# SheffieldML/GPy

Measured on AMD Instinct MI355X. Metric: exact-GP log_lik+grad iters/sec, higher is better.
Workload: dtype f64; 1 GPU; BASELINE configs[2]: matern52 ARD exact GP, one GPRegression.parameters_changed, N=16384 D=32 Dy=1 per GPU; N=16384, D=32, kernel=matern52, ARD=True, parallelism=replicas x1

## Files before the change

### gpy_amd/_lib.py

```python
import ctypes
import os
import subprocess

import numpy as np
from numpy.ctypeslib import ndpointer

_HERE = os.path.dirname(os.path.abspath(__file__))
LIB_PATH = os.environ.get("MI355GP_LIB") or os.path.join(_HERE, "libmi355gp.so")
CSRC = os.path.join(_HERE, "csrc")

KIND_IDS = {"rbf": 0, "matern52": 1, "matern32": 2, "exponential": 3, "white": 4, "bias": 5, "ratquad": 6, "stdperiodic": 7,
            "coregionalize": 8, "linear": 9, "mlp": 10, "poly": 11, "cosine": 12, "sinc": 13, "expquadcosine": 14}


def ard_id(kind, ARD):
    if kind == "coregionalize":
        return int(ARD)
    return int(ARD) & 3 if kind == "stdperiodic" else int(bool(ARD))


class Part(ctypes.Structure):
    _fields_ = [("kind", ctypes.c_int), ("ard", ctypes.c_int), ("n_active", ctypes.c_int),
                ("active_dims", ctypes.POINTER(ctypes.c_int)), ("theta", ctypes.POINTER(ctypes.c_double)),
                ("term", ctypes.c_int)]


def make_parts(specs):
    arr = (Part * len(specs))()
    keep, ntheta = [], 0
    for i, spec in enumerate(specs):
        kind, ARD, theta, dims = spec[:4]
        arr[i].term = int(spec[4]) if len(spec) > 4 else 0
        th = np.ascontiguousarray(theta, dtype=np.float64)
        keep.append(th)
        arr[i].kind = KIND_IDS[kind]
        arr[i].ard = ard_id(kind, ARD)
        arr[i].theta = th.ctypes.data_as(ctypes.POINTER(ctypes.c_double))
        if dims is None:
            arr[i].n_active = 0
            arr[i].active_dims = None
        else:
            d = np.ascontiguousarray(dims, dtype=np.int32)
            keep.append(d)
            arr[i].n_active = d.size
            arr[i].active_dims = d.ctypes.data_as(ctypes.POINTER(ctypes.c_int))
        ntheta += th.size
    return arr, keep, ntheta
FETCH_L, FETCH_KINV, FETCH_DLDK, FETCH_K = 0, 1, 2, 3
EP_BERNOULLI_PROBIT = 0
OUT_LML, OUT_LOGDET, OUT_DATAFIT, OUT_DNOISE, OUT_TRKINV, NUM_OUT = 0, 1, 2, 3, 4, 8
STAGE_NAMES = ("kbuild", "potrf", "trtri", "lauum", "solve", "grad", "total")
NUM_T = 8
PROFILE_FAMILIES = ("update_nt", "trtri", "lauum", "diag128", "trsm128", "update_nt64", "potrf_persist", "trtri_early")

_lib = None


class MI355GPError(RuntimeError):
    pass


DIAG_LIB_PATH = os.path.join(_HERE, "libmi355gp_diag.so")


def build(force=False):
    srcs = [os.path.join(CSRC, f) for f in os.listdir(CSRC) if f.endswith((".hip", ".h")) or f == "Makefile"]
    srcs.append(os.path.join(_HERE, "..", "include", "mi355gp.h"))
    srcs.append(os.path.join(_HERE, "..", "include", "mi355gp_debug.h"))
    product = os.path.join(_HERE, "libmi355gp.so")
    if not force and os.path.exists(product) and os.path.exists(DIAG_LIB_PATH):
        t = min(os.path.getmtime(product), os.path.getmtime(DIAG_LIB_PATH))
        if all(os.path.getmtime(s) <= t for s in srcs if os.path.exists(s)):
            return product
    r = subprocess.run(["make", "-C", CSRC, "-j8", "all", "diag"], capture_output=True, text=True)
    if r.returncode != 0 or not os.path.exists(product) or not os.path.exists(DIAG_LIB_PATH):
        raise MI355GPError("building libmi355gp.so failed:\n" + r.stdout[-4000:] + r.stderr[-4000:])
    return product


_ci, _i64, _cd, _vp, _str = ctypes.c_int, ctypes.c_int64, ctypes.c_double, ctypes.c_void_p, ctypes.c_char_p
_dp = ndpointer(dtype=np.float64, flags="C_CONTIGUOUS")
_c_dp = ctypes.POINTER(ctypes.c_double)
_ip, _hp, _parts = ctypes.POINTER(_ci), ctypes.POINTER(_vp), ctypes.POINTER(Part)
_i32a, _i64a = (ndpointer(dtype=t, flags="C_CONTIGUOUS") for t in (np.int32, np.int64))
_EXACT = [_vp, _ci, _ci, _dp, _dp, _i64, _cd, _cd, _dp] + [_c_dp] * 4
_KERN_X2 = [_dp, _i64, _c_dp, _i64, _ci, _dp]

ABI = {
    "mi355gp_last_error": [],
    "mi355gp_version": [],
    "mi355gp_device_count": [_ip],
    "mi355gp_device_synchronize": [_ci],
    "mi355gp_create": [_ci, _hp],
    "mi355gp_destroy": [_vp],
    "mi355gp_set_data": [_vp, _dp, _i64, _ci, _dp, _ci],
    "mi355gp_set_targets": [_vp, _dp, _ci],
    "mi355gp_kern_K": [_ci, _ci, _ci, _dp] + _KERN_X2,
    "mi355gp_kern_Kdiag": [_ci, _dp, _i64, _dp],
    "mi355gp_update_gradients_full": [_ci, _ci, _ci, _dp, _dp] + _KERN_X2,
    "mi355gp_gradients_X": [_ci, _ci, _ci, _dp, _dp] + _KERN_X2,
    "mi355gp_exact_inference": _EXACT,
    "mi355gp_exact_inference_sum": [_vp, _ci, _parts, _dp, _i64, _cd, _cd, _dp] + [_c_dp] * 4,
    "mi355gp_exact_studentt_sum": [_vp, _ci, _parts, _cd, _cd, _cd, _dp] + [_c_dp] * 3,
    "mi355gp_inference_given_K": [_vp, _dp, _dp, _i64, _cd, _cd, _dp] + [_c_dp] * 3,
    "mi355gp_fetch": [_vp, _ci, _dp, _ci],
    "mi355gp_predict": [_vp, _ci, _ci, _dp, _dp, _i64, _c_dp, _c_dp, _ci],
    "mi355gp_predict_sum": [_vp, _ci, _parts, _dp, _i64, _c_dp, _c_dp, _ci],
    "mi355gp_predictive_gradients_sum": [_vp, _ci, _parts, _dp, _i64, _c_dp, _c_dp],
    "mi355gp_laplace_begin": [_vp, _ci, _parts],
    "mi355gp_laplace_newton": [_vp, _dp, _dp, _cd, _dp, _dp, _c_dp],
    "mi355gp_laplace_finish": [_vp, _dp, _cd, _dp, _c_dp],
    "mi355gp_laplace_gradients": [_vp, _dp, _dp, _dp],
    "mi355gp_laplace_implicit": [_vp, _dp, _dp],
    "mi355gp_laplace_predict": [_vp, _ci, _parts, _dp, _i64, _dp, _c_dp, _c_dp, _ci],
    "mi355gp_ep_recompute": [_vp, _dp, _dp, _cd, _cd, _ci, _dp, _dp, _c_dp, _c_dp],
    "mi355gp_ep_sweep": [_vp, _ci, _i64a, _dp, _cd, _cd] + [_dp] * 7 + [_c_dp],
    "mi355gp_covariance_between_points": [_vp, _ci, _parts, _dp, _i64, _dp, _i64, _dp],
    "mi355gp_potrf": [_ci, _dp, _i64, _c_dp],
    "mi355gp_pdinv": [_ci, _dp, _i64] + [_c_dp] * 4,
    "mi355gp_pdinv_full": [_ci, _dp, _i64] + [_c_dp] * 5,
    "mi355gp_set_option": [_vp, _ci, _ci],
    "mi355gp_get_option": [_vp, _ci, _ip],
    "mi355gp_get_profile": [_vp, _dp, _dp, _i32a],
    "mi355gp_grid_unique_id": [_str],
    "mi355gp_grid_create": [_ci] * 6 + [_str, _hp],
    "mi355gp_grid_destroy": [_vp],
    "mi355gp_grid_set_data": [_vp, _dp, _i64, _ci, _dp, _ci],
    "mi355gp_grid_exact_inference": _EXACT,
    "mi355gp_grid_fetch": [_vp, _ci, _dp],
    "mi355gp_grid_set_option": [_vp, _ci, _ci],
    "mi355gp_grid_get_option": [_vp, _ci, _ip],
    "mi355gp_grid_coll_log": [_vp, _ci, _dp],
    "mi355gp_sparse_create": [_ci, _hp],
    "mi355gp_sparse_destroy": [_vp],
    "mi355gp_sparse_set_data": [_vp, _dp, _i64, _ci, _dp, _ci],
    "mi355gp_vardtc_inference": _EXACT,
    "mi355gp_vardtc_inference_sum": [_vp, _ci, _parts, _dp, _i64, _dp, _i64, _cd, _dp] + [_c_dp] * 6,
    "mi355gp_sparse_set_input_variance": [_vp, _dp, _i64, _ci],
    "mi355gp_sparse_set_inputs": [_vp, _dp, _c_dp, _i64, _ci],
    "mi355gp_vardtc_inference_uncertain": [_vp, _ci, _parts, _dp, _i64, _dp, _i64, _cd, _dp] + [_c_dp] * 6,
    "mi355gp_sparse_predict": [_vp, _ci, _parts, _dp, _i64, _c_dp, _c_dp, _ci],
    "mi355gp_sparse_predict_uncertain": [_vp, _ci, _parts, _dp, _dp, _i64, _dp, _c_dp],
    "mi355gp_sparse_get_predict_ms": [_vp, _c_dp],
    "mi355gp_sparse_fetch_dLdKnm": [_vp, _i64, _i64, _dp],
    "mi355gp_sparse_attach_comm": [_vp, _ci, _ci, _str],
    "mi355gp_sparse_attach_loopback": [_vp, _ci, _ci, _ci],
    "mi355gp_sparse_fetch": [_vp, _ci, _dp],
    "mi355gp_sparse_get_profile": [_vp, _dp],
    "mi355gp_svgp_forward": [_vp, _ci, _parts, _dp, _i64, _dp, _dp, _ci, _cd, _dp, _dp, _dp, _c_dp],
    "mi355gp_svgp_backward": [_vp, _dp, _dp] + [_c_dp] * 5,
    "mi355gp_svgp_predict": [_vp, _ci, _parts, _c_dp, _i64, _ci] + [_c_dp] * 4,
    "mi355gp_pep_inference": [_vp, _ci, _parts, _dp, _i64, _cd, _cd, _cd, _dp] + [_c_dp] * 5,
    "mi355gp_pep_check_sigma": [_dp, _i64, _i64, _cd, _cd],
    "mi355gp_rbf_psi": [_ci, _cd, _dp, _ci, _dp, _i64, _dp, _dp, _i64, _ci] + [_c_dp] * 3,
    "mi355gp_rbf_psi_grad": [_ci, _cd, _dp, _ci, _dp, _i64, _dp, _dp, _i64, _ci] + [_c_dp] * 4 + [_dp] * 5,
    "mi355gp_bench_factor": [_ci, _i64, _ci, _c_dp, _c_dp, _c_dp],
    "mi355gp_dbg_ipc_selftest": [_str, _ci, _ci, _ci, _ci, _i64, _dp],
    "mi355gp_dbg_comm_selftest": [_ci, _str, _ci, _ci, _ci, _ci, _i64, _ci, _dp],
    "mi355gp_dbg_grid_multi": [_ci, _ci, _ci, _ci, _dp],
    "mi355gp_dbg_update_nt": [_ci, _ci, _ip, _ci, _ci, _dp],
    "mi355gp_dbg_update_rect": [_ci, _ci, _ci, _ip, _ci, _ci, _dp],
    "mi355gp_dbg_mfma": [_ci, _dp, _dp, _dp],
    "mi355gp_dbg_gemm": [_ci, _ci, _ci, _i64, _i64, _i64, _dp, _dp, _dp, _cd, _cd, _ci, _c_dp],
    "mi355gp_dbg_peaks": [_ci, _dp],
    "mi355gp_dbg_gemm_clock": [_c_dp, _c_dp],
    "mi355gp_dbg_cu_map": [_ci, _ci, _ci, ctypes.POINTER(ctypes.c_uint)],
    "mi355gp_dbg_pipe_share": [_ci, _dp],
    "mi355gp_dbg_graph_factor": [_ci, _i64, _ci, _dp],
    "mi355gp_dbg_persist": [_ci, _i64, _ci, _ci, _dp],
    "mi355gp_dbg_lauum_plan": [_ci, _ip, _ci, _ip],
    "mi355gp_dbg_persist_owners": [_ci, _ci, _ci, _ip, _ip],
    "mi355gp_dbg_mask_probe": [_ci, _ci, _ci, _dp],
}
EXPORTED = tuple(ABI)


def _opt(a):
    return None if a is None else a.ctypes.data_as(_c_dp)


def lib():
    global _lib
    if _lib is None:
        if not os.path.exists(LIB_PATH):
            build()
        L = ctypes.CDLL(LIB_PATH)
        for name, argtypes in ABI.items():
            getattr(L, name).argtypes = argtypes
        L.mi355gp_last_error.restype = L.mi355gp_version.restype = _str
        _lib = L
    return _lib


OPTIONS = {"profile": 0, "lookahead": 1, "tri_overlap": 2, "tri_min_nt": 3, "tri_h": 4, "tri_wgs": 5, "tri_half": 6,
           "part1_on_panel": 7, "nbo": 8, "solve_overlap": 9, "diag_excl_first": 10, "graph": 11, "persist": 12, "agg2": 13,
           "persist_test": 14, "persist_aborts": 15, "persist_skip": 16, "persist_sched": 17}


def last_error():
    return lib().mi355gp_last_error().decode()


def check(rc, what):
    if rc < 0:
        raise MI355GPError("%s failed (rc=%d): %s" % (what, rc, last_error()))
    return rc


def device_count():
    n = ctypes.c_int(0)
    lib().mi355gp_device_count(ctypes.byref(n))
    return n.value


def device_synchronize(device=0):
    require_device(device)
    check(lib().mi355gp_device_synchronize(int(device)), "mi355gp_device_synchronize")


def require_device(device=0):
    n = device_count()
    if device >= n:
        raise MI355GPError("no MI355X visible to HIP (device %d requested, %d present): the gpy_amd backend has "
                           "no CPU fallback" % (device, n))


def f64(a):
    return np.ascontiguousarray(a, dtype=np.float64)


def theta_vec(variance, lengthscale, ARD, D):
    ls = np.atleast_1d(np.asarray(lengthscale, dtype=np.float64)).ravel()
    if ARD:
        if ls.size == 1:
            ls = np.full(D, ls[0])
        assert ls.size == D, "ARD kernel needs one lengthscale per input dimension"
    else:
        assert ls.size == 1, "isotropic kernel has a single lengthscale"
    return np.concatenate([[float(np.asarray(variance).ravel()[0])], ls])


def _exact_result(out, ms, **arrays):
    res = dict(lml=out[OUT_LML], logdet=out[OUT_LOGDET], datafit=out[OUT_DATAFIT], dnoise=out[OUT_DNOISE],
               trKinv=out[OUT_TRKINV], **arrays)
    if ms is not None:
        res["stage_ms"] = dict(zip(STAGE_NAMES, ms[:len(STAGE_NAMES)]))
    return res


def _predict(entry, head, Xnew, D, Dy, full_cov, want_var, between=()):
    Xnew = f64(Xnew)
    M = Xnew.shape[0]
    assert Xnew.shape[1] == D
    mu = np.empty((M, Dy))
    var = (np.empty((M, M)) if full_cov else np.empty(M)) if want_var else None
    check(getattr(lib(), entry)(*(tuple(head) + (Xnew, M) + tuple(between) + (mu.ctypes.data_as(_c_dp), _opt(var),
                                                                              int(bool(full_cov))))), entry)
    if var is not None and not full_cov:
        var = var[:, None]
    return mu, var


class _Handle(object):
    _create = _destroy = None

    def __init__(self, device=0):
        require_device(device)
        self._h = ctypes.c_void_p()
        check(getattr(lib(), self._create)(device, ctypes.byref(self._h)), self._create)
        self.device = device

    def close(self):
        if getattr(self, "_h", None) is not None and self._h.value:
            getattr(lib(), self._destroy)(self._h)
            self._h = ctypes.c_void_p()

    def __del__(self):
        try:
            self.close()
        except Exception:
            pass


class Context(_Handle):
    _create, _destroy = "mi355gp_create", "mi355gp_destroy"

    def __init__(self, device=0):
        super(Context, self).__init__(device)
        self.N = self.D = self.Dy = 0

    def set_data(self, X, R):
        X, R = f64(X), f64(R)
        assert X.ndim == 2 and R.ndim == 2 and X.shape[0] == R.shape[0]
        self.N, self.D = X.shape
        self.Dy = R.shape[1]
        check(lib().mi355gp_set_data(self._h, X, self.N, self.D, R, self.Dy), "mi355gp_set_data")

    def set_targets(self, R):
        R = f64(R)
        check(lib().mi355gp_set_targets(self._h, R, R.shape[1]), "mi355gp_set_targets")

    def _exact(self, entry, head, ntheta, noise, jitter, extra_jitter, want_alpha, want_diag, want_stage_ms):
        noise = f64(np.atleast_1d(noise))
        out = np.zeros(NUM_OUT)
        alpha = np.empty((self.N, self.Dy)) if want_alpha else None
        dtheta = np.zeros(ntheta)
        diag = np.empty(self.N) if want_diag else None
        ms = np.zeros(NUM_T) if want_stage_ms else None
        rc = check(getattr(lib(), entry)(self._h, *(tuple(head) + (noise, noise.size, jitter, extra_jitter, out, _opt(alpha),
                                                                   _opt(dtheta), _opt(diag), _opt(ms)))), entry)
        return rc, _exact_result(out, ms, alpha=alpha, dtheta=dtheta, diag_dL_dK=diag)

    def exact_inference(self, kind, ARD, theta, noise, jitter=1e-8, extra_jitter=0.0, want_alpha=True,
                        want_diag=False, want_stage_ms=False):
        theta = f64(theta)
        return self._exact("mi355gp_exact_inference", (KIND_IDS[kind], ard_id(kind, ARD), theta), theta.size, noise, jitter,
                           extra_jitter, want_alpha, want_diag, want_stage_ms)

    def exact_inference_sum(self, specs, noise, jitter=1e-8, extra_jitter=0.0, want_alpha=True, want_diag=False,
                            want_stage_ms=False):
        arr, keep, ntheta = make_parts(specs)
        return self._exact("mi355gp_exact_inference_sum", (len(specs), arr), ntheta, noise, jitter, extra_jitter, want_alpha,
                           want_diag, want_stage_ms)

    def predict_sum(self, specs, Xnew, full_cov=False, want_var=True):
        arr, keep, _ = make_parts(specs)
        return _predict("mi355gp_predict_sum", (self._h, len(specs), arr), Xnew, self.D, self.Dy, full_cov, want_var)

    def exact_studentt_sum(self, specs, nu, jitter=1e-8, extra_jitter=0.0):
        arr, keep, ntheta = make_parts(specs)
        out = np.zeros(NUM_OUT)
        alpha = np.empty((self.N, self.Dy))
        dtheta = np.zeros(ntheta)
        rc = check(lib().mi355gp_exact_studentt_sum(self._h, len(specs), arr, float(nu), jitter, extra_jitter, out,
                                                    _opt(alpha), _opt(dtheta), None), "mi355gp_exact_studentt_sum")
        return rc, dict(lml=out[OUT_LML], logdet=out[OUT_LOGDET], beta=out[OUT_DATAFIT], scale=out[5], alpha=alpha,
                        dtheta=dtheta)

    def predictive_gradients(self, specs, Xnew, want_var=True):
        arr, keep, _ = make_parts(specs)
        Xnew = f64(Xnew)
        M = Xnew.shape[0]
        assert Xnew.shape[1] == self.D
        dmu = np.empty((M, self.D, self.Dy))
        dvar = np.empty((M, self.D)) if want_var else None
        check(lib().mi355gp_predictive_gradients_sum(self._h, len(specs), arr, Xnew, M, dmu.ctypes.data_as(_c_dp), _opt(dvar)),
              "mi355gp_predictive_gradients_sum")
        return dmu, dvar

    def covariance_between_points(self, specs, X1, X2):
        arr, keep, _ = make_parts(specs)
        X1, X2 = f64(X1), f64(X2)
        out = np.empty((X1.shape[0], X2.shape[0]))
        check(lib().mi355gp_covariance_between_points(self._h, len(specs), arr, X1, X1.shape[0], X2, X2.shape[0], out),
              "mi355gp_covariance_between_points")
        return out

    def inference_given_K(self, K, noise, jitter=1e-8, extra_jitter=0.0, want_diag=False, want_stage_ms=False):
        K = f64(K)
        assert K.shape == (self.N, self.N)
        noise = f64(np.atleast_1d(noise))
        out = np.zeros(NUM_OUT)
        alpha = np.empty((self.N, self.Dy))
        diag = np.empty(self.N) if want_diag else None
        ms = np.zeros(NUM_T) if want_stage_ms else None
        rc = check(lib().mi355gp_inference_given_K(self._h, K, noise, noise.size, jitter, extra_jitter, out,
                                                   _opt(alpha), _opt(diag), _opt(ms)), "mi355gp_inference_given_K")
        return rc, _exact_result(out, ms, alpha=alpha, diag_dL_dK=diag)

    def laplace_begin(self, specs):
        arr, keep, ntheta = make_parts(specs)
        check(lib().mi355gp_laplace_begin(self._h, len(specs), arr), "mi355gp_laplace_begin")
        self._lap_ntheta = ntheta

    def laplace_newton(self, W, b, extra_jitter=0.0):
        W, b = f64(np.ravel(W)), f64(np.ravel(b))
        assert W.size == self.N and b.size == self.N
        a, Ka = np.empty(self.N), np.empty(self.N)
        ld = ctypes.c_double(0.0)
        rc = check(lib().mi355gp_laplace_newton(self._h, W, b, float(extra_jitter), a, Ka, ctypes.byref(ld)),
                   "mi355gp_laplace_newton")
        return rc, a, Ka, ld.value

    def laplace_finish(self, W, extra_jitter=0.0):
        W = f64(np.ravel(W))
        assert W.size == self.N
        d = np.empty(self.N)
        ld = ctypes.c_double(0.0)
        rc = check(lib().mi355gp_laplace_finish(self._h, W, float(extra_jitter), d, ctypes.byref(ld)), "mi355gp_laplace_finish")
        return rc, d, ld.value

    def laplace_gradients(self, Ki_f, dL_dfhat):
        Ki_f, s = f64(np.ravel(Ki_f)), f64(np.ravel(dL_dfhat))
        assert Ki_f.size == self.N and s.size == self.N
        dtheta = np.zeros(self._lap_ntheta)
        check(lib().mi355gp_laplace_gradients(self._h, Ki_f, s, dtheta), "mi355gp_laplace_gradients")
        return dtheta

    def laplace_implicit(self, dL_dfhat):
        d = f64(np.ravel(dL_dfhat))
        assert d.size == self.N
        s = np.empty(self.N)
        check(lib().mi355gp_laplace_implicit(self._h, d, s), "mi355gp_laplace_implicit")
        return s

    def laplace_predict(self, specs, Xnew, wv, full_cov=False, want_var=True):
        arr, keep, _ = make_parts(specs)
        wv = f64(np.ravel(wv))
        assert wv.size == self.N
        return _predict("mi355gp_laplace_predict", (self._h, len(specs), arr), Xnew, self.D, 1, full_cov, want_var,
                        between=(wv,))

    def ep_recompute(self, tau, v, extra_jitter=0.0, add_diag=0.0, want_sigma=True, want_ms=False):
        tau, v = f64(np.ravel(tau)), f64(np.ravel(v))
        assert tau.size == self.N and v.size == self.N
        mu, sd = np.empty(self.N), np.empty(self.N)
        ld, ms = ctypes.c_double(0.0), ctypes.c_double(0.0)
        rc = check(lib().mi355gp_ep_recompute(self._h, tau, v, float(extra_jitter), float(add_diag), int(bool(want_sigma)), mu, sd,
                                              ctypes.byref(ld), ctypes.byref(ms)), "mi355gp_ep_recompute")
        return (rc, mu, sd, ld.value) + ((ms.value,) if want_ms else ())

    def ep_sweep(self, order, ysign, tau, v, eta=1.0, delta=1.0, lik=EP_BERNOULLI_PROBIT, want_ms=False):
        order = np.ascontiguousarray(np.ravel(order), dtype=np.int64)
        ysign = f64(np.ravel(ysign))
        tau, v = f64(np.ravel(tau)).copy(), f64(np.ravel(v)).copy()
        assert order.size == self.N and ysign.size == self.N and tau.size == self.N and v.size == self.N
        o = [np.empty(self.N) for _ in range(5)]
        ms = ctypes.c_double(0.0)
        check(lib().mi355gp_ep_sweep(self._h, int(lik), order, ysign, float(eta), float(delta), tau, v, o[0], o[1], o[2], o[3], o[4],
                                     ctypes.byref(ms)), "mi355gp_ep_sweep")
        r = dict(tau=tau, v=v, cav_tau=o[0], cav_v=o[1], log_Z_hat=o[2], mu=o[3], Sigma_diag=o[4])
        if want_ms:
            r["ms"] = ms.value
        return r

    def set_option(self, name, value):
        if name == "profile" and not isinstance(value, (int, bool)):
            value = sum(1 << PROFILE_FAMILIES.index(f) for f in value) << 1
        check(lib().mi355gp_set_option(self._h, OPTIONS[name], int(value)), "mi355gp_set_option")

    def get_option(self, name):
        v = ctypes.c_int(0)
        check(lib().mi355gp_get_option(self._h, OPTIONS[name], ctypes.byref(v)), "mi355gp_get_option")
        return int(v.value)

    def get_profile(self):
        ms, fl, n = np.zeros(8), np.zeros(8), np.zeros(8, dtype=np.int32)
        check(lib().mi355gp_get_profile(self._h, ms, fl, n), "mi355gp_get_profile")
        return {k: (ms[i], fl[i], int(n[i])) for i, k in enumerate(PROFILE_FAMILIES)}

    def predict(self, kind, ARD, theta, Xnew, full_cov=False, want_var=True):
        return _predict("mi355gp_predict", (self._h, KIND_IDS[kind], ard_id(kind, ARD), f64(theta)), Xnew, self.D, self.Dy,
                        full_cov, want_var)

    def fetch(self, which, fortran_order=False):
        out = np.empty((self.N, self.N))
        check(lib().mi355gp_fetch(self._h, which, out, int(fortran_order)), "mi355gp_fetch")
        if fortran_order:
            return out.T
        return out


class SparseContext(_Handle):
    FETCH_DLDKMM, FETCH_WOODBURY_INV, FETCH_LM, FETCH_KMM, FETCH_PSI2, FETCH_DLDPSI2_BETA = 0, 1, 2, 3, 4, 5
    sharded = False
    _create, _destroy = "mi355gp_sparse_create", "mi355gp_sparse_destroy"

    def __init__(self, device=0):
        super(SparseContext, self).__init__(device)
        self.N = self.D = self.Dy = self.M = 0

    def attach_comm(self, rank, world, id_bytes):
        check(lib().mi355gp_sparse_attach_comm(self._h, rank, world, id_bytes), "mi355gp_sparse_attach_comm")
        self.sharded = True

    def set_data(self, X, Y):
        X, Y = f64(X), f64(Y)
        self.N, self.D = X.shape
        self.Dy = Y.shape[1]
        check(lib().mi355gp_sparse_set_data(self._h, X, self.N, self.D, Y, self.Dy), "mi355gp_sparse_set_data")

    def get_profile(self):
        o = np.zeros(6)
        check(lib().mi355gp_sparse_get_profile(self._h, o), "mi355gp_sparse_get_profile")
        return {"gemm_T": (o[0], o[1], int(o[2])), "gram_psi2": (o[3], o[4], int(o[5]))}

    def _fit(self, entry, head, ntheta, Z, scalars, extras, want_stage_ms, wv_cols=None):
        Z = f64(Z)
        self.M = Z.shape[0]
        assert Z.shape[1] == self.D
        out = np.zeros(NUM_OUT)
        dtheta = np.zeros(ntheta)
        dZ = np.zeros((self.M, self.D))
        wv = np.zeros((self.M, self.Dy if wv_cols is None else wv_cols))
        ms = np.zeros(4) if want_stage_ms else None
        args = tuple(head) + (Z, self.M) + tuple(scalars) + (out, _opt(dtheta), _opt(dZ), _opt(wv))
        rc = check(getattr(lib(), entry)(self._h, *(args + tuple(_opt(e) for e in extras) + (_opt(ms),))), entry)
        res = dict(lml=out[0], dnoise=out[1], dtheta=dtheta, dZ=dZ, woodbury_vector=wv)
        if ms is not None:
            res["stage_ms"] = dict(pass1=ms[0], mxm=ms[1], pass2=ms[2], total=ms[3])
        return rc, out, res

    def vardtc(self, kind, ARD, theta, Z, noise_var, extra_jitter=0.0, want_stage_ms=False):
        theta = f64(theta)
        rc, out, res = self._fit("mi355gp_vardtc_inference", (KIND_IDS[kind], int(bool(ARD)), theta), theta.size, Z,
                                 (float(noise_var), float(extra_jitter)), (), want_stage_ms)
        res.update(trA=out[2], data_fit=out[3])
        return rc, res

    def fetch(self, which):
        out = np.empty((self.M, self.M))
        check(lib().mi355gp_sparse_fetch(self._h, which, out), "mi355gp_sparse_fetch")
        return out

    def attach_loopback(self, rank, world, group_key):
        check(lib().mi355gp_sparse_attach_loopback(self._h, rank, world, int(group_key)), "mi355gp_sparse_attach_loopback")
        self.sharded = True

    def vardtc_sum(self, specs, Z, noise, extra_jitter=0.0, want_dL_dm=False, want_stage_ms=False):
        arr, keep, ntheta = make_parts(specs)
        noise = f64(np.atleast_1d(noise)).ravel()
        rows = np.zeros((self.N, self.Dy)) if noise.size > 1 else None
        dm = np.zeros((self.N, self.Dy)) if want_dL_dm else None
        rc, out, res = self._fit("mi355gp_vardtc_inference_sum", (len(specs), arr), ntheta, Z,
                                 (noise, noise.size, float(extra_jitter)), (rows, dm), want_stage_ms)
        if rows is not None:
            res["dnoise"] = rows[:, 0] if self.Dy == 1 else rows
        res.update(trA=out[2], data_fit=out[3], dL_dm=dm)
        return rc, res

    def set_input_variance(self, S):
        S = f64(S)
        assert S.ndim == 2, "S must be N x D"
        check(lib().mi355gp_sparse_set_input_variance(self._h, S, S.shape[0], S.shape[1]), "mi355gp_sparse_set_input_variance")

    def set_inputs(self, X, S=None):
        X = f64(X)
        S = None if S is None else f64(S)
        assert X.ndim == 2 and (S is None or S.shape == X.shape), "X and S must be N x D"
        check(lib().mi355gp_sparse_set_inputs(self._h, X, _opt(S), X.shape[0], X.shape[1]), "mi355gp_sparse_set_inputs")

    def predict_uncertain(self, specs, mu_new, S_new, want_var=True):
        arr, keep, _ = make_parts(specs)
        mu_new, S_new = f64(mu_new), f64(S_new)
        assert mu_new.ndim == 2 and mu_new.shape[1] == self.D and S_new.shape == mu_new.shape, "mu_new and S_new must be M* x D"
        Mn = mu_new.shape[0]
        mean = np.empty((Mn, self.Dy))
        var = np.empty((Mn, self.Dy)) if want_var else None
        check(lib().mi355gp_sparse_predict_uncertain(self._h, len(specs), arr, mu_new, S_new, Mn, mean, _opt(var)),
              "mi355gp_sparse_predict_uncertain")
        return mean, var

    def predict_ms(self):
        out = np.zeros(1)
        check(lib().mi355gp_sparse_get_predict_ms(self._h, out.ctypes.data_as(_c_dp)), "mi355gp_sparse_get_predict_ms")
        return float(out[0])

    def vardtc_uncertain(self, specs, Z, noise, extra_jitter=0.0, want_dmu_dS=True, want_stage_ms=False):
        arr, keep, ntheta = make_parts(specs)
        noise = f64(np.atleast_1d(noise)).ravel()
        dmu = np.zeros((self.N, self.D)) if want_dmu_dS else None
        dS = np.zeros((self.N, self.D)) if want_dmu_dS else None
        rc, out, res = self._fit("mi355gp_vardtc_inference_uncertain", (len(specs), arr), ntheta, Z,
                                 (noise, noise.size, float(extra_jitter)), (dmu, dS), want_stage_ms)
        res.update(trA=out[2], data_fit=out[3], dmu=dmu, dS=dS)
        return rc, res

    def predict(self, specs, Xnew, full_cov=False, want_var=True):
        arr, keep, _ = make_parts(specs)
        return _predict("mi355gp_sparse_predict", (self._h, len(specs), arr), Xnew, self.D, self.Dy, full_cov, want_var)

    def fetch_dL_dKnm(self, row0, nrows):
        out = np.empty((nrows, self.M))
        check(lib().mi355gp_sparse_fetch_dLdKnm(self._h, int(row0), int(nrows), out), "mi355gp_sparse_fetch_dLdKnm")
        return out

    def pep(self, specs, Z, noise_variance, alpha, jitter, want_stage_ms=False):
        arr, keep, ntheta = make_parts(specs)
        dR = np.zeros(self.N)
        rc, out, res = self._fit("mi355gp_pep_inference", (len(specs), arr), ntheta, Z,
                                 (float(noise_variance), float(alpha), float(jitter)), (dR,), want_stage_ms, wv_cols=1)
        res.update(sum_dL_dR=out[2], dL_dR=dR)
        return rc, res

    def svgp_forward(self, specs, Z, q_mean, q_chol, extra_jitter=0.0, want_stage_ms=False):
        arr, keep, ntheta = make_parts(specs)
        Z, q_mean, q_chol = f64(Z), f64(q_mean), f64(q_chol)
        self.M = Z.shape[0]
        assert Z.shape[1] == self.D
        assert q_mean.ndim == 2 and q_mean.shape[0] == self.M, "q_mean must be M x L"
        L = q_mean.shape[1]
        assert q_chol.shape == (L, self.M, self.M), "q_chol must be L x M x M"
        self.L, self._svgp_ntheta = L, ntheta
        mu, v = np.zeros((self.N, L)), np.zeros((self.N, L))
        sc = np.zeros(2 + L)
        ms = np.zeros(3) if want_stage_ms else None
        rc = check(lib().mi355gp_svgp_forward(self._h, len(specs), arr, Z, self.M, q_mean, q_chol, L, float(extra_jitter), mu, v,
                                              sc, _opt(ms)), "mi355gp_svgp_forward")
        res = dict(mu=mu, v=v, KL=sc[0], logdet_Kmm=sc[1], logdet_S=sc[2:2 + L].copy())
        if ms is not None:
            res["stage_ms"] = dict(mxm=ms[0], rows=ms[1], total=ms[2])
        return rc, res

    def svgp_backward(self, dF_dmu, dF_dv, want_stage_ms=False):
        L = getattr(self, "L", 0)
        dF_dmu, dF_dv = f64(dF_dmu), f64(dF_dv)
        if L:
            assert dF_dmu.shape == (self.N, L) and dF_dv.shape == (self.N, L), "dF_dmu and dF_dv must be N x L"
        dtheta = np.zeros(getattr(self, "_svgp_ntheta", 0))
        dZ, dm, dchol = np.zeros((self.M, self.D)), np.zeros((self.M, L)), np.zeros((L, self.M, self.M))
        ms = np.zeros(3) if want_stage_ms else None
        check(lib().mi355gp_svgp_backward(self._h, dF_dmu, dF_dv, _opt(dtheta), _opt(dZ), _opt(dm), _opt(dchol), _opt(ms)),
              "mi355gp_svgp_backward")
        res = dict(dtheta=dtheta, dZ=dZ, dL_dm=dm, dL_dchol=dchol)
        if ms is not None:
            res["stage_ms"] = dict(rows=ms[0], mxm=ms[1], total=ms[2])
        return res

    def svgp_predict(self, specs, Xnew, full_cov=False, want_var=True):
        arr, keep, _ = make_parts(specs)
        Xnew = f64(Xnew)
        Mn, L = Xnew.shape[0], getattr(self, "L", 1)
        assert Xnew.shape[1] == self.D
        mu = np.empty((Mn, L))
        var = (np.empty((Mn, Mn, L)) if full_cov else np.empty((Mn, L))) if want_var else None
        check(lib().mi355gp_svgp_predict(self._h, len(specs), arr, Xnew.ctypes.data_as(_c_dp), Mn, int(bool(full_cov)),
                                         mu.ctypes.data_as(_c_dp), _opt(var), None, None), "mi355gp_svgp_predict")
        return mu, var

    def svgp_woodbury(self, want_inv=True):
        L = getattr(self, "L", 1)
        wv = np.empty((self.M, L))
        wi = np.empty((L, self.M, self.M)) if want_inv else None
        check(lib().mi355gp_svgp_predict(self._h, 0, None, None, 0, 0, None, None, wv.ctypes.data_as(_c_dp), _opt(wi)),
              "mi355gp_svgp_predict")
        return wv, (None if wi is None else np.ascontiguousarray(np.transpose(wi, (1, 2, 0))))


def _point_sets(X, X2, dL_dK=None):
    X = f64(X)
    N, D = X.shape
    if X2 is None:
        M, p2 = N, None
    else:
        X2 = f64(X2)
        M, p2 = X2.shape[0], X2.ctypes.data_as(_c_dp)
        assert X2.shape[1] == D
    if dL_dK is None:
        return X, N, p2, M, D
    G = f64(dL_dK)
    assert G.shape == (N, M), "dL_dK must be N x M"
    return G, X, N, p2, M, D


def kern_K(kind, ARD, theta, X, X2=None, device=0):
    require_device(device)
    sets = _point_sets(X, X2)
    out = np.empty((sets[1], sets[3]))
    check(lib().mi355gp_kern_K(device, KIND_IDS[kind], ard_id(kind, ARD), f64(theta), *(sets + (out,))), "mi355gp_kern_K")
    return out


def kern_Kdiag(kind, theta, N):
    out = np.empty(N)
    check(lib().mi355gp_kern_Kdiag(KIND_IDS[kind], f64(theta), N, out), "mi355gp_kern_Kdiag")
    return out


def update_gradients_full(kind, ARD, theta, dL_dK, X, X2=None, device=0):
    require_device(device)
    theta = f64(theta)
    out = np.zeros(theta.size)
    check(lib().mi355gp_update_gradients_full(device, KIND_IDS[kind], ard_id(kind, ARD), theta,
                                              *(_point_sets(X, X2, dL_dK) + (out,))), "mi355gp_update_gradients_full")
    return out


def gradients_X(kind, ARD, theta, dL_dK, X, X2=None, device=0):
    require_device(device)
    sets = _point_sets(X, X2, dL_dK)
    out = np.zeros(sets[1].shape)
    check(lib().mi355gp_gradients_X(device, KIND_IDS[kind], ard_id(kind, ARD), f64(theta), *(sets + (out,))),
          "mi355gp_gradients_X")
    return out


def _psi_args(variance, lengthscale, ARD, Z, mu, S, weights):
    Z, mu, S = f64(Z), f64(mu), f64(S)
    N, D = mu.shape
    assert S.shape == mu.shape and Z.ndim == 2 and Z.shape[1] == D, "Z is M x D, mu and S are N x D"
    ls = theta_vec(variance, lengthscale, ARD, D)[1:]
    w = None if weights is None else f64(np.ravel(weights))
    assert w is None or w.size == N
    return (float(np.ravel(variance)[0]), f64(ls), int(bool(ARD)), Z, Z.shape[0], mu, S, N, D, _opt(w)), w


def rbf_psi(variance, lengthscale, ARD, Z, mu, S, weights=None, want_psi1=True, want_psi2=True, device=0):
    require_device(device)
    args, keep = _psi_args(variance, lengthscale, ARD, Z, mu, S, weights)
    M, N = args[4], args[7]
    p1 = np.empty((N, M)) if want_psi1 else None
    p2 = np.empty((M, M)) if want_psi2 else None
    check(lib().mi355gp_rbf_psi(device, *(args + (_opt(p1), _opt(p2)))), "mi355gp_rbf_psi")
    return p1, p2


def rbf_psi_grad(variance, lengthscale, ARD, Z, mu, S, dL_dpsi0=None, dL_dpsi1=None, dL_dpsi2=None, weights=None, device=0):
    require_device(device)
    args, keep = _psi_args(variance, lengthscale, ARD, Z, mu, S, weights)
    M, N, D = args[4], args[7], args[8]
    d0 = None if dL_dpsi0 is None else f64(np.ravel(dL_dpsi0))
    d1 = None if dL_dpsi1 is None else f64(dL_dpsi1)
    d2 = None if dL_dpsi2 is None else f64(dL_dpsi2)
    assert d0 is None or d0.size == N
    assert d1 is None or d1.shape == (N, M), "dL_dpsi1 must be N x M"
    assert d2 is None or d2.shape == (M, M), "dL_dpsi2 must be M x M"
    dvar, dl = np.zeros(1), np.zeros(D if ARD else 1)
    dZ, dmu, dS = np.zeros((M, D)), np.zeros((N, D)), np.zeros((N, D))
    check(lib().mi355gp_rbf_psi_grad(device, *(args + (_opt(d0), _opt(d1), _opt(d2), dvar, dl, dZ, dmu, dS))),
          "mi355gp_rbf_psi_grad")
    return dvar[0], dl, dZ, dmu, dS


def potrf(A, device=0):
    require_device(device)
    L = f64(A).copy()
    ms = ctypes.c_double(0.0)
    info = check(lib().mi355gp_potrf(device, L, L.shape[0], ctypes.byref(ms)), "mi355gp_potrf")
    return L, info, ms.value


def pdinv(A, device=0):
    require_device(device)
    A = f64(A)
    n = A.shape[0]
    Ai, L = np.empty((n, n)), np.empty((n, n))
    ld, ms = ctypes.c_double(0.0), ctypes.c_double(0.0)
    info = check(lib().mi355gp_pdinv(device, A, n, Ai.ctypes.data_as(_c_dp), L.ctypes.data_as(_c_dp),
                                     ctypes.byref(ld), ctypes.byref(ms)), "mi355gp_pdinv")
    return Ai, L, ld.value, info, ms.value


def pdinv_full(A, device=0):
    require_device(device)
    A = f64(A)
    n = A.shape[0]
    Ai, L, Li = np.empty((n, n)), np.empty((n, n)), np.empty((n, n))
    ld, ms = ctypes.c_double(0.0), ctypes.c_double(0.0)
    info = check(lib().mi355gp_pdinv_full(device, A, n, Ai.ctypes.data_as(_c_dp), L.ctypes.data_as(_c_dp),
                                          Li.ctypes.data_as(_c_dp), ctypes.byref(ld), ctypes.byref(ms)), "mi355gp_pdinv_full")
    return Ai, L, Li, ld.value, info


def bench_factor(N, reps=3, device=0):
    require_device(device)
    p, t, l = ctypes.c_double(0.0), ctypes.c_double(0.0), ctypes.c_double(0.0)
    check(lib().mi355gp_bench_factor(device, N, reps, ctypes.byref(p), ctypes.byref(t), ctypes.byref(l)),
          "mi355gp_bench_factor")
    fl = float(N) ** 3 / 3.0
    return {"potrf_ms": p.value, "trtri_ms": t.value, "lauum_ms": l.value,
            "potrf_tflops": fl / p.value / 1e9, "trtri_tflops": fl / t.value / 1e9, "lauum_tflops": fl / l.value / 1e9}


def dbg_persist(N, reps=3, kcap=0, device=0):
    require_device(device)
    nt = (int(N) + 127) // 128
    out = np.zeros(8 + 32 * nt)
    check(lib().mi355gp_dbg_persist(device, int(N), int(reps), int(kcap), out), "mi355gp_dbg_persist")
    st = out[8:8 + 8 * nt].reshape(nt, 8)
    near = out[8 + 8 * nt:8 + 20 * nt].reshape(nt, 3, 4)
    far = out[8 + 20 * nt:].reshape(nt, 12)
    return dict(ms_steps=out[0], ms_persist=out[1], mismatches=int(out[2]), info=int(out[3]), abort=int(out[4]), nt=nt,
                steps=(st - st[0, 0]) / 100.0, near=(near - st[0, 0]) / 100.0, far=(far - st[0, 0]) / 100.0)


def dbg_mask_probe(pct=75, order=0, device=0):
    require_device(device)
    out = np.zeros(3)
    check(lib().mi355gp_dbg_mask_probe(device, pct, order, out), "mi355gp_dbg_mask_probe")
    return out


def dbg_mfma(a, b, device=0):
    require_device(device)
    d = np.zeros(256)
    check(lib().mi355gp_dbg_mfma(device, f64(a), f64(b), d), "dbg_mfma")
    return d.reshape(64, 4)


def dbg_gemm(A, B, C, a_mcontig, b_ncontig, alpha=1.0, beta=0.0, reps=0, device=0):
    require_device(device)
    A, B, C = f64(A), f64(B), f64(C).copy()
    M, K = (A.shape[1], A.shape[0]) if a_mcontig else A.shape
    N = B.shape[1] if b_ncontig else B.shape[0]
    ms = ctypes.c_double(0.0)
    check(lib().mi355gp_dbg_gemm(device, int(a_mcontig), int(b_ncontig), M, N, K, A, B, C, alpha, beta, reps,
                                 ctypes.byref(ms)), "dbg_gemm")
    return C, ms.value


def dbg_gemm_clock():
    mhz, cyc = ctypes.c_double(0.0), ctypes.c_double(0.0)
    check(lib().mi355gp_dbg_gemm_clock(ctypes.byref(mhz), ctypes.byref(cyc)), "dbg_gemm_clock")
    return mhz.value, cyc.value


def dbg_peaks(device=0):
    require_device(device)
    out = np.zeros(8)
    check(lib().mi355gp_dbg_peaks(device, out), "dbg_peaks")
    return dict(mfma_f64_tflops=out[0], valu_f64_tflops=out[1], hbm_copy_gbs=out[2], hbm_fill_gbs=out[3],
                mfma_cycles_per_inst_1wave=out[4], shader_mhz_under_load=out[5], mfma_1wave_tflops=out[6],
                mfma_cycles_per_inst_loaded=out[7])


def dbg_grid_multi(T, nb=512, reps=3, device=0):
    require_device(device)
    out = np.zeros(5)
    check(lib().mi355gp_dbg_grid_multi(device, int(T), int(nb), int(reps), out), "mi355gp_dbg_grid_multi")
    return out


def dbg_update_nt(nt, ks, reps=5, device=0):
    require_device(device)
    ka = (ctypes.c_int * len(ks))(*[int(k) for k in ks])
    out = np.zeros(len(ks))
    check(lib().mi355gp_dbg_update_nt(device, int(nt), ka, len(ks), int(reps), out), "mi355gp_dbg_update_nt")
    return out


def dbg_update_rect(ntr, ntc, ks, reps=5, device=0):
    require_device(device)
    ka = (ctypes.c_int * len(ks))(*[int(k) for k in ks])
    out = np.zeros(len(ks))
    check(lib().mi355gp_dbg_update_rect(device, int(ntr), int(ntc), ka, len(ks), int(reps), out), "mi355gp_dbg_update_rect")
    return out


def persist_owners(nt, nw, tune=0):
    owner = (ctypes.c_int * (nt * nt))()
    out4 = (ctypes.c_int * 4)()
    dup = lib().mi355gp_dbg_persist_owners(nt, nw, tune, owner, out4)
    return np.frombuffer(owner, dtype=np.int32, count=nt * nt).reshape(nt, nt).copy(), out4[0], out4[1], out4[2], out4[3], dup


def lauum_plan(nt):
    out4 = (ctypes.c_int * 4)()
    lib().mi355gp_dbg_lauum_plan(nt, None, 0, out4)
    n = out4[0]
    buf = (ctypes.c_int * (6 * max(n, 1)))()
    check(lib().mi355gp_dbg_lauum_plan(nt, buf, n, out4), "mi355gp_dbg_lauum_plan")
    return np.frombuffer(buf, dtype=np.int32, count=6 * n).reshape(n, 6).copy(), out4[1], out4[2], out4[3]
```

### gpy_amd/csrc/api.hip

```cpp
#include <cstdarg>
#include <cstdio>
#include <climits>
#include <string>
#include <vector>

#include "ctx.h"

static thread_local std::string g_err;

void mi355gp_set_error(const char* fmt, ...) {
    char buf[1024];
    va_list ap;
    va_start(ap, fmt);
    vsnprintf(buf, sizeof(buf), fmt, ap);
    va_end(ap);
    g_err = buf;
}

void apply_options(mi355gp_ctx* c) {
    FactorWs& w = c->ws;
    auto set = [&](int o, int* field) { if (c->opt[o] != INT_MIN) *field = c->opt[o]; };
    set(MI355GP_OPT_LOOKAHEAD, &w.lookahead);
    set(MI355GP_OPT_TRI_OVERLAP, &w.tri_overlap);
    set(MI355GP_OPT_TRI_MIN_NT, &w.tri_min_nt);
    set(MI355GP_OPT_TRI_H, &w.tri_h_override);
    set(MI355GP_OPT_TRI_WGS, &w.tri_wgs);
    set(MI355GP_OPT_TRI_HALF, &w.tri_half_ok);
    set(MI355GP_OPT_PART1_ON_PANEL, &w.part1_on_panel);
    set(MI355GP_OPT_NBO, &w.nbo_override);
    set(MI355GP_OPT_SOLVE_OVERLAP, &w.solve_overlap);
    set(MI355GP_OPT_DIAG_EXCL_FIRST, &w.diag_excl_first);
    set(MI355GP_OPT_PERSIST, &w.persist);
    set(MI355GP_OPT_AGG2, &w.agg2);
    if (c->opt[MI355GP_OPT_GRAPH] != INT_MIN) c->graph_enabled = c->opt[MI355GP_OPT_GRAPH] ? 1 : 0;
}

void drop_graph(mi355gp_ctx* c) {
    if (c->fgraph) (void)hipGraphExecDestroy(c->fgraph);
    c->fgraph = nullptr;
    c->fgraph_calls = 0;
}

void free_data(mi355gp_ctx* c) {
    drop_graph(c);
    c->parts.clear();
    double** ptrs[] = {&c->dX, &c->dR, &c->dNoise, &c->A, &c->B, &c->C, &c->Mbuf,
                       &c->dTmp, &c->dTrmvPart, &c->dGradPart, &c->dGradOut, &c->dPack, &c->dCoregPart};
    for (auto p : ptrs) {
        if (*p) (void)hipFree(*p);
        *p = nullptr;
    }
    if (c->hPack) (void)hipHostFree(c->hPack);
    c->hPack = nullptr;
    c->dAlpha = c->dScal = c->dDiag = c->dGradOutAll = nullptr;
    c->hIdx.clear();
    c->hIdxCol = -1;
    laplace_session_free(c->lap);
    c->lap = nullptr;
    c->lap_stage = 0;
    factor_ws_free(&c->ws);
    c->have_factor = c->have_kernel = false;
}

int ctx_prepare_parts(mi355gp_ctx* c, int nparts, const mi355gp_part* parts) {
    ARG_CHECK(nparts >= 1 && nparts <= 16 && parts, "between 1 and 16 kernel parts");
    if ((int)c->parts.size() != nparts) {
        c->parts.clear();
        c->parts.resize((size_t)nparts);
        for (auto& p : c->parts) HIP_CHECK(p.dXt.alloc((size_t)c->D * c->npad));
    }
    for (int i = 0; i < nparts; ++i) {
        mi355gp_ctx::Part& p = c->parts[(size_t)i];
        if (int rc = parse_part(parts[i], c->D, KS_STATIONARY | KS_STATIC | KS_EXT | KS_COREG | KS_LINEAR | KS_DOT | KS_OSC, "exact-GP path", &p)) return rc;
        if (p.coreg()) {
            const int col = p.kp.col;
            if (c->hIdxCol != col) {
                c->hIdx.resize((size_t)c->n);
                HIP_CHECK(hipMemcpy2D(c->hIdx.data(), sizeof(double), c->dX + col, sizeof(double) * c->D, sizeof(double), c->n,
                                      hipMemcpyDeviceToHost));
                c->hIdxCol = col;
            }
            if (int rc = coreg_check_index(c->hIdx.data(), c->n, 1, p.kp.ard, "training")) return rc;
            if (!c->dCoregPart) HIP_CHECK(hipMalloc(&c->dCoregPart, sizeof(double) * grad_num_blocks(c->n) * COREG_REC));
        }
        if (int rc = p.upload(c->st)) return rc;
    }
    c->terms = group_terms(c->parts);
    if (has_product(c->terms) && !c->Mbuf) HIP_CHECK(hipMalloc(&c->Mbuf, sizeof(double) * c->npad * c->npad));
    return 0;
}

void ctx_scale_parts(mi355gp_ctx* c) {
    for (auto& p : c->parts) launch_scale_inputs(c->st, c->dX, c->n, c->D, p.dIl,  1, p.dXt, c->npad);
}
Resident<mi355gp_ctx::Part> ctx_training_points(const mi355gp_ctx* c) { return {&mi355gp_ctx::Part::dXt, c->npad, c->n}; }

int ctx_coreg_check_points(const mi355gp_ctx* c, const double* Xn, int64_t M, const char* what) {
    for (const auto& p : c->parts)
        if (p.coreg())
            if (int rc = coreg_check_index(Xn + p.kp.col, M, c->D, p.kp.ard, what)) return rc;
    return 0;
}
bool ctx_has_point_diag(const mi355gp_ctx* c) {
    for (const auto& p : c->parts)
        if (p.diag_by_point()) return true;
    return false;
}
std::vector<double> ctx_kdiag_points(const mi355gp_ctx* c, const double* Xn, int64_t M) {
    std::vector<double> kd((size_t)M, 0.0);
    for (int64_t m = 0; m < M; ++m) {
        double s = 0.0;
        for (const auto& t : c->terms) {
            double v = 1.0;
            for (int f : t) {
                const mi355gp_ctx::Part& p = c->parts[(size_t)f];
                if (p.coreg()) {
                    const int a = (int)Xn[m * c->D + p.kp.col], P = p.kp.ard;
                    v *= p.theta[(size_t)(a * P + a)];
                } else if (p.linear()) {
                    double d = 0.0;
                    for (size_t a = 0; a < p.dims.size(); ++a) {
                        const double x = Xn[m * c->D + p.dims[a]];
                        d += p.theta[p.kp.ard ? a : 0] * x * x;
                    }
                    v *= d;
                } else if (p.mlp()) {
                    v *= mlp_kdiag(p, Xn + m * c->D);
                } else if (p.poly()) {
                    v *= poly_kdiag(p, Xn + m * c->D);
                } else {
                    v *= p.kp.variance;
                }
            }
            s += v;
        }
        kd[(size_t)m] = s;
    }
    return kd;
}

extern "C" {

const char* mi355gp_last_error(void) { return g_err.c_str(); }
const char* mi355gp_version(void) { return "mi355gp 0.1 (gfx950)"; }

int mi355gp_device_synchronize(int device) {
    HIP_CHECK(hipSetDevice(device));
    HIP_CHECK(hipDeviceSynchronize());
    return 0;
}

int mi355gp_device_count(int* count) {
    int n = 0;
    hipError_t e = hipGetDeviceCount(&n);
    if (e != hipSuccess) {
        (void)hipGetLastError();
        n = 0;
    }
    *count = n;
    return 0;
}

int mi355gp_create(int device, mi355gp_ctx** out) {
    int n = 0;
    mi355gp_device_count(&n);
    if (device < 0 || device >= n) {
        mi355gp_set_error("mi355gp_create: device %d not available (%d HIP devices visible)", device, n);
        return -2;
    }
    HIP_CHECK(hipSetDevice(device));
    mi355gp_ctx* c = new mi355gp_ctx();
    c->device = device;
    for (int& o : c->opt) o = INT_MIN;
    if (factor_engine(device, &c->st, nullptr, nullptr) != 0) return -2;
    for (auto& e : c->ev) HIP_CHECK(hipEventCreate(&e));
    {
        const char* e = PRODUCT_ENV("GRAPH");
        if (e && *e) c->graph_enabled = atoi(e) ? 1 : 0;
    }
    *out = c;
    return 0;
}

int mi355gp_destroy(mi355gp_ctx* c) {
    if (!c) return 0;
    (void)hipSetDevice(c->device);
    (void)hipStreamSynchronize(c->st);
    free_data(c);
    for (auto& e : c->ev)
        if (e) (void)hipEventDestroy(e);
    if (c->st) (void)hipStreamSynchronize(c->st);
    delete c;
    return 0;
}

int mi355gp_set_data(mi355gp_ctx* c, const double* X, int64_t N, int D, const double* R, int Dy) {
    ARG_CHECK(c && X && R && N > 0 && D > 0 && Dy > 0, "mi355gp_set_data: bad arguments");
    HIP_CHECK(hipSetDevice(c->device));
    EngineShared gate(c->device);
    HIP_CHECK(hipStreamSynchronize(c->st));
    free_data(c);
    c->n = N;
    c->npad = round_up(N, NB);
    c->D = D;
    c->Dy = Dy;
    const long np = c->npad;
    HIP_CHECK(hipMalloc(&c->dX, sizeof(double) * N * D));
    HIP_CHECK(hipMalloc(&c->dR, sizeof(double) * N * Dy));
    HIP_CHECK(hipMalloc(&c->dNoise, sizeof(double) * N));
    HIP_CHECK(hipMalloc(&c->A, sizeof(double) * np * np));
    HIP_CHECK(hipMalloc(&c->B, sizeof(double) * np * np));
    HIP_CHECK(hipMalloc(&c->C, sizeof(double) * np * np));
    if (factor_ws_alloc(&c->ws, np) != 0) return -3;
    c->ws.can_calibrate = 1;
    {
        const int lookahead = c->ws.lookahead;
        const char* e = PRODUCT_ENV("GRAPH");
        c->graph_enabled = (e && *e) ? (atoi(e) ? 1 : 0) : 1;
        apply_options(c);
        if (c->opt[MI355GP_OPT_LOOKAHEAD] == INT_MIN) c->ws.lookahead = lookahead;
    }
    HIP_CHECK(hipMalloc(&c->dTmp, sizeof(double) * N * Dy));
    const long nchunks = (N + trmv_chunk_rows(N) - 1) / trmv_chunk_rows(N);
    HIP_CHECK(hipMalloc(&c->dTrmvPart, sizeof(double) * nchunks * N * Dy));
    const int groups = (D + 31) / 32;
    c->gradPartDoubles = 2L * groups * 2048 * GP_STRIDE;
    HIP_CHECK(hipMalloc(&c->dGradPart, sizeof(double) * c->gradPartDoubles));
    HIP_CHECK(hipMalloc(&c->dGradOut, sizeof(double) * groups * GP_STRIDE));
    c->offGrad = 8;
    c->offExt = c->offGrad + (size_t)16 * groups * GP_STRIDE;
    c->offAlpha = c->offExt + (size_t)16 * groups * GP_STRIDE;
    c->offDiag = c->offAlpha + (size_t)N * Dy;
    c->offCoreg = c->offDiag + (size_t)N;
    c->packDoubles = c->offCoreg + (size_t)16 * COREG_REC;
    HIP_CHECK(hipMalloc(&c->dPack, sizeof(double) * c->packDoubles));
    HIP_CHECK(hipHostMalloc(&c->hPack, sizeof(double) * c->packDoubles, hipHostMallocDefault));
    c->dScal = c->dPack;
    c->dGradOutAll = c->dPack + c->offGrad;
    c->dAlpha = c->dPack + c->offAlpha;
    c->dDiag = c->dPack + c->offDiag;
    HIP_CHECK(hipMemcpy(c->dX, X, sizeof(double) * N * D, hipMemcpyHostToDevice));
    HIP_CHECK(hipMemcpy(c->dR, R, sizeof(double) * N * Dy, hipMemcpyHostToDevice));
    return 0;
}

int mi355gp_set_targets(mi355gp_ctx* c, const double* R, int Dy) {
    ARG_CHECK(c && R && c->n > 0 && Dy == c->Dy, "mi355gp_set_targets: set_data first / Dy mismatch");
    HIP_CHECK(hipSetDevice(c->device));
    EngineShared gate(c->device);
    HIP_CHECK(hipStreamSynchronize(c->st));
    HIP_CHECK(hipMemcpy(c->dR, R, sizeof(double) * c->n * Dy, hipMemcpyHostToDevice));
    return 0;
}

int mi355gp_fetch(mi355gp_ctx* c, int which, double* out, int fortran_order) {
    ARG_CHECK(c && c->n > 0 && out, "mi355gp_fetch: bad arguments");
    HIP_CHECK(hipSetDevice(c->device));
    EngineShared gate(c->device);
    const long n = c->n, np = c->npad;
    hipStream_t st = c->st;
    DevBuf tmp, scratch;
    HIP_CHECK(tmp.alloc(n * n));
    if (c->lap_stage > 0) {
        if (int rc = laplace_fetch(c, which, tmp)) return rc;
    } else if (which == MI355GP_FETCH_K) {
        if (!c->have_kernel) {
            mi355gp_set_error("mi355gp_fetch(K): no device kernel evaluation in this context");
            return -4;
        }
        if (has_product(c->terms)) HIP_CHECK(scratch.alloc(n * n));
        const auto x = ctx_training_points(c);
        emit_cross(st, c->parts, c->terms, x, x, tmp, n, scratch, false, 1);
    } else if (!c->have_factor) {
        mi355gp_set_error("mi355gp_fetch: no successful factorisation in this context");
        return -4;
    } else if (which == MI355GP_FETCH_L) {
        launch_extract(st, c->A, np, n, 0, nullptr, 0, tmp, fortran_order);
    } else if (which == MI355GP_FETCH_LINV) {
        launch_extract(st, c->B, np, n, 0, nullptr, 0, tmp, fortran_order);
    } else if (which == MI355GP_FETCH_KINV) {
        launch_extract(st, c->C, np, n, 1, nullptr, 0, tmp, 0);
    } else if (which == MI355GP_FETCH_DLDK) {
        launch_extract(st, c->C, np, n, 2, c->dAlpha, c->Dy, tmp, 0, c->studentt ? c->dScal + 4 : nullptr);
    } else {
        mi355gp_set_error("mi355gp_fetch: unknown matrix id %d", which);
        return -1;
    }
    HIP_CHECK(hipMemcpyAsync(out, tmp, sizeof(double) * n * n, hipMemcpyDeviceToHost, st));
    HIP_CHECK(hipStreamSynchronize(st));
    return 0;
}

int mi355gp_set_option(mi355gp_ctx* c, int option, int value) {
    ARG_CHECK(c != nullptr, "mi355gp_set_option: NULL context");
    if (option == MI355GP_OPT_PROFILE) {
        c->ws.prof.on = (value != 0);
        c->ws.prof.mask = (value == 1) ? 0xffu : (unsigned)value >> 1;
        return 0;
    }
    if (option == MI355GP_OPT_PERSIST_TEST) {
#ifndef MI355GP_DIAG
        if (value != 0) {
            mi355gp_set_error("mi355gp_set_option: MI355GP_OPT_PERSIST_TEST is a test hook of the diagnostics build (libmi355gp_diag.so)");
            return -1;
        }
#endif
        c->ws.persist_test = value;
        if (value) c->ws.persist_skip = 0;
        drop_graph(c);
        return 0;
    }
    if (option < 0 || option >= MI355GP_OPT_NUM || option == MI355GP_OPT_PERSIST_ABORTS || option == MI355GP_OPT_PERSIST_SKIP ||
        option == MI355GP_OPT_PERSIST_SCHED) {
        mi355gp_set_error("mi355gp_set_option: unknown or read-only option %d", option);
        return -1;
    }
    if (option == MI355GP_OPT_LOOKAHEAD) value = (value == 0) ? 0 : 1;
    if (option == MI355GP_OPT_NBO && value > 0 && value % NB != 0) {
        mi355gp_set_error("mi355gp_set_option: NBO must be a multiple of %d", NB);
        return -1;
    }
    c->opt[option] = (value < 0) ? INT_MIN : value;
    if (value < 0) {
        FactorWs d;
#define env(name, dflt) diag_env_int(DIAG_ENV(name), dflt)
#define penv(name, dflt) diag_env_int(PRODUCT_ENV(name), dflt)
        switch (option) {
            case MI355GP_OPT_LOOKAHEAD: c->ws.lookahead = d.lookahead; break;
            case MI355GP_OPT_TRI_OVERLAP: c->ws.tri_overlap = penv("TRI_OVERLAP", d.tri_overlap) ? 1 : 0; break;
            case MI355GP_OPT_TRI_MIN_NT: c->ws.tri_min_nt = env("TRI_MIN_NT", d.tri_min_nt); break;
            case MI355GP_OPT_TRI_H: c->ws.tri_h_override = env("TRI_H", d.tri_h_override); break;
            case MI355GP_OPT_TRI_WGS: c->ws.tri_wgs = env("TRI_WGS", d.tri_wgs); break;
            case MI355GP_OPT_TRI_HALF: c->ws.tri_half_ok = env("TRI_HALF", d.tri_half_ok) ? 1 : 0; break;
            case MI355GP_OPT_PART1_ON_PANEL: c->ws.part1_on_panel = env("PART1_ON_PANEL", d.part1_on_panel) ? 1 : 0; break;
            case MI355GP_OPT_NBO: c->ws.nbo_override = env("NBO", d.nbo_override); break;
            case MI355GP_OPT_SOLVE_OVERLAP: c->ws.solve_overlap = env("SOLVE_OVERLAP", d.solve_overlap) ? 1 : 0; break;
            case MI355GP_OPT_DIAG_EXCL_FIRST: c->ws.diag_excl_first = env("DIAG_EXCL_FIRST", d.diag_excl_first) ? 1 : 0; break;
            case MI355GP_OPT_PERSIST: c->ws.persist = penv("PERSIST", d.persist); break;
            case MI355GP_OPT_AGG2: c->ws.agg2 = env("AGG2", d.agg2) ? 1 : 0; break;
            case MI355GP_OPT_GRAPH: c->graph_enabled = penv("GRAPH", 1) ? 1 : 0; break;
            default: break;
        }
#undef env
#undef penv
    }
    if (option == MI355GP_OPT_PERSIST) {
        c->ws.persist_auto_off = 0;
        c->ws.sched_force_steps = 0;
        c->ws.sched_np = c->ws.sched_ns = 0;
        c->ws.sched_state = (value < 0) ? 0 : 2;
    }
    apply_options(c);
    drop_graph(c);
    return 0;
}

int mi355gp_get_option(mi355gp_ctx* c, int option, int* value) {
    ARG_CHECK(c && value && option > MI355GP_OPT_PROFILE && option < MI355GP_OPT_NUM, "mi355gp_get_option: bad arguments");
    const FactorWs& w = c->ws;
    const int v[MI355GP_OPT_NUM] = {0, w.lookahead, w.tri_overlap, w.tri_min_nt, w.tri_h_override, w.tri_wgs, w.tri_half_ok,
                                    w.part1_on_panel, w.nbo_override, w.solve_overlap, w.diag_excl_first, c->graph_enabled,
                                    w.persist, w.agg2, w.persist_test, w.persist_aborts, w.persist_skip,
                                    w.sched_state == 2 ? ((w.persist_auto_off || !w.persist) ? 2 : 1) : 0};
    *value = v[option];
    return 0;
}

int mi355gp_get_profile(mi355gp_ctx* c, double* ms, double* flops, int* launches) {
    ARG_CHECK(c && ms && flops && launches, "mi355gp_get_profile: NULL argument");
    HIP_CHECK(hipSetDevice(c->device));
    HIP_CHECK(hipStreamSynchronize(c->st));
    if (c->ws.st_panel) HIP_CHECK(hipStreamSynchronize(c->ws.st_panel));
    if (c->ws.prof.collect(ms, flops, launches) != 0) {
        mi355gp_set_error("mi355gp_get_profile: event timing failed");
        return -5;
    }
    return 0;
}

}
```

### gpy_amd/csrc/common.h

```cpp
#pragma once
#include <hip/hip_runtime.h>
#include <stdint.h>

typedef double d4 __attribute__((ext_vector_type(4)));
typedef double d2 __attribute__((ext_vector_type(2)));

#define NB 128
#define NBO 512
#define FACTOR_NBO_SMALL_N 0
#define FACTOR_NBO_SMALL 256
#define FACTOR_DEFAULT_TRI_OVERLAP 1
#define FACTOR_DEFAULT_PERSIST 1
#define FACTOR_PERSIST_MAX_NT 64
#define PS_ABORT_INFO (1 << 30)
#define PS_ABORT_CLEAN ((1 << 30) + 1)
#define PS_SKIP_AFTER_CLEAN 16
#define FACTOR_DEFAULT_DIAG_EXCL_FIRST 1
#define GEMM_DEFAULT_TRI64_MAX 512
#define GEMM_DEFAULT_LAUUM64_MAX 528
#define LAUUM_SPLIT_MAX_NT 44
#define GEMM_DEFAULT_UPD64_MAX 128

__device__ __forceinline__ d4 mfma_f64(double a, double b, d4 c) {
    return __builtin_amdgcn_mfma_f64_16x16x4f64(a, b, c, 0, 0, 0);
}

void mi355gp_set_error(const char* fmt, ...);
#define HIP_CHECK(expr)                                                                          \
    do {                                                                                         \
        hipError_t _e = (expr);                                                                  \
        if (_e != hipSuccess) {                                                                  \
            mi355gp_set_error("%s failed: %s (%s:%d)", #expr, hipGetErrorString(_e), __FILE__,  \
                              __LINE__);                                                         \
            return -(1000 + (int)_e);                                                            \
        }                                                                                        \
    } while (0)
#define ARG_CHECK(cond, msg)              \
    do {                                  \
        if (!(cond)) {                    \
            mi355gp_set_error("%s", msg); \
            return -1;                    \
        }                                 \
    } while (0)

template <typename T>
struct DevArr {
    T* p = nullptr;
    DevArr() = default;
    DevArr(DevArr&& o) noexcept : p(o.p) { o.p = nullptr; }
    DevArr(const DevArr&) = delete;
    DevArr& operator=(const DevArr&) = delete;
    DevArr& operator=(DevArr&& o) noexcept {
        if (this != &o) {
            if (p) (void)hipFree(p);
            p = o.p;
            o.p = nullptr;
        }
        return *this;
    }
    ~DevArr() {
        if (p) (void)hipFree(p);
    }
    hipError_t alloc(size_t count) { return hipMalloc(&p, sizeof(T) * (count ? count : 1)); }
    operator T*() const { return p; }
};
typedef DevArr<double> DevBuf;

static inline int64_t round_up(int64_t n, int64_t m) { return (n + m - 1) / m * m; }

#define MI355GP_LOCAL __attribute__((visibility("hidden")))

#include <cstdlib>
#define PRODUCT_ENV(name) getenv("MI355GP_" name)
#ifdef MI355GP_DIAG
#define DIAG_ENV(name) getenv("MI355GP_" name)
#else
#define DIAG_ENV(name) ((const char*)nullptr)
#endif
static inline int diag_env_int(const char* v, int dflt) { return (v && *v) ? atoi(v) : dflt; }
```

### gpy_amd/csrc/factor.hip

```cpp
#include <cstdlib>
#include <mutex>
#include <vector>

#include "internal.h"

void KernelProf::begin(hipStream_t st, int fam, double flops) {
    open = on && ((mask >> fam) & 1u);
    if (!open) return;
    const size_t e0 = 2 * recs.size();
    while (pool.size() < e0 + 2) {
        hipEvent_t e;
        (void)hipEventCreate(&e);
        pool.push_back(e);
    }
    recs.push_back(Rec{fam, flops, e0});
    (void)hipEventRecord(pool[e0], st);
}

void KernelProf::end(hipStream_t st) {
    if (!open) return;
    open = false;
    (void)hipEventRecord(pool[recs.back().e0 + 1], st);
}

int KernelProf::collect(double* ms, double* flops, int* launches) {
    for (int f = 0; f < PF_NUM; ++f) { ms[f] = 0.0; flops[f] = 0.0; launches[f] = 0; }
    for (const Rec& r : recs) {
        float t = 0.f;
        if (hipEventElapsedTime(&t, pool[r.e0], pool[r.e0 + 1]) != hipSuccess) return -1;
        ms[r.fam] += t;
        flops[r.fam] += r.flops;
        launches[r.fam] += 1;
    }
    return 0;
}

void KernelProf::destroy() {
    for (hipEvent_t e : pool) (void)hipEventDestroy(e);
    pool.clear();
    recs.clear();
}

struct FactorEngine {
    hipStream_t main = nullptr, panel = nullptr, tri = nullptr, tri_half = nullptr;
    int tri_pct = 0;
    bool ready = false;
};
static FactorEngine g_engine[16];
static std::mutex g_engine_mutex;
static std::shared_mutex g_engine_gate[16];
std::shared_mutex& engine_gate(int device) { return g_engine_gate[device & 15]; }

int factor_engine(int device, hipStream_t* main, hipStream_t* panel, hipStream_t* tri, hipStream_t* tri_half) {
    if (device < 0 || device >= 16) return -1;
    std::lock_guard<std::mutex> lock(g_engine_mutex);
    FactorEngine& e = g_engine[device];
    if (!e.ready) {
        int least = 0, greatest = 0;
        HIP_CHECK(hipDeviceGetStreamPriorityRange(&least, &greatest));
        HIP_CHECK(hipStreamCreateWithFlags(&e.main, hipStreamNonBlocking));
        HIP_CHECK(hipStreamCreateWithPriority(&e.panel, hipStreamNonBlocking, greatest));
        const char* envc = DIAG_ENV("TRI_CU_PCT");
        e.tri_pct = (envc && *envc) ? atoi(envc) : 75;
        hipDeviceProp_t prop;
        HIP_CHECK(hipGetDeviceProperties(&prop, device));
        const int ncu = prop.multiProcessorCount, nx = 8;
        if (e.tri_pct > 0 && e.tri_pct < 100 && ncu % nx == 0) {
            const int per = ncu / nx, keep = (per * e.tri_pct + 50) / 100;
            std::vector<uint32_t> mask((size_t)(ncu + 31) / 32, 0u);
            const char* envm = DIAG_ENV("TRI_MASK_MODE");
            const int mode = (envm && *envm) ? atoi(envm) : 0;
            for (int cu = 0; cu < ncu; ++cu) {
                const int idx = cu / nx;
                bool on = idx < keep;
                if (mode == 1) on = (idx % 4) != 3;
                if (mode == 2) on = idx >= per - keep;
                if (on) mask[cu / 32] |= 1u << (cu % 32);
            }
            if (hipExtStreamCreateWithCUMask(&e.tri, (uint32_t)mask.size(), mask.data()) != hipSuccess) {
                (void)hipGetLastError();
                e.tri = nullptr;
            }
        }
        if (!e.tri) HIP_CHECK(hipStreamCreateWithPriority(&e.tri, hipStreamNonBlocking, least));
        if (ncu % nx == 0) {
            const int per = ncu / nx, keep = per / 2;
            std::vector<uint32_t> mask((size_t)(ncu + 31) / 32, 0u);
            for (int cu = 0; cu < ncu; ++cu)
                if (cu / nx < keep) mask[cu / 32] |= 1u << (cu % 32);
            if (hipExtStreamCreateWithCUMask(&e.tri_half, (uint32_t)mask.size(), mask.data()) != hipSuccess) {
                (void)hipGetLastError();
                e.tri_half = nullptr;
            }
        }
        {
            void* touch = nullptr;
            if (hipMalloc(&touch, 256) == hipSuccess) {
                hipStream_t order[4] = {e.main, e.panel, e.tri, e.tri_half};
                for (hipStream_t s : order)
                    if (s) {
                        (void)hipMemsetAsync(touch, 0, 256, s);
                        (void)hipStreamSynchronize(s);
                    }
                (void)hipFree(touch);
            }
        }
        e.ready = true;
    }
    if (main) *main = e.main;
    if (panel) *panel = e.panel;
    if (tri) *tri = e.tri;
    if (tri_half) *tri_half = e.tri_half;
    return 0;
}

static bool lauum_plan_wanted(const FactorWs* ws, int nt);
static bool lauum_plan_build(FactorWs* ws, int nt);
int factor_ws_alloc(FactorWs* ws, long npad) {
    ws->nblk = npad / NB;
    HIP_CHECK(hipMalloc(&ws->dinv, sizeof(double) * ws->nblk * 8 * 256));
    HIP_CHECK(hipMalloc(&ws->logsum, sizeof(double) * ws->nblk));
    HIP_CHECK(hipMalloc(&ws->info, sizeof(int) * 4));
    int least = 0, greatest = 0;
    HIP_CHECK(hipDeviceGetStreamPriorityRange(&least, &greatest));
    int dev = 0;
    HIP_CHECK(hipGetDevice(&dev));
    if (factor_engine(dev, nullptr, &ws->st_panel, &ws->st_tri, &ws->st_tri_half) != 0) return -1;
    {
        const char* envo = PRODUCT_ENV("TRI_OVERLAP");
        if (envo && *envo) ws->tri_overlap = atoi(envo) ? 1 : 0;
        const char* envn2 = DIAG_ENV("TRI_MIN_NT");
        if (envn2 && *envn2) ws->tri_min_nt = atoi(envn2);
        const char* envw2 = DIAG_ENV("TRI_WGS");
        if (envw2 && *envw2) ws->tri_wgs = atoi(envw2);
        ws->tri_cu_pct = g_engine[dev].tri_pct > 0 && g_engine[dev].tri_pct <= 100 ? g_engine[dev].tri_pct : 75;
        HIP_CHECK(hipEventCreateWithFlags(&ws->ev_tri, hipEventDisableTiming));
        HIP_CHECK(hipEventCreateWithFlags(&ws->ev_tri_lead, hipEventDisableTiming));
        HIP_CHECK(hipMalloc(&ws->tri_counter, sizeof(int) * 4));
        const char* envh = DIAG_ENV("TRI_H");
        if (envh && *envh) ws->tri_h_override = atoi(envh);
    }
    const char* envp1 = DIAG_ENV("PART1_ON_PANEL");
    if (envp1 && *envp1) ws->part1_on_panel = atoi(envp1) ? 1 : 0;
    ws->sched_state = ws->sched_force_steps = ws->persist_auto_off = 0;
    ws->sched_np = ws->sched_ns = 0;
    ws->evals_done = ws->early_pending = 0;
    const char* envpa = PRODUCT_ENV("PERSIST_AUTO");
    if (envpa && *envpa) ws->persist_auto = atoi(envpa) ? 1 : 0;
    const char* envls = DIAG_ENV("LAUUM_SPLIT");
    if (envls && *envls) ws->lauum_split = atoi(envls) > 0 ? atoi(envls) : 0;
    const char* envptri = DIAG_ENV("PERSIST_TRI");
    if (envptri && *envptri) ws->persist_tri = atoi(envptri) ? 1 : 0;
    const char* envptn = DIAG_ENV("PERSIST_TRI_MIN_NT");
    if (envptn && *envptn) ws->persist_tri_min_nt = atoi(envptn);
#ifdef MI355GP_DIAG
    const char* envuq = DIAG_ENV("DBG_UPD_QUEUE");
    if (envuq && *envuq && atoi(envuq)) {
        ws->upd_queue_probe = 1;
        HIP_CHECK(hipMalloc(&ws->upd_tasks, sizeof(UpdTask) * 64 + 64));
    }
#endif
    const char* envag = DIAG_ENV("AGG2");
    if (envag && *envag) ws->agg2 = atoi(envag) ? 1 : 0;
    const char* envnbo = DIAG_ENV("NBO");
    if (envnbo && *envnbo) ws->nbo_override = atoi(envnbo);
    const char* envso = DIAG_ENV("SOLVE_OVERLAP");
    if (envso && *envso) ws->solve_overlap = atoi(envso) ? 1 : 0;
    const char* envth = DIAG_ENV("TRI_HALF");
    if (envth && *envth) ws->tri_half_ok = atoi(envth) ? 1 : 0;
    const char* envps = PRODUCT_ENV("PERSIST");
    if (envps && *envps) ws->persist = atoi(envps);
    const char* envpm = DIAG_ENV("PERSIST_MAX_NT");
    if (envpm && *envpm) ws->persist_max_nt = atoi(envpm);
    const char* envpt = DIAG_ENV("PERSIST_TUNE");
    if (envpt && *envpt) ws->persist_tune = atoi(envpt);
    const char* envpk = DIAG_ENV("PERSIST_KCAP");
    if (envpk && *envpk) ws->persist_kcap = atoi(envpk) > 0 ? atoi(envpk) : 1;
    {
        hipDeviceProp_t prop;
        HIP_CHECK(hipGetDeviceProperties(&prop, dev));
        ws->persist_cus = prop.multiProcessorCount;
        const char* envpc = DIAG_ENV("PERSIST_WGS");
        if (envpc && *envpc && atoi(envpc) >= 2 && atoi(envpc) <= ws->persist_cus) ws->persist_cus = atoi(envpc);
        HIP_CHECK(hipMalloc(&ws->persist_sync, sizeof(int) * potrf_persist_sync_ints()));
        HIP_CHECK(hipMalloc(&ws->persist_hs, sizeof(double) * (size_t)(ws->nblk < 64 ? ws->nblk : 64) * NB * NB));
    }
    const char* envx = DIAG_ENV("DIAG_EXCL_FIRST");
    if (envx && *envx) ws->diag_excl_first = atoi(envx) ? 1 : 0;
    HIP_CHECK(hipEventCreateWithFlags(&ws->ev_fork, hipEventDisableTiming));
    HIP_CHECK(hipEventCreateWithFlags(&ws->ev_early_pre, hipEventDisableTiming));
    if (lauum_plan_wanted(ws, (int)ws->nblk)) (void)lauum_plan_build(ws, (int)ws->nblk);
    const size_t nouter = (size_t)(npad + NB - 1) / NB + 2;
    ws->ev_panel.resize(nouter);
    ws->ev_cols.resize(nouter);
    for (size_t i = 0; i < nouter; ++i) {
        HIP_CHECK(hipEventCreateWithFlags(&ws->ev_panel[i], hipEventDisableTiming));
        HIP_CHECK(hipEventCreateWithFlags(&ws->ev_cols[i], hipEventDisableTiming));
    }
    return 0;
}

void factor_ws_free(FactorWs* ws) {
    if (ws->dinv) (void)hipFree(ws->dinv);
    if (ws->logsum) (void)hipFree(ws->logsum);
    if (ws->info) (void)hipFree(ws->info);
    ws->dinv = ws->logsum = nullptr;
    ws->info = nullptr;
    for (hipEvent_t e : ws->ev_panel) (void)hipEventDestroy(e);
    for (hipEvent_t e : ws->ev_cols) (void)hipEventDestroy(e);
    ws->ev_panel.clear();
    ws->ev_cols.clear();
    if (ws->ev_fork) (void)hipEventDestroy(ws->ev_fork);
    ws->ev_fork = nullptr;
    if (ws->ev_early_pre) (void)hipEventDestroy(ws->ev_early_pre);
    ws->ev_early_pre = nullptr;
    ws->st_panel = nullptr;
    ws->st_tri = nullptr;
    ws->st_tri_half = ws->st_tri_cur = nullptr;
    if (ws->ev_tri) (void)hipEventDestroy(ws->ev_tri);
    ws->ev_tri = nullptr;
    if (ws->ev_tri_lead) (void)hipEventDestroy(ws->ev_tri_lead);
    ws->ev_tri_lead = nullptr;
    if (ws->tri_counter) (void)hipFree(ws->tri_counter);
    ws->tri_counter = nullptr;
    if (ws->upd_tasks) (void)hipFree(ws->upd_tasks);
    ws->upd_tasks = nullptr;
    if (ws->lauum_plan_dev) (void)hipFree(ws->lauum_plan_dev);
    ws->lauum_plan_dev = nullptr;
    if (ws->lauum_part) (void)hipFree(ws->lauum_part);
    ws->lauum_part = nullptr;
    ws->lauum_plan_nt = 0;
    if (ws->persist_sync) (void)hipFree(ws->persist_sync);
    ws->persist_sync = nullptr;
    if (ws->persist_hs) (void)hipFree(ws->persist_hs);
    ws->persist_hs = nullptr;
    ws->prof.destroy();
}

static double syrk_flops(double n, double K) { return K * n * (n + 1.0); }
static double gemm_flops(double m, double n, double K) { return 2.0 * m * n * K; }

static void factor_panel(hipStream_t s, double* A, long npad, long K0, long W, FactorWs* ws) {
    const long ld = npad;
    for (long j = 0; j < W; j += NB) {
        const long c = K0 + j, blk = c / NB;
        double* dv = ws->dinv + blk * 8 * 256;
        ws->prof.begin(s, PF_DIAG, (double)NB * NB * NB / 3.0);
        launch_diag128(s, A, ld, c, dv, ws->logsum + blk, ws->info,
                       ws->diag_excl_first && c == K0 && ws->lookahead == 1 && ws->excl_first_ok);
        ws->prof.end(s);
        const long below = npad - (c + NB);
        if (below <= 0) continue;
        ws->prof.begin(s, PF_TRSM, (double)below * NB * NB);
        launch_trsm128(s, A, ld, c, c + NB, below, dv);
        ws->prof.end(s);
        const long cd = c + NB, ncols = K0 + W - cd;
        if (ncols <= 0) continue;
        const double* P = A + cd * ld + c;
        ws->prof.begin(s, update_nt_uses_64((int)(below / NB), (int)(ncols / NB), (int)(cd / NB), (int)(cd / NB)) ? PF_UPDATE64 : PF_UPDATE,
                       syrk_flops((double)ncols, (double)NB) + gemm_flops((double)(below - ncols), (double)ncols, (double)NB));
        launch_update_nt(s, A + cd * ld + cd, ld, P, ld, P, ld, NB, (int)(below / NB), (int)(ncols / NB), (int)(cd / NB), (int)(cd / NB));
        ws->prof.end(s);
    }
}

static void update_cols(hipStream_t s, double* A, long npad, long K0, long W, long c0, long c1, FactorWs* ws) {
    if (c1 <= c0) return;
    const long ld = npad, rows = npad - c0, cols = c1 - c0;
    const double* P = A + c0 * ld + K0;
    ws->prof.begin(s, update_nt_uses_64((int)(rows / NB), (int)(cols / NB), (int)(c0 / NB), (int)(c0 / NB)) ? PF_UPDATE64 : PF_UPDATE,
                   syrk_flops((double)cols, (double)W) + gemm_flops((double)(rows - cols), (double)cols, (double)W));
    launch_update_nt(s, A + c0 * ld + c0, ld, P, ld, P, ld, (int)W, (int)(rows / NB), (int)(cols / NB), (int)(c0 / NB),
                     (int)(c0 / NB));
    ws->prof.end(s);
}

static void potrf_serial(hipStream_t st, double* A, long npad, FactorWs* ws) {
    (void)hipMemsetAsync(ws->info, 0, sizeof(int) * 4, st);
    const long nbo = ws->nbo_for(npad);
    const long P = (npad + nbo - 1) / nbo;
    auto pcol = [&](long p) { return (p * nbo < npad) ? p * nbo : npad; };
    for (long p = 0; p < P; ++p) {
        factor_panel(st, A, npad, pcol(p), pcol(p + 1) - pcol(p), ws);
        update_cols(st, A, npad, pcol(p), pcol(p + 1) - pcol(p), pcol(p + 1), npad, ws);
    }
}

static void early_inverse(hipStream_t sq, double* A, long npad, int h, FactorWs* ws, bool gated, int gate_gives_up = 0) {
    const int ntl = (int)(npad / NB);
    (void)hipMemsetAsync(ws->tri_counter, 0, sizeof(int) * 4, sq);
    if (gated) launch_wait_persist_rows(sq, ws, 0, h, 0, gate_gives_up);
    ws->prof.begin(sq, PF_TRTRI_EARLY, 0.0);
    launch_inv128(sq, A, ws->scratchX, npad, h, ws->dinv);
    int level = 0;
    for (; (1 << level) < h; ++level) launch_trtri_level(sq, A, ws->scratchX, ws->scratchT, npad, h, level);
    (void)hipEventRecord(ws->ev_tri_lead, sq);
    const int nt_pair = ntl < 2 * h ? ntl : 2 * h;
    if (gated) launch_wait_persist_rows(sq, ws, h, nt_pair, h);
    launch_trtri_stage1_steal(sq, A, ws->scratchX, ws->scratchT, npad, nt_pair, level, ws->tri_counter,
                              ws->tri_wgs > 0 ? ws->tri_wgs : 512 * ws->tri_cur_pct / 100);
    ws->prof.end(sq);
    (void)hipEventRecord(ws->ev_tri, sq);
    ws->early_pending = 1;
}

int persist_early_h(long npad, const FactorWs* ws) {
    const int ntl = (int)(npad / NB);
    if (!potrf_persist_eligible(npad, ws) || !ws->tri_overlap || !ws->persist_tri || !ws->st_tri || !ws->scratchX || !ws->scratchT ||
        ntl < ws->persist_tri_min_nt || ws->evals_done < 1)
        return 0;
    int h = 1;
    static const int two_thirds = diag_env_int(DIAG_ENV("PERSIST_TRI_H23"), 1);
    if (two_thirds) while (6 * h <= 2 * ntl) h *= 2;
    else while (4 * h <= ntl) h *= 2;
    return h;
}

void calibrate_schedule(FactorWs& w, float ms, int nt) {
    if (w.sched_state == 0 && w.persist_used && w.evals_done >= 3) {
        w.sched_ms_persist = (w.sched_np == 0 || ms < w.sched_ms_persist) ? ms : w.sched_ms_persist;
        if (++w.sched_np >= 2) {
            w.sched_state = 1;
            w.sched_force_steps = 3;
            w.sched_ns = 0;
        }
    } else if (w.sched_state == 1 && !w.persist_used) {
        if (w.sched_ns++ > 0) w.sched_ms_steps = (w.sched_ns == 2 || ms < w.sched_ms_steps) ? ms : w.sched_ms_steps;
        if (w.sched_ns >= 3) {
            w.sched_state = 2;
            w.sched_force_steps = 0;
            w.persist_auto_off = (w.sched_ms_steps < 0.97f * w.sched_ms_persist) ? 1 : 0;
            if (nt >= 21) persist_box_verdict(w.persist_auto_off);
        }
    }
}

void potrf_device(hipStream_t st, double* A, long npad, FactorWs* ws) {
    if (ws->early_pending) {
        (void)hipStreamWaitEvent(st, ws->ev_tri, 0);
        ws->early_pending = 0;
    }
    ws->ovl_h = 0;
    ws->persist_used = 0;
    if (potrf_persist_eligible(npad, ws)) {
        const int h = persist_early_h(npad, ws);
        const int gate_gives_up = (ws->persist_test == 3) ? 1 : 0;
        hipEvent_t pre_saved = ws->ev_persist_pre;
        if (h > 0 && !ws->ev_persist_pre) ws->ev_persist_pre = ws->ev_early_pre;
        const bool ok = launch_potrf_persist(st, A, npad, ws);
        hipEvent_t pre = ws->ev_persist_pre;
        ws->ev_persist_pre = pre_saved;
        if (ok) {
            ws->persist_used = 1;
            if (h > 0) {
                hipStream_t sq = ws->st_tri;
                ws->tri_cur_pct = ws->tri_cu_pct;
                (void)hipStreamWaitEvent(sq, pre, 0);
                launch_wait_persist_resident(sq, ws, 50);
                early_inverse(sq, A, npad, h, ws, true, gate_gives_up);
                ws->ovl_h = h;
            }
            return;
        }
        ws->persist = 0;
    } else if (ws->persist_skip > 0 && ws->persist_skip != 0x7fffffff) {
        --ws->persist_skip;
    }
    if (ws->sched_force_steps > 0) --ws->sched_force_steps;
    if (ws->lookahead != 1) {
        potrf_serial(st, A, npad, ws);
        return;
    }
    (void)hipMemsetAsync(ws->info, 0, sizeof(int) * 4, st);
    const long nbo = ws->nbo_for(npad);
    const long P = (npad + nbo - 1) / nbo;
    auto pcol = [&](long p) { return (p * nbo < npad) ? p * nbo : npad; };
    hipStream_t sp = ws->st_panel;
    hipStream_t su = st;
    (void)hipEventRecord(ws->ev_fork, st);
    (void)hipStreamWaitEvent(sp, ws->ev_fork, 0);
    factor_panel(sp, A, npad, 0, pcol(1), ws);
    const int ntl = (int)(npad / NB);
    int ovl_h = 0;
    if (ws->tri_overlap && ws->st_tri && ws->scratchX && ws->scratchT && ntl >= ws->tri_min_nt) {
        int h = 1;
        while (2 * h < ntl) h *= 2;
        for (; h >= 8; h /= 2) {
            const double lead = (double)h * NB, rest = (double)npad - lead;
            const double t_lead = lead * lead * lead / 3.0 / 45e12;
            const double t_tail = rest * rest * rest / 3.0 / 50e12 + rest / (double)nbo * 0.45e-3 * ((double)nbo / NBO);
            if (t_lead <= t_tail) break;
        }
        if (ws->tri_h_override > 0) h = ws->tri_h_override;
        if (h >= 8 && h < ntl && (h & (h - 1)) == 0) ovl_h = h;
        if (ovl_h > 0) {
            const double lead = (double)ovl_h * NB, rest = (double)npad - lead, right = rest < lead ? rest : lead;
            const double t_early = (lead * lead * lead / 3.0 + lead * lead * right) / 60e12;
            const double t_tail = rest * rest * rest / 3.0 / 50e12 + rest / (double)nbo * 0.45e-3 * ((double)nbo / NBO);
            ws->st_tri_cur = (ws->st_tri_half && ws->tri_half_ok && t_early < 0.8 * t_tail) ? ws->st_tri_half : ws->st_tri;
            ws->tri_cur_pct = (ws->st_tri_cur == ws->st_tri_half) ? 50 : ws->tri_cu_pct;
        }
    }
    ws->ovl_h = 0;
    ws->excl_first_ok = (ovl_h == 0 && ntl < ws->tri_min_nt) ? 1 : 0;
#ifdef MI355GP_DIAG
    const bool uq = ws->upd_queue_probe && ws->upd_tasks && ws->part1_on_panel && ntl >= ws->tri_min_nt && !ws->agg2 && P <= 64;
#else
    const bool uq = false;
#endif
#ifdef MI355GP_DIAG
    if (uq) {
        std::vector<UpdTask> tasks;
        for (long p = 0; p + 2 < P; ++p) {
            const long c0 = pcol(p + 2), ntr = (npad - c0) / NB;
            tasks.push_back(UpdTask{c0 * npad + c0, c0 * npad + pcol(p), ntr * (ntr + 1) / 2, (int)(pcol(p + 1) - pcol(p)), (int)ntr});
        }
        int* counter = reinterpret_cast<int*>(ws->upd_tasks + 64);
        (void)hipMemcpyAsync(ws->upd_tasks, tasks.data(), sizeof(UpdTask) * tasks.size(), hipMemcpyHostToDevice, su);
        (void)hipMemsetAsync(counter, 0, sizeof(int), su);
        ws->prof.begin(su, PF_UPDATE, 0.0);
        launch_update_nt_queue(su, A, npad, ws->upd_tasks, (int)tasks.size(), counter, 512);
        ws->prof.end(su);
    }
#endif
    for (long p = 0; p + 1 < P; ++p) {
        const long K0 = pcol(p), W = pcol(p + 1) - K0;
        (void)hipEventRecord(ws->ev_panel[p], sp);
        if (ovl_h > 0 && pcol(p + 1) == (long)ovl_h * NB) {
            hipStream_t sq = ws->st_tri_cur ? ws->st_tri_cur : ws->st_tri;
            (void)hipStreamWaitEvent(sq, ws->ev_panel[p], 0);
            early_inverse(sq, A, npad, ovl_h, ws, false);
            ws->ovl_h = ovl_h;
        }
        if (ws->part1_on_panel && ntl >= ws->tri_min_nt) {
            if (p > 0 && !uq) (void)hipStreamWaitEvent(sp, ws->ev_cols[p], 0);
            update_cols(sp, A, npad, K0, W, pcol(p + 1), pcol(p + 2), ws);
            factor_panel(sp, A, npad, pcol(p + 1), pcol(p + 2) - pcol(p + 1), ws);
            if (uq) continue;
            (void)hipStreamWaitEvent(su, ws->ev_panel[p], 0);
            if (!ws->agg2) {
                update_cols(su, A, npad, K0, W, pcol(p + 2), npad, ws);
                (void)hipEventRecord(ws->ev_cols[p + 1], su);
                continue;
            }
            if ((p & 1) == 0) {
                if (p + 2 < P) {
                    update_cols(su, A, npad, K0, W, pcol(p + 2), pcol(p + 3), ws);
                } else {
                    update_cols(su, A, npad, K0, W, pcol(p + 2), npad, ws);
                }
                (void)hipEventRecord(ws->ev_cols[p + 1], su);
            } else {
                const long K1 = pcol(p - 1), W2 = pcol(p + 1) - K1;
                update_cols(su, A, npad, K1, W2, pcol(p + 2), pcol(p + 3), ws);
                (void)hipEventRecord(ws->ev_cols[p + 1], su);
                update_cols(su, A, npad, K1, W2, pcol(p + 3), npad, ws);
            }
            continue;
        }
        (void)hipStreamWaitEvent(su, ws->ev_panel[p], 0);
        update_cols(su, A, npad, K0, W, pcol(p + 1), pcol(p + 2), ws);
        (void)hipEventRecord(ws->ev_cols[p + 1], su);
        (void)hipStreamWaitEvent(sp, ws->ev_cols[p + 1], 0);
        factor_panel(sp, A, npad, pcol(p + 1), pcol(p + 2) - pcol(p + 1), ws);
        update_cols(su, A, npad, K0, W, pcol(p + 2), npad, ws);
    }
    (void)hipEventRecord(ws->ev_panel[P], sp);
    (void)hipStreamWaitEvent(st, ws->ev_panel[P], 0);
}

void trtri_device(hipStream_t st, const double* L, double* X, double* T, long npad, FactorWs* ws) {
    const int nt = (int)(npad / NB);
    ws->prof.begin(st, PF_TRTRI, (double)npad * npad * npad / 3.0);
    const int h = ws->ovl_h;
    ws->ovl_h = 0;
    ws->evals_done += 1;
    ws->early_pending = 0;
    if (h > 0 && X == ws->scratchX && T == ws->scratchT && h < nt) {
        int lev = 0;
        while ((1 << lev) < h) ++lev;
        const long off = (long)h * NB * npad + (long)h * NB;
        launch_inv128(st, L + off, X + off, npad, nt - h, ws->dinv + (long)h * 8 * 256);
        for (int level = 0; level < lev; ++level) launch_trtri_level(st, L + off, X + off, T + off, npad, nt - h, level);
        if (nt > 2 * h) {
            const long off2 = (long)2 * h * NB * npad + (long)2 * h * NB;
            launch_trtri_level(st, L + off2, X + off2, T + off2, npad, nt - 2 * h, lev);
        }
        const int nt_pair = nt < 2 * h ? nt : 2 * h;
        (void)hipStreamWaitEvent(st, ws->ev_tri_lead, 0);
        launch_trtri_stage1_steal(st, L, X, T, npad, nt_pair, lev, ws->tri_counter, 512);
        (void)hipStreamWaitEvent(st, ws->ev_tri, 0);
        launch_trtri_level(st, L, X, T, npad, nt_pair, lev, 2);
        for (int level = lev + 1; (1 << level) < nt; ++level) launch_trtri_level(st, L, X, T, npad, nt, level);
    } else {
        if (h > 0) (void)hipStreamWaitEvent(st, ws->ev_tri, 0);
        launch_inv128(st, L, X, npad, nt, ws->dinv);
        for (int level = 0; (1 << level) < nt; ++level) launch_trtri_level(st, L, X, T, npad, nt, level);
    }
    ws->prof.end(st);
}

static bool lauum_plan_wanted(const FactorWs* ws, int nt) {
    return ws->lauum_split && nt <= (ws->lauum_split > 1 ? ws->lauum_split : LAUUM_SPLIT_MAX_NT) && (long)nt * NB > 1024;
}
static bool lauum_plan_build(FactorWs* ws, int nt) {
    std::vector<LauumItem> items;
    std::vector<LauumSum> sums;
    int nparts = 0;
    lauum_split_plan(nt, items, sums, &nparts);
    if (ws->lauum_plan_dev) (void)hipFree(ws->lauum_plan_dev);
    if (ws->lauum_part) (void)hipFree(ws->lauum_part);
    ws->lauum_plan_dev = nullptr;
    ws->lauum_part = nullptr;
    ws->lauum_plan_nt = 0;
    const size_t bi = sizeof(LauumItem) * items.size(), bs = sizeof(LauumSum) * sums.size();
    if (hipMalloc(&ws->lauum_plan_dev, bi + bs + 16) == hipSuccess &&
        hipMalloc(&ws->lauum_part, sizeof(double) * (size_t)lauum_split_tile(nt) * lauum_split_tile(nt) * (size_t)(nparts + 1)) ==
            hipSuccess) {
        (void)hipMemcpy(ws->lauum_plan_dev, items.data(), bi, hipMemcpyHostToDevice);
        if (bs) (void)hipMemcpy((char*)ws->lauum_plan_dev + bi, sums.data(), bs, hipMemcpyHostToDevice);
        ws->lauum_plan_nt = nt;
        ws->lauum_nitems = (int)items.size();
        ws->lauum_nsums = (int)sums.size();
        return true;
    }
    (void)hipGetLastError();
    return false;
}

void lauum_device(hipStream_t st, const double* X, double* W, long npad, FactorWs* ws) {
    const int nt = (int)(npad / NB);
    ws->prof.begin(st, PF_LAUUM, (double)npad * npad * npad / 3.0);
    bool split = lauum_plan_wanted(ws, nt);
    if (split && ws->lauum_plan_nt != nt) {
        hipStreamCaptureStatus cap = hipStreamCaptureStatusNone;
        if (hipStreamIsCapturing(st, &cap) != hipSuccess) (void)hipGetLastError();
        split = (cap == hipStreamCaptureStatusNone) && lauum_plan_build(ws, nt);
    }
    if (split && ws->lauum_plan_nt == nt)
        launch_lauum_split(st, X, W, npad, nt, (const LauumItem*)ws->lauum_plan_dev, ws->lauum_nitems,
                           (const LauumSum*)((const char*)ws->lauum_plan_dev + sizeof(LauumItem) * ws->lauum_nitems), ws->lauum_nsums,
                           ws->lauum_part);
    else
        launch_lauum(st, X, W, npad, nt);
    ws->prof.end(st);
}
```

### gpy_amd/csrc/gemm.hip

```cpp
#include "gemm_tile.h"
#include "internal.h"

#define LDS_OPT_IN(kernel)                                                                              \
    do {                                                                                                \
        static bool done = false;                                                                       \
        if (!done) {                                                                                    \
            (void)hipFuncSetAttribute(reinterpret_cast<const void*>(kernel),                            \
                                      hipFuncAttributeMaxDynamicSharedMemorySize, GT_LDS_BYTES);        \
            done = true;                                                                                \
        }                                                                                               \
    } while (0)

#include <algorithm>
#include <cstdlib>
#include <vector>
#define env_int(name, dflt) diag_env_int(DIAG_ENV(name), dflt)
#define LB(NW) __launch_bounds__((NW) * 64, (NW) / 2)

template <int NW, bool PRE>
__global__ LB(NW) void k_update_nt(double* __restrict__ C, long ldc,
                                                      const double* __restrict__ A, long lda,
                                                      const double* __restrict__ B, long ldb, int K, int ntc,
                                                      int row0t, int col0t, int tri, long ntiles) {
    extern __shared__ __attribute__((aligned(16))) double smem[];
    for (long bid = blockIdx.x; bid < ntiles; bid += gridDim.x) {
        int ti, tj;
        if (tri) {
            ti = (int)((sqrtf(8.0f * (float)bid + 1.0f) - 1.0f) * 0.5f);
            while ((long)ti * (ti + 1) / 2 > bid) --ti;
            while ((long)(ti + 1) * (ti + 2) / 2 <= bid) ++ti;
            tj = (int)(bid - (long)ti * (ti + 1) / 2);
        } else {
            ti = (int)(bid / ntc);
            tj = (int)(bid - (long)ti * ntc);
            if (col0t + tj > row0t + ti) continue;
        }
        d4 acc[4][GTCfg<NW>::NI];
        double* Ct = C + (long)ti * NB * ldc + (long)tj * NB;
        if (PRE) {
            gt_load_buf<NW>(Ct, ldc, acc);
            gemm_tile_128<true, true, NW, true>(A + (long)ti * NB * lda, lda, B + (long)tj * NB * ldb, ldb, K, acc, smem);
            gt_store<0, NW>(Ct, ldc, acc);
        } else {
            gt_zero<NW>(acc);
            gemm_tile_128<true, true, NW>(A + (long)ti * NB * lda, lda, B + (long)tj * NB * ldb, ldb, K, acc, smem);
            gt_store<2, NW>(Ct, ldc, acc);
        }
    }
}

__global__ __launch_bounds__(256) void k_update_nt64(double* __restrict__ C, long ldc, const double* __restrict__ A, long lda,
                                                     const double* __restrict__ B, long ldb, int K, int ntc, int row0t,
                                                     int col0t, int tri) {
    extern __shared__ __attribute__((aligned(16))) double smem[];
    const long bid = blockIdx.x >> 2;
    const int qi = (blockIdx.x >> 1) & 1, qj = blockIdx.x & 1;
    int ti, tj;
    if (tri) {
        ti = (int)((sqrtf(8.0f * (float)bid + 1.0f) - 1.0f) * 0.5f);
        while ((long)ti * (ti + 1) / 2 > bid) --ti;
        while ((long)(ti + 1) * (ti + 2) / 2 <= bid) ++ti;
        tj = (int)(bid - (long)ti * (ti + 1) / 2);
    } else {
        ti = (int)(bid / ntc);
        tj = (int)(bid - (long)ti * ntc);
        if (col0t + tj > row0t + ti) return;
    }
    d4 acc[2][2];
    double* Ct = C + ((long)ti * NB + qi * 64) * ldc + (long)tj * NB + qj * 64;
    gt64_load(Ct, ldc, acc);
    gemm_tile_64_v3<true, true, true>(A + ((long)ti * NB + qi * 64) * lda, lda, B + ((long)tj * NB + qj * 64) * ldb, ldb, K,
                                      acc, smem);
    gt64_store<0>(Ct, ldc, acc);
}

bool update_nt_uses_64(int ntr, int ntc, int row0t, int col0t) {
    static const int upd64_max = env_int("UPD64_MAX", GEMM_DEFAULT_UPD64_MAX);
    const int tri = (row0t == col0t && ntr == ntc) ? 1 : 0;
    const long nblocks = tri ? (long)ntr * (ntr + 1) / 2 : (long)ntr * ntc;
    return nblocks <= upd64_max;
}

void launch_update_nt(hipStream_t st, double* C, long ldc, const double* A, long lda, const double* B, long ldb,
                      int K, int ntr, int ntc, int row0t, int col0t) {
    if (ntr <= 0 || ntc <= 0) return;
    const int tri = (row0t == col0t && ntr == ntc) ? 1 : 0;
    const long nblocks = tri ? (long)ntr * (ntr + 1) / 2 : (long)ntr * ntc;
    if (update_nt_uses_64(ntr, ntc, row0t, col0t)) {
        hipLaunchKernelGGL(k_update_nt64, dim3((unsigned)(4 * nblocks)), dim3(256), GT64_LDS_BYTES, st, C, ldc, A, lda, B, ldb,
                           K, ntc, row0t, col0t, tri);
        return;
    }
    LDS_OPT_IN((k_update_nt<4, true>));
    hipLaunchKernelGGL((k_update_nt<4, true>), dim3((unsigned)nblocks), dim3(256), GT_LDS_BYTES, st, C, ldc, A, lda, B, ldb, K,
                       ntc, row0t, col0t, tri, nblocks);
}

#ifdef MI355GP_DIAG
__global__ LB(4) void k_update_nt_queue(double* __restrict__ A, long ld, const UpdTask* __restrict__ tasks, int ntasks,
                                        int* __restrict__ counter) {
    extern __shared__ __attribute__((aligned(16))) double smem[];
    __shared__ long s_tile;
    for (;;) {
        __syncthreads();
        if (threadIdx.x == 0) s_tile = (long)atomicAdd(counter, 1);
        __syncthreads();
        long bid = s_tile;
        int q = 0;
        while (q < ntasks && bid >= tasks[q].ntiles) bid -= tasks[q++].ntiles;
        if (q >= ntasks) return;
        const UpdTask tk = tasks[q];
        int ti = (int)((sqrtf(8.0f * (float)bid + 1.0f) - 1.0f) * 0.5f);
        while ((long)ti * (ti + 1) / 2 > bid) --ti;
        while ((long)(ti + 1) * (ti + 2) / 2 <= bid) ++ti;
        const int tj = (int)(bid - (long)ti * (ti + 1) / 2);
        d4 acc[4][GTCfg<4>::NI];
        double* Ct = A + tk.c_off + (long)ti * NB * ld + (long)tj * NB;
        const double* P = A + tk.p_off;
        gt_load_buf<4>(Ct, ld, acc);
        gemm_tile_128<true, true, 4, true>(P + (long)ti * NB * ld, ld, P + (long)tj * NB * ld, ld, tk.K, acc, smem);
        gt_store<0, 4>(Ct, ld, acc);
    }
}

void launch_update_nt_queue(hipStream_t st, double* A, long ld, const UpdTask* tasks_dev, int ntasks, int* counter, int wgs) {
    LDS_OPT_IN(k_update_nt_queue);
    hipLaunchKernelGGL(k_update_nt_queue, dim3((unsigned)wgs), dim3(256), GT_LDS_BYTES, st, A, ld, tasks_dev, ntasks, counter);
}
#endif

__host__ __device__ __forceinline__ int trtri_rows_last(int nt, int nbt) {
    const int pairs = (nt + 2 * nbt - 1) / (2 * nbt), right0 = (2 * (pairs - 1) + 1) * nbt;
    const int rows = nt - right0;
    return rows < 0 ? 0 : (rows > nbt ? nbt : rows);
}
__host__ __device__ __forceinline__ long trtri_level_tiles(int nt, int nbt) {
    const int pairs = (nt + 2 * nbt - 1) / (2 * nbt);
    return (long)(pairs - 1) * nbt * nbt + (long)nbt * trtri_rows_last(nt, nbt);
}
template <int STAGE>
__device__ __forceinline__ void trtri_map(int bid, int nt, int nbt, int& p, int& ri, int& cj) {
    const int per = nbt * nbt, pairs = (nt + 2 * nbt - 1) / (2 * nbt), full = (pairs - 1) * per;
    if (bid < full) {
        p = bid / per;
        const int rem = bid - p * per;
        if (STAGE == 1) {
            cj = rem / nbt;
            ri = rem - cj * nbt;
        } else {
            ri = nbt - 1 - rem / nbt;
            cj = rem % nbt;
        }
    } else {
        p = pairs - 1;
        const int rem = bid - full, rows = trtri_rows_last(nt, nbt);
        if (STAGE == 1) {
            cj = rem / rows;
            ri = rem - cj * rows;
        } else {
            ri = rows - 1 - rem / nbt;
            cj = rem % nbt;
        }
    }
}

template <int STAGE, int NW>
__device__ __forceinline__ void trtri_stage_tile(int bid, const double* __restrict__ L, double* __restrict__ X,
                                                 double* __restrict__ T, long ld, int nt, int nbt, double* smem) {
    int p, ri, cj;
    trtri_map<STAGE>(bid, nt, nbt, p, ri, cj);
    const int left0 = 2 * p * nbt, right0 = left0 + nbt;
    const int ti = right0 + ri, tj = left0 + cj;
    if (ti >= nt) return;
    d4 acc[4][GTCfg<NW>::NI];
    gt_zero<NW>(acc);
    if (STAGE == 1) {
        const int K = (right0 - tj) * NB;
        gemm_tile_128<true, false, NW>(L + (long)ti * NB * ld + (long)tj * NB, ld,
                                   X + (long)tj * NB * ld + (long)tj * NB, ld, K, acc, smem);
        gt_store<0, NW>(T + (long)ti * NB * ld + (long)tj * NB, ld, acc);
    } else {
        const int K = (ti - right0 + 1) * NB;
        gemm_tile_128<true, false, NW>(X + (long)ti * NB * ld + (long)right0 * NB, ld,
                                   T + (long)right0 * NB * ld + (long)tj * NB, ld, K, acc, smem);
        gt_store<1, NW>(X + (long)ti * NB * ld + (long)tj * NB, ld, acc);
    }
}

template <int STAGE>
__global__ __launch_bounds__(256) void k_trtri_stage64(const double* __restrict__ L, double* __restrict__ X,
                                                       double* __restrict__ T, long ld, int nt, int nbt) {
    extern __shared__ __attribute__((aligned(16))) double smem[];
    const int bid = blockIdx.x >> 2, qi = (blockIdx.x >> 1) & 1, qj = blockIdx.x & 1;
    int p, ri, cj;
    trtri_map<STAGE>(bid, nt, nbt, p, ri, cj);
    const int left0 = 2 * p * nbt, right0 = left0 + nbt;
    const int ti = right0 + ri, tj = left0 + cj;
    if (ti >= nt) return;
    d4 acc[2][2];
    gt64_zero(acc);
    const long r0 = (long)ti * NB + qi * 64, c0 = (long)tj * NB + qj * 64;
    if (STAGE == 1) {
        const int K = (right0 - tj) * NB;
        gemm_tile_64_v3<true, false>(L + r0 * ld + (long)tj * NB, ld, X + (long)tj * NB * ld + c0, ld, K, acc, smem);
        gt64_store<0>(T + r0 * ld + c0, ld, acc);
    } else {
        const int K = (ti - right0 + 1) * NB;
        gemm_tile_64_v3<true, false>(X + r0 * ld + (long)right0 * NB, ld, T + (long)right0 * NB * ld + c0, ld, K, acc, smem);
        gt64_store<1>(X + r0 * ld + c0, ld, acc);
    }
}

template <int STAGE, int NW>
__global__ LB(NW) void k_trtri_stage(const double* __restrict__ L, double* __restrict__ X,
                                                        double* __restrict__ T, long ld, int nt, int nbt) {
    extern __shared__ __attribute__((aligned(16))) double smem[];
    trtri_stage_tile<STAGE, NW>((int)blockIdx.x, L, X, T, ld, nt, nbt, smem);
}

__global__ LB(4) void k_trtri_stage1_steal(const double* __restrict__ L, double* __restrict__ X, double* __restrict__ T,
                                           long ld, int nt, int nbt, int* __restrict__ counter, int nblocks) {
    extern __shared__ __attribute__((aligned(16))) double smem[];
    __shared__ int s_bid;
    for (;;) {
        if (threadIdx.x == 0) s_bid = atomicAdd(counter, 1);
        __syncthreads();
        const int bid = s_bid;
        __syncthreads();
        if (bid >= nblocks) return;
        trtri_stage_tile<1, 4>(bid, L, X, T, ld, nt, nbt, smem);
    }
}

void launch_trtri_stage1_steal(hipStream_t st, const double* L, double* X, double* T, long ld, int nt, int level,
                               int* counter, int grid) {
    const int nbt = 1 << level;
    if (nbt >= nt) return;
    const int nblocks = (int)trtri_level_tiles(nt, nbt);
    if (nblocks <= 0) return;
    LDS_OPT_IN(k_trtri_stage1_steal);
    if (grid > nblocks) grid = nblocks;
    hipLaunchKernelGGL(k_trtri_stage1_steal, dim3((unsigned)grid), dim3(256), GT_LDS_BYTES, st, L, X, T, ld, nt, nbt,
                       counter, nblocks);
}

template <int NW>
static void launch_trtri_level_t(hipStream_t st, long nblocks, const double* L, double* X, double* T, long ld, int nt,
                                 int nbt, int stages) {
    LDS_OPT_IN((k_trtri_stage<1, NW>));
    LDS_OPT_IN((k_trtri_stage<2, NW>));
    if (stages & 1)
        hipLaunchKernelGGL((k_trtri_stage<1, NW>), dim3((unsigned)nblocks), dim3(NW * 64), GT_LDS_BYTES, st, L, X, T, ld, nt, nbt);
    if (stages & 2)
        hipLaunchKernelGGL((k_trtri_stage<2, NW>), dim3((unsigned)nblocks), dim3(NW * 64), GT_LDS_BYTES, st, L, X, T, ld, nt, nbt);
}

void launch_trtri_level(hipStream_t st, const double* L, double* X, double* T, long ld, int nt, int level, int stages) {
    const int nbt = 1 << level;
    if (nbt >= nt) return;
    const long nblocks = trtri_level_tiles(nt, nbt);
    if (nblocks <= 0) return;
    static const int tri64_max = env_int("TRI64_MAX", GEMM_DEFAULT_TRI64_MAX);
    if (nblocks <= tri64_max) {
        if (stages & 1)
            hipLaunchKernelGGL((k_trtri_stage64<1>), dim3((unsigned)(4 * nblocks)), dim3(256), GT64_LDS_BYTES, st, L, X, T, ld, nt, nbt);
        if (stages & 2)
            hipLaunchKernelGGL((k_trtri_stage64<2>), dim3((unsigned)(4 * nblocks)), dim3(256), GT64_LDS_BYTES, st, L, X, T, ld, nt, nbt);
        return;
    }
    launch_trtri_level_t<4>(st, nblocks, L, X, T, ld, nt, nbt, stages);
}

template <int NW>
__global__ LB(NW) void k_lauum(const double* __restrict__ X, double* __restrict__ W, long ld, int nt) {
    extern __shared__ __attribute__((aligned(16))) double smem[];
    const int bid = blockIdx.x;
    int ti = (int)((sqrtf(8.0f * (float)bid + 1.0f) - 1.0f) * 0.5f);
    while ((long)ti * (ti + 1) / 2 > bid) --ti;
    while ((long)(ti + 1) * (ti + 2) / 2 <= bid) ++ti;
    const int tj = bid - (int)((long)ti * (ti + 1) / 2);
    d4 acc[4][GTCfg<NW>::NI];
    gt_zero<NW>(acc);
    const int K = (nt - ti) * NB;
    gemm_tile_128<false, false, NW>(X + (long)ti * NB * ld + (long)ti * NB, ld, X + (long)ti * NB * ld + (long)tj * NB, ld,
                                K, acc, smem);
    gt_store<0, NW>(W + (long)ti * NB * ld + (long)tj * NB, ld, acc);
}

__global__ __launch_bounds__(256) void k_lauum64(const double* __restrict__ X, double* __restrict__ W, long ld, int nt) {
    extern __shared__ __attribute__((aligned(16))) double smem[];
    const int bid = blockIdx.x >> 2, qi = (blockIdx.x >> 1) & 1, qj = blockIdx.x & 1;
    int ti = (int)((sqrtf(8.0f * (float)bid + 1.0f) - 1.0f) * 0.5f);
    while ((long)ti * (ti + 1) / 2 > bid) --ti;
    while ((long)(ti + 1) * (ti + 2) / 2 <= bid) ++ti;
    const int tj = bid - (int)((long)ti * (ti + 1) / 2);
    d4 acc[2][2];
    gt64_zero(acc);
    const int K = (nt - ti) * NB;
    const long r0 = (long)ti * NB + qi * 64, c0 = (long)tj * NB + qj * 64;
    gemm_tile_64_v3<false, false>(X + (long)ti * NB * ld + r0, ld, X + (long)ti * NB * ld + c0, ld, K, acc, smem);
    gt64_store<0>(W + r0 * ld + c0, ld, acc);
}

#define LAUUM_KC 1024
#define LAUUM_T128_MIN_NT 24
static int lauum_kc_rows_128(int nt) {
    static const int forced = env_int("LAUUM_KC", 0);
    if (forced >= NB) return forced / NB * NB;
    int best = LAUUM_KC;
    double best_us = 1e30;
    for (int kc = 2; kc <= 32 && kc <= nt; ++kc) {
        std::vector<int> len;
        long parts = 0;
        for (int ti = 0; ti < nt; ++ti) {
            const int K = nt - ti, nch = (K + kc - 1) / kc;
            for (int tj = 0; tj <= ti; ++tj)
                for (int c = 0; c < nch; ++c) len.push_back(c + 1 < nch ? kc : K - c * kc);
            if (nch > 1) parts += (long)nch * (ti + 1);
        }
        std::sort(len.begin(), len.end(), [](int a, int b) { return a > b; });
        std::vector<double> slot(512, 0.0);
        std::make_heap(slot.begin(), slot.end(), [](double a, double b) { return a > b; });
        double end = 0.0;
        for (int l : len) {
            std::pop_heap(slot.begin(), slot.end(), [](double a, double b) { return a > b; });
            const double t = slot.back() + 27.4 * l + 8.0;
            slot.back() = t;
            if (t > end) end = t;
            std::push_heap(slot.begin(), slot.end(), [](double a, double b) { return a > b; });
        }
        const double us = end + (double)parts * (NB * NB * 8.0) / 3.0e6;
        if (us < best_us - 0.5) {
            best_us = us;
            best = kc * NB;
        }
    }
    return best;
}
__global__ __launch_bounds__(256) void k_lauum64_items(const double* __restrict__ X, double* __restrict__ W, long ld,
                                                       const LauumItem* __restrict__ items, double* __restrict__ part) {
    extern __shared__ __attribute__((aligned(16))) double smem[];
    const LauumItem it = items[blockIdx.x];
    d4 acc[2][2];
    gt64_zero(acc);
    const long r0 = (long)it.ti * NB + (it.q >> 1) * 64, c0 = (long)it.tj * NB + (it.q & 1) * 64;
    gemm_tile_64_v3<false, false>(X + (long)it.k0 * ld + r0, ld, X + (long)it.k0 * ld + c0, ld, it.klen, acc, smem);
    if (it.part < 0) gt64_store<0>(W + r0 * ld + c0, ld, acc);
    else gt64_store<0>(part + (long)it.part * 4096, 64, acc);
}

__global__ LB(4) void k_lauum128_items(const double* __restrict__ X, double* __restrict__ W, long ld,
                                       const LauumItem* __restrict__ items, double* __restrict__ part) {
    extern __shared__ __attribute__((aligned(16))) double smem[];
    const LauumItem it = items[blockIdx.x];
    d4 acc[4][GTCfg<4>::NI];
    gt_zero<4>(acc);
    const long r0 = (long)it.ti * NB, c0 = (long)it.tj * NB;
    gemm_tile_128<false, false, 4>(X + (long)it.k0 * ld + r0, ld, X + (long)it.k0 * ld + c0, ld, it.klen, acc, smem);
    if (it.part < 0) gt_store<0, 4>(W + r0 * ld + c0, ld, acc);
    else gt_store<0, 4>(part + (long)it.part * (NB * NB), NB, acc);
}

__global__ __launch_bounds__(256) void k_lauum128_reduce(double* __restrict__ W, long ld, const LauumSum* __restrict__ sums,
                                                         const double* __restrict__ part) {
    const LauumSum sm = sums[blockIdx.x];
    const long r0 = (long)sm.ti * NB, c0 = (long)sm.tj * NB;
    for (int e = threadIdx.x; e < NB * NB / 2; e += 256) {
        const int i = e >> 6, j = 2 * (e & 63);
        d2 s = *reinterpret_cast<const d2*>(part + (long)sm.first * (NB * NB) + i * NB + j);
        for (int c = 1; c < sm.n; ++c) s += *reinterpret_cast<const d2*>(part + (long)(sm.first + c) * (NB * NB) + i * NB + j);
        *reinterpret_cast<d2*>(W + (r0 + i) * ld + c0 + j) = s;
    }
}

__global__ __launch_bounds__(256) void k_lauum64_reduce(double* __restrict__ W, long ld, const LauumSum* __restrict__ sums,
                                                        const double* __restrict__ part) {
    const LauumSum sm = sums[blockIdx.x];
    const long r0 = (long)sm.ti * NB + (sm.q >> 1) * 64, c0 = (long)sm.tj * NB + (sm.q & 1) * 64;
    for (int e = threadIdx.x; e < 2048; e += 256) {
        const int i = e >> 5, j = 2 * (e & 31);
        d2 s = *reinterpret_cast<const d2*>(part + (long)sm.first * 4096 + i * 64 + j);
        for (int c = 1; c < sm.n; ++c) s += *reinterpret_cast<const d2*>(part + (long)(sm.first + c) * 4096 + i * 64 + j);
        *reinterpret_cast<d2*>(W + (r0 + i) * ld + c0 + j) = s;
    }
}

int lauum_split_tile(int nt) { return nt >= LAUUM_T128_MIN_NT ? 128 : 64; }

void lauum_split_plan(int nt, std::vector<LauumItem>& items, std::vector<LauumSum>& sums, int* nparts) {
    items.clear();
    sums.clear();
    int np = 0;
    const int nq = lauum_split_tile(nt) == 128 ? 1 : 4;
    static const int kc64 = env_int("LAUUM_KC64", 0) / NB * NB;
    const int kc = (nq == 1) ? lauum_kc_rows_128(nt) : (kc64 >= NB ? kc64 : (nt <= 16 ? 512 : LAUUM_KC));
    for (int ti = 0; ti < nt; ++ti)
        for (int tj = 0; tj <= ti; ++tj)
            for (int q = 0; q < nq; ++q) {
                const int k0 = ti * NB, K = (nt - ti) * NB, nch = (K + kc - 1) / kc;
                if (nch > 1) sums.push_back(LauumSum{ti, tj, q, np, nch});
                for (int c = 0; c < nch; ++c) {
                    const int len = (c + 1 < nch) ? kc : K - c * kc;
                    items.push_back(LauumItem{ti, tj, q, k0 + c * kc, len, nch > 1 ? np++ : -1});
                }
            }
    std::stable_sort(items.begin(), items.end(), [](const LauumItem& a, const LauumItem& b) { return a.klen > b.klen; });
    *nparts = np;
}

void launch_lauum_split(hipStream_t st, const double* X, double* W, long ld, int nt, const LauumItem* items_dev, int nitems,
                        const LauumSum* sums_dev, int nsums, double* part) {
    if (lauum_split_tile(nt) == 128) {
        LDS_OPT_IN(k_lauum128_items);
        hipLaunchKernelGGL(k_lauum128_items, dim3((unsigned)nitems), dim3(256), GT_LDS_BYTES, st, X, W, ld, items_dev, part);
        if (nsums > 0) hipLaunchKernelGGL(k_lauum128_reduce, dim3((unsigned)nsums), dim3(256), 0, st, W, ld, sums_dev, part);
        return;
    }
    hipLaunchKernelGGL(k_lauum64_items, dim3((unsigned)nitems), dim3(256), GT64_LDS_BYTES, st, X, W, ld, items_dev, part);
    if (nsums > 0) hipLaunchKernelGGL(k_lauum64_reduce, dim3((unsigned)nsums), dim3(256), 0, st, W, ld, sums_dev, part);
}

template <int NW>
static void launch_lauum_t(hipStream_t st, long nblocks, const double* X, double* W, long ld, int nt) {
    LDS_OPT_IN((k_lauum<NW>));
    hipLaunchKernelGGL((k_lauum<NW>), dim3((unsigned)nblocks), dim3(NW * 64), GT_LDS_BYTES, st, X, W, ld, nt);
}

bool lauum_uses_64(int nt) {
    static const int lauum64_max = env_int("LAUUM64_MAX", GEMM_DEFAULT_LAUUM64_MAX);
    return (long)nt * (nt + 1) / 2 <= lauum64_max;
}

void launch_lauum(hipStream_t st, const double* X, double* W, long ld, int nt) {
    const long nblocks = (long)nt * (nt + 1) / 2;
    static const int lauum64_max = env_int("LAUUM64_MAX", GEMM_DEFAULT_LAUUM64_MAX);
    if (nblocks <= lauum64_max) {
        hipLaunchKernelGGL(k_lauum64, dim3((unsigned)(4 * nblocks)), dim3(256), GT64_LDS_BYTES, st, X, W, ld, nt);
        return;
    }
    launch_lauum_t<4>(st, nblocks, X, W, ld, nt);
}

template <int NW>
__global__ LB(NW) void k_trmm_lower(const double* __restrict__ X, long ldx,
                                                       const double* __restrict__ B, long ldb,
                                                       double* __restrict__ Out, long ldo, int ntc) {
    extern __shared__ __attribute__((aligned(16))) double smem[];
    const int ti = (int)(gridDim.x / ntc) - 1 - (int)(blockIdx.x / ntc), tj = blockIdx.x % ntc;
    d4 acc[4][GTCfg<NW>::NI];
    gt_zero<NW>(acc);
    gemm_tile_128<true, false, NW>(X + (long)ti * NB * ldx, ldx, B + (long)tj * NB, ldb, (ti + 1) * NB, acc, smem);
    gt_store<0, NW>(Out + (long)ti * NB * ldo + (long)tj * NB, ldo, acc);
}

template <int NW>
__global__ LB(NW) void k_trmm_lower_T(const double* __restrict__ X, long ldx, const double* __restrict__ B, long ldb,
                                      double* __restrict__ Out, long ldo, int ntc, int nt) {
    extern __shared__ __attribute__((aligned(16))) double smem[];
    const int ti = blockIdx.x / ntc, tj = blockIdx.x % ntc;
    d4 acc[4][GTCfg<NW>::NI];
    gt_zero<NW>(acc);
    gemm_tile_128<false, false, NW>(X + (long)ti * NB * ldx + (long)ti * NB, ldx, B + (long)ti * NB * ldb + (long)tj * NB, ldb,
                                    (nt - ti) * NB, acc, smem);
    gt_store<0, NW>(Out + (long)ti * NB * ldo + (long)tj * NB, ldo, acc);
}

void launch_trmm_lower_T(hipStream_t st, const double* X, long ldx, const double* B, long ldb, double* Out, long ldo,
                         int ntr, int ntc) {
    LDS_OPT_IN((k_trmm_lower_T<4>));
    hipLaunchKernelGGL((k_trmm_lower_T<4>), dim3((unsigned)(ntr * ntc)), dim3(256), GT_LDS_BYTES, st, X, ldx, B, ldb, Out,
                       ldo, ntc, ntr);
}

template <int NW>
static void launch_trmm_lower_t(hipStream_t st, const double* X, long ldx, const double* B, long ldb, double* Out,
                                long ldo, int ntr, int ntc) {
    LDS_OPT_IN((k_trmm_lower<NW>));
    hipLaunchKernelGGL((k_trmm_lower<NW>), dim3((unsigned)(ntr * ntc)), dim3(NW * 64), GT_LDS_BYTES, st, X, ldx, B, ldb,
                       Out, ldo, ntc);
}

void launch_trmm_lower(hipStream_t st, const double* X, long ldx, const double* B, long ldb, double* Out, long ldo,
                       int ntr, int ntc) {
    launch_trmm_lower_t<4>(st, X, ldx, B, ldb, Out, ldo, ntr, ntc);
}

template <int MODE>
__global__ __launch_bounds__(256) void k_trmm64(const double* __restrict__ X, long ldx, const double* __restrict__ B, long ldb,
                                                double* __restrict__ Out, long ldo, int nt, int ntother, double alpha) {
    extern __shared__ __attribute__((aligned(16))) double smem[];
    const int q = blockIdx.x & 3, qi = q >> 1, qj = q & 1, bid = blockIdx.x >> 2;
    int ti, tj;
    if (MODE == 0) { ti = nt - 1 - bid / ntother; tj = bid % ntother; }
    else if (MODE == 1) { ti = bid / ntother; tj = bid % ntother; }
    else if (MODE == 2) { tj = nt - 1 - bid / ntother; ti = bid % ntother; }
    else { tj = bid / ntother; ti = bid % ntother; }
    const long r0 = (long)ti * NB + qi * 64, c0 = (long)tj * NB + qj * 64;
    d4 acc[2][2];
    gt64_zero(acc);
    if (MODE == 0) gemm_tile_64_v3<true, false>(X + r0 * ldx, ldx, B + c0, ldb, (ti + 1) * NB, acc, smem);
    else if (MODE == 1) gemm_tile_64_v3<false, false>(X + (long)ti * NB * ldx + r0, ldx, B + (long)ti * NB * ldb + c0, ldb, (nt - ti) * NB, acc, smem);
    else if (MODE == 2) gemm_tile_64_v3<true, true>(B + r0 * ldb, ldb, X + c0 * ldx, ldx, (tj + 1) * NB, acc, smem);
    else gemm_tile_64_v3<true, false>(B + r0 * ldb + (long)tj * NB, ldb, X + (long)tj * NB * ldx + c0, ldx, (nt - tj) * NB, acc, smem);
#pragma unroll
    for (int mi = 0; mi < 2; ++mi)
#pragma unroll
        for (int ni = 0; ni < 2; ++ni) acc[mi][ni] *= alpha;
    gt64_store<0>(Out + r0 * ldo + c0, ldo, acc);
}

void launch_trmm64(hipStream_t st, int mode, const double* X, long ldx, const double* B, long ldb, double* Out, long ldo, int nt,
                   int ntother, double alpha) {
    const unsigned grid = (unsigned)(4 * nt * ntother);
    switch (mode) {
        case 0: hipLaunchKernelGGL((k_trmm64<0>), dim3(grid), dim3(256), GT64_LDS_BYTES, st, X, ldx, B, ldb, Out, ldo, nt, ntother, alpha); break;
        case 1: hipLaunchKernelGGL((k_trmm64<1>), dim3(grid), dim3(256), GT64_LDS_BYTES, st, X, ldx, B, ldb, Out, ldo, nt, ntother, alpha); break;
        case 2: hipLaunchKernelGGL((k_trmm64<2>), dim3(grid), dim3(256), GT64_LDS_BYTES, st, X, ldx, B, ldb, Out, ldo, nt, ntother, alpha); break;
        default: hipLaunchKernelGGL((k_trmm64<3>), dim3(grid), dim3(256), GT64_LDS_BYTES, st, X, ldx, B, ldb, Out, ldo, nt, ntother, alpha); break;
    }
}

void launch_gemm_tn_sq(hipStream_t st, const double* A, long lda, long K, double* C, long ldc, int nt, double alpha,
                       double beta);

__device__ long long g_gemm_clk[2];

template <bool AK, bool BK, int NW>
__global__ LB(NW) void k_gemm_full(const double* __restrict__ A, long lda,
                                                      const double* __restrict__ B, long ldb, double* __restrict__ C,
                                                      long ldc, int K, int ntc, double alpha, double beta, int swz) {
    extern __shared__ __attribute__((aligned(16))) double smem[];
    int bid = blockIdx.x;
    if (swz & 1) {
        const int xcd = bid & 7, loc = bid >> 3;
        const int stiles = ntc >> 3;
        const int sidx = (loc >> 6) * 8 + xcd;
        const int in = loc & 63;
        bid = ((sidx / stiles) * 8 + (in >> 3)) * ntc + (sidx % stiles) * 8 + (in & 7);
    }
    const int ti = bid / ntc, tj = bid % ntc;
    d4 acc[4][GTCfg<NW>::NI];
    gt_zero<NW>(acc);
    const double* Ap = AK ? A + (long)ti * NB * lda : A + (long)ti * NB;
    const double* Bp = BK ? B + (long)tj * NB * ldb : B + (long)tj * NB;
    const long long c0 = clock64(), w0 = wall_clock64();
    gemm_tile_128<AK, BK, NW>(Ap, lda, Bp, ldb, K, acc, smem);
    if (blockIdx.x == 0 && threadIdx.x == 0) {
        g_gemm_clk[0] = clock64() - c0;
        g_gemm_clk[1] = wall_clock64() - w0;
    }
    double* Ct = C + (long)ti * NB * ldc + (long)tj * NB;
    if (beta == 0.0) {
#pragma unroll
        for (int mi = 0; mi < 4; ++mi)
#pragma unroll
            for (int ni = 0; ni < GTCfg<NW>::NI; ++ni) acc[mi][ni] *= alpha;
        gt_store<0, NW>(Ct, ldc, acc);
    } else {
        gt_store<3, NW>(Ct, ldc, acc, alpha, beta);
    }
}

template <bool AK, bool BK>
static void launch_gemm_full(hipStream_t st, unsigned nblocks, const double* A, long lda, const double* B, long ldb,
                             double* C, long ldc, int K, int ntc, double alpha, double beta) {
    static const int dbg_ld0 = env_int("DBG_LD0", 0), dbg_swz = env_int("DBG_SWZ", 0);
    if (dbg_ld0) lda = ldb = 0;
    static const int dbg_1wg = env_int("DBG_1WG", 0);
    const int swz = (dbg_swz && (ntc % 8 == 0) && ((nblocks / ntc) % 8 == 0)) ? 1 : 0;
    const size_t lds = dbg_1wg ? 100 * 1024 : GT_LDS_BYTES;
    (void)hipFuncSetAttribute(reinterpret_cast<const void*>(k_gemm_full<AK, BK, 4>),
                              hipFuncAttributeMaxDynamicSharedMemorySize, (int)lds);
    hipLaunchKernelGGL((k_gemm_full<AK, BK, 4>), dim3(nblocks), dim3(256), lds, st, A, lda, B, ldb, C, ldc, K,
                       ntc, alpha, beta, swz);
}

void launch_dbg_gemm(hipStream_t st, int a_mcontig, int b_ncontig, long M, long N, long K, const double* A,
                     const double* B, double* C, double alpha, double beta) {
    const int ntr = (int)(M / NB), ntc = (int)(N / NB);
    const unsigned grid = (unsigned)(ntr * ntc);
    const long lda = a_mcontig ? M : K, ldb = b_ncontig ? N : K;
    if (!a_mcontig && !b_ncontig) launch_gemm_full<true, true>(st, grid, A, lda, B, ldb, C, N, (int)K, ntc, alpha, beta);
    else if (!a_mcontig && b_ncontig) launch_gemm_full<true, false>(st, grid, A, lda, B, ldb, C, N, (int)K, ntc, alpha, beta);
    else if (a_mcontig && b_ncontig) launch_gemm_full<false, false>(st, grid, A, lda, B, ldb, C, N, (int)K, ntc, alpha, beta);
    else launch_gemm_full<false, true>(st, grid, A, lda, B, ldb, C, N, (int)K, ntc, alpha, beta);
}

void launch_gemm_tn_sq(hipStream_t st, const double* A, long lda, long K, double* C, long ldc, int nt, double alpha,
                       double beta) {
    launch_gemm_full<false, false>(st, (unsigned)(nt * nt), A, lda, A, lda, C, ldc, (int)K, nt, alpha, beta);
}

int gemm_last_clock(double* mhz, double* cycles) {
    long long h[2] = {0, 0};
    if (hipMemcpyFromSymbol(h, HIP_SYMBOL(g_gemm_clk), sizeof(h)) != hipSuccess) return -1;
    *mhz = h[1] > 0 ? (double)h[0] / (double)h[1] * 100.0 : 0.0;
    *cycles = (double)h[0];
    return 0;
}

void launch_gemm(hipStream_t st, int a_mcontig, int b_ncontig, long M, long N, long K, const double* A, long lda,
                 const double* B, long ldb, double* C, long ldc, double alpha, double beta) {
    const int ntr = (int)(M / NB), ntc = (int)(N / NB);
    const unsigned grid = (unsigned)(ntr * ntc);
    if (!a_mcontig && !b_ncontig) launch_gemm_full<true, true>(st, grid, A, lda, B, ldb, C, ldc, (int)K, ntc, alpha, beta);
    else if (!a_mcontig && b_ncontig) launch_gemm_full<true, false>(st, grid, A, lda, B, ldb, C, ldc, (int)K, ntc, alpha, beta);
    else if (a_mcontig && b_ncontig) launch_gemm_full<false, false>(st, grid, A, lda, B, ldb, C, ldc, (int)K, ntc, alpha, beta);
    else launch_gemm_full<false, true>(st, grid, A, lda, B, ldb, C, ldc, (int)K, ntc, alpha, beta);
}

__global__ __launch_bounds__(256, 2) void k_gram_splitk(const double* __restrict__ P, long ldp, long rows_per_split,
                                                        long mp, int ntl, int accumulate, double* __restrict__ part) {
    extern __shared__ __attribute__((aligned(16))) double smem[];
    const int s = blockIdx.x / ntl, bid = blockIdx.x % ntl;
    int ti = (int)((sqrtf(8.0f * (float)bid + 1.0f) - 1.0f) * 0.5f);
    while ((long)ti * (ti + 1) / 2 > bid) --ti;
    while ((long)(ti + 1) * (ti + 2) / 2 <= bid) ++ti;
    const int tj = bid - (int)((long)ti * (ti + 1) / 2);
    const double* Ps = P + (long)s * rows_per_split * ldp;
    d4 acc[4][4];
    gt_zero<4>(acc);
    gemm_tile_128<false, false, 4>(Ps + (long)ti * NB, ldp, Ps + (long)tj * NB, ldp, (int)rows_per_split, acc, smem);
    double* C = part + (long)s * mp * mp + (long)ti * NB * mp + (long)tj * NB;
    if (accumulate) gt_store<3, 4>(C, mp, acc, 1.0, 1.0);
    else gt_store<0, 4>(C, mp, acc);
}

void launch_gram_splitk(hipStream_t st, const double* P, long ldp, long rows, long mp, int S, int accumulate,
                        double* part) {
    LDS_OPT_IN(k_gram_splitk);
    const int nt = (int)(mp / NB), ntl = nt * (nt + 1) / 2;
    hipLaunchKernelGGL(k_gram_splitk, dim3((unsigned)(ntl * S)), dim3(256), GT_LDS_BYTES, st, P, ldp, rows / S, mp, ntl,
                       accumulate, part);
}
```

### gpy_amd/csrc/internal.h

```cpp
#pragma once
#include <shared_mutex>
#include <vector>

#include "common.h"

bool update_nt_uses_64(int ntr, int ntc, int row0t, int col0t);
struct UpdTask { long c_off, p_off, ntiles; int K, ntr; };
#ifdef MI355GP_DIAG
void launch_update_nt_queue(hipStream_t st, double* A, long ld, const UpdTask* tasks_dev, int ntasks, int* counter, int wgs);
#endif
void launch_update_nt(hipStream_t st, double* C, long ldc, const double* A, long lda, const double* B, long ldb,
                      int K, int ntr, int ntc, int row0t, int col0t);
void launch_trtri_level(hipStream_t st, const double* L, double* X, double* T, long ld, int nt, int level,
                        int stages = 3);
void launch_lauum(hipStream_t st, const double* X, double* W, long ld, int nt);
struct LauumItem { int ti, tj, q, k0, klen, part; };
struct LauumSum { int ti, tj, q, first, n; };
void lauum_split_plan(int nt, std::vector<LauumItem>& items, std::vector<LauumSum>& sums, int* nparts);
int lauum_split_tile(int nt);
void launch_lauum_split(hipStream_t st, const double* X, double* W, long ld, int nt, const LauumItem* items_dev, int nitems,
                        const LauumSum* sums_dev, int nsums, double* part);
bool lauum_uses_64(int nt);
void launch_trmm_lower(hipStream_t st, const double* X, long ldx, const double* B, long ldb, double* Out, long ldo,
                       int ntr, int ntc);
void launch_trmm_lower_T(hipStream_t st, const double* X, long ldx, const double* B, long ldb, double* Out, long ldo,
                         int ntr, int ntc);
void launch_trmm64(hipStream_t st, int mode, const double* X, long ldx, const double* B, long ldb, double* Out, long ldo, int nt,
                   int ntother, double alpha);
void launch_gemm_tn_sq(hipStream_t st, const double* A, long lda, long K, double* C, long ldc, int nt, double alpha,
                       double beta);
void launch_dbg_gemm(hipStream_t st, int a_mcontig, int b_ncontig, long M, long N, long K, const double* A,
                     const double* B, double* C, double alpha, double beta);

void launch_diag128(hipStream_t st, double* A, long ld, long c0, double* dinv, double* logsum, int* info,
                    int exclusive = 0);
void launch_trsm128(hipStream_t st, double* A, long ld, long c0, long r0, long mrows, const double* dinv);
void launch_trtri_stage1_steal(hipStream_t st, const double* L, double* X, double* T, long ld, int nt, int level,
                               int* counter, int grid);
void launch_inv128(hipStream_t st, const double* L, double* X, long ld, int nblk, const double* dinv_all);
void launch_dbg_mfma(hipStream_t st, const double* a, const double* b, double* d);

enum { PF_UPDATE = 0, PF_TRTRI = 1, PF_LAUUM = 2, PF_DIAG = 3, PF_TRSM = 4, PF_UPDATE64 = 5, PF_PERSIST = 6, PF_TRTRI_EARLY = 7, PF_NUM = 8 };
struct KernelProf {
    unsigned mask = 0;
    bool on = false;
    std::vector<hipEvent_t> pool;
    struct Rec { int fam; double flops; size_t e0; };
    std::vector<Rec> recs;
    bool open = false;
    void begin(hipStream_t st, int fam, double flops);
    void end(hipStream_t st);
    void reset() { recs.clear(); }
    int collect(double* ms, double* flops, int* launches);
    void destroy();
};

struct FactorWs {
    double* dinv = nullptr;
    double* logsum = nullptr;
    int* info = nullptr;
    long nblk = 0;
    hipStream_t st_panel = nullptr;
    std::vector<hipEvent_t> ev_panel;
    std::vector<hipEvent_t> ev_cols;
    hipEvent_t ev_fork = nullptr;
    hipEvent_t ev_early_pre = nullptr;
    int agg2 = 0;
    int persist_auto = 1, sched_state = 0, sched_force_steps = 0, persist_auto_off = 0;
    int sched_np = 0, sched_ns = 0;
    int can_calibrate = 0;
    float sched_ms_persist = 0.f, sched_ms_steps = 0.f;
    int evals_done = 0;
    int early_pending = 0;
    int lauum_split = 1, lauum_plan_nt = 0, lauum_nitems = 0, lauum_nsums = 0;
    void* lauum_plan_dev = nullptr;
    double* lauum_part = nullptr;
    int persist_tri = 1;
    int persist_tri_min_nt = 16;
    int upd_queue_probe = 0;
    UpdTask* upd_tasks = nullptr;
    int part1_on_panel = 1;
    int lookahead = 1;
    int nbo_override = 0;
    long nbo_for(long npad) const {
        long w = nbo_override > 0 ? nbo_override : (npad <= FACTOR_NBO_SMALL_N ? FACTOR_NBO_SMALL : NBO);
        w = (w / NB) * NB;
        return w < NB ? NB : w;
    }
    double* scratchX = nullptr;
    double* scratchT = nullptr;
    int tri_overlap = FACTOR_DEFAULT_TRI_OVERLAP, tri_cu_pct = 75, tri_min_nt = 48, tri_wgs = 0, ovl_h = 0;
    hipStream_t st_tri = nullptr, st_tri_half = nullptr, st_tri_cur = nullptr;
    int tri_half_ok = 1, tri_cur_pct = 75;
    hipEvent_t ev_tri = nullptr, ev_tri_lead = nullptr;
    int* tri_counter = nullptr;
    int tri_h_override = 0;
    int diag_excl_first = FACTOR_DEFAULT_DIAG_EXCL_FIRST, excl_first_ok = 0;
    int solve_overlap = 1;
    int persist = FACTOR_DEFAULT_PERSIST, persist_max_nt = FACTOR_PERSIST_MAX_NT, persist_kcap = 2, persist_cus = 0;
    int persist_skip = 0, persist_aborts = 0, persist_used = 0;
    hipEvent_t ev_persist_pre = nullptr;
    int persist_grid_last = 0;
    int persist_tune = 0;
    int persist_test = 0;
    int* persist_sync = nullptr;
    double* persist_hs = nullptr;
    KernelProf prof;
};
std::shared_mutex& engine_gate(int device);
struct EngineShared {
    std::shared_mutex* m;
    bool shared = true;
    explicit EngineShared(int device) : m(&engine_gate(device)) { m->lock_shared(); }
    EngineShared(const EngineShared&) = delete;
    EngineShared& operator=(const EngineShared&) = delete;
    ~EngineShared() {
        if (shared) m->unlock_shared();
        else m->unlock();
    }
    bool try_exclusive() {
        m->unlock_shared();
        if (m->try_lock()) {
            shared = false;
            return true;
        }
        m->lock_shared();
        return false;
    }
    void share() {
        m->unlock();
        m->lock_shared();
        shared = true;
    }
};
int factor_engine(int device, hipStream_t* main, hipStream_t* panel, hipStream_t* tri, hipStream_t* tri_half = nullptr);
int factor_ws_alloc(FactorWs* ws, long npad);
void factor_ws_free(FactorWs* ws);
template <int N>
struct MI355GP_LOCAL WorkspaceGuard {
    FactorWs ws;
    hipEvent_t ev[N] = {};
    ~WorkspaceGuard() {
        factor_ws_free(&ws);
        for (hipEvent_t e : ev)
            if (e) (void)hipEventDestroy(e);
    }
    int create_events() {
        for (hipEvent_t& e : ev) HIP_CHECK(hipEventCreate(&e));
        return 0;
    }
};
MI355GP_LOCAL void calibrate_schedule(FactorWs& w, float ms, int nt);
void potrf_device(hipStream_t st, double* A, long npad, FactorWs* ws);
void trtri_device(hipStream_t st, const double* L, double* X, double* T, long npad, FactorWs* ws);
void lauum_device(hipStream_t st, const double* X, double* W, long npad, FactorWs* ws);

bool potrf_persist_eligible(long npad, const FactorWs* ws);
int persist_box_verdict(int set = -2);
bool potrf_persist_aborted(int info, FactorWs* ws, bool* clean);
int potrf_persist_sync_ints();
bool launch_potrf_persist(hipStream_t st, double* A, long npad, FactorWs* ws, long long* dbg = nullptr);
void launch_wait_persist_resident(hipStream_t st, const FactorWs* ws, int timeout_ms = 2);
int persist_early_h(long npad, const FactorWs* ws);
void launch_wait_persist_rows(hipStream_t st, const FactorWs* ws, int r0, int r1, int cols, int give_up = 0);

#define GP_STRIDE 34
struct KernParams {
    int kind;
    int ard;
    int D;
    double variance;
    double power = 0.0;
    const double* pw = nullptr;
    int col = 0;
    double bias = 0.0;
};
void launch_scale_inputs(hipStream_t st, const double* X, long n, int D, const double* inv_ls, int ard,
                         double* Xt, long ldx);
void launch_kbuild_sym(hipStream_t st, KernParams kp, const double* Xt, long ldx, long n, long npad, double* A,
                       const double* noise, long noise_len, double jit, int lower_only, int add_diag,
                       int accumulate = 0, const double* mul = nullptr);
struct MI355GP_LOCAL SyntheticSpd {
    long n = 0, np = 0;
    DevBuf dX, dXt, dIl, dNoise;
    int init(hipStream_t st, long N);
    void build(hipStream_t st, double* A) const;
};
void launch_kbuild_cross(hipStream_t st, KernParams kp, const double* Xt1, long ld1, long n, const double* Xt2,
                         long ld2, long m, double* Kout, long ldk, int accumulate = 0, int diag_same = 0,
                         const double* mul = nullptr);
int launch_kbuild_cols(hipStream_t st, KernParams kp, const double* Xt1, long ld1, long n, const double* Xt2, long ld2, long m,
                       long mcols, double* Kout, long ldk, const double* V, int Dy, double* colpart);
void launch_tri_matvec(hipStream_t st, const double* X, long ld, long n, const double* R, int Dy, double* tmp,
                       double* alpha, double* partials);
struct GradOut {
    double* partials;
    int stride;
    int nblocks;
};
int grad_num_blocks(long n);
void launch_grad_fused(hipStream_t st, KernParams kp, const double* Xt, long ldx, long n, const double* W,
                       long ldw, const double* alpha, int Dy, double* partials,
                       const double* aa_scale = nullptr, const double* Mul = nullptr, long ldm = 0);
struct RankTerm {
    const double* Y;
    const double* V;
    int Dy;
    double beta, gscale;
    const double* rowscale = nullptr;
};
int launch_grad_cols(hipStream_t st, KernParams kp, const double* Xt1, long ld1, long n, const double* Xt2, long ld2,
                     long m, long mcols, const double* G, long ldg, RankTerm rk, double* partials, double* colpart,
                     int* nblocks_out);
void launch_studentt_scale(hipStream_t st, const double* scal, double nu, long n, double* out);
void launch_grad_generic(hipStream_t st, KernParams kp, const double* Xt1, long ld1, long n, const double* Xt2,
                         long ld2, long m, int symmetric, const double* G, long ldg, double* partials,
                         double* Hout = nullptr, long ldh = 0,
                         RankTerm rk = RankTerm{nullptr, nullptr, 0, 0.0, 1.0, nullptr});
void launch_periodic_gradx(hipStream_t st, KernParams kp, const double* Xt1, long ld1, long n, const double* Xt2, long ld2,
                           long m, const double* W, long ldw, int wt, double* out);
int launch_grad_coreg(hipStream_t st, bool fused, KernParams kp, const double* Xt1, long ld1, long n, const double* Xt2, long ld2,
                      long m, const double* G, long ldg, const double* alpha, int Dy, double* partials,
                      const double* aa_scale = nullptr, const double* Mul = nullptr, long ldm = 0);
void launch_col_reduce_vec(hipStream_t st, const double* M, long ld, long rows, long cols, const double* kd, double* out);
int launch_colreduce_multi(hipStream_t st, const double* M, long ld, long rows, long cols, const double* V, long sr,
                           long sc, int nvt, int ones, double* part);
void launch_sum_splits(hipStream_t st, const double* src, long cnt, int nsplit, int accumulate, double* dst);
int trmv_chunk_rows(long n);
void launch_trmv_lower(hipStream_t st, const double* X, long ld, long n, const double* R, int Dy, double* y);
void launch_trmv_lower_T(hipStream_t st, const double* X, long ld, long n, const double* y, int Dy, double* out,
                         double* partials);
int gemm_last_clock(double* mhz, double* cycles);
void launch_gemm(hipStream_t st, int a_mcontig, int b_ncontig, long M, long N, long K, const double* A, long lda,
                 const double* B, long ldb, double* C, long ldc, double alpha, double beta);
void launch_gram_splitk(hipStream_t st, const double* P, long ldp, long rows, long mp, int S, int accumulate,
                        double* part);
int grad_generic_num_blocks(long n, long m);
void launch_reduce_partials(hipStream_t st, const double* partials, int nblocks, int stride, double* out);
void launch_scalars(hipStream_t st, const double* alpha, const double* R, const double* W, long ldw, long n,
                    int Dy, const double* logsum, long nblk, double* out4, double* diag_out, const int* info = nullptr);
void launch_extract(hipStream_t st, const double* A, long ld, long n, int mode, const double* alpha, int Dy,
                    double* out, int transpose, const double* aa_scale = nullptr);
void launch_pad_from_dense(hipStream_t st, const double* src, long n, double* A, long npad, const double* noise,
                           long noise_len, double jit);
void launch_col_reduce(hipStream_t st, const double* M, long ld, long rows, long cols, const double* v, int Dy,
                       double c0, int mode, double* out);

void launch_rowdots(hipStream_t st, const double* K, const double* T, long ld, long rows, long m, const double* v, int Dy,
                    double* out_s, double* t_out);
void launch_rowscale_sqrt(hipStream_t st, const double* M, long ld, long rows, long cols, const double* w, double* Out);

void launch_laplace_B(hipStream_t st, const double* K, long npad, long n, const double* sw, double jit, double* A);
size_t symv_part_doubles(long npad);
void launch_symv_lower(hipStream_t st, const double* K, long npad, long n, const double* v0, const double* v1, double* y0,
                       double* y1, double* part);
void launch_laplace_dLdK(hipStream_t st, const double* Binv, long npad, long n, const double* sw, const double* a,
                         const double* u, double* G);

int rccl_comm_create(int rank, int world, const void* id128, void** comm);
int rccl_allreduce_sum(void* comm, double* buf, size_t count, hipStream_t st);
void rccl_comm_destroy(void* comm);
```

### include/mi355gp.h

```cpp
#ifndef MI355GP_H
#define MI355GP_H

#include <stdint.h>

#ifdef __cplusplus
extern "C" {
#endif

typedef struct mi355gp_ctx mi355gp_ctx;

enum { MI355GP_RBF = 0, MI355GP_MATERN52 = 1, MI355GP_MATERN32 = 2, MI355GP_EXPONENTIAL = 3,
       MI355GP_WHITE = 4, MI355GP_BIAS = 5 ,
       MI355GP_RATQUAD = 6, MI355GP_STDPERIODIC = 7, MI355GP_COREGIONALIZE = 8, MI355GP_LINEAR = 9,
       MI355GP_MLP = 10, MI355GP_POLY = 11, MI355GP_COSINE = 12, MI355GP_SINC = 13, MI355GP_EXPQUADCOSINE = 14 };






typedef struct {
    int kind;
    int ard;
    int n_active;
    const int* active_dims;
    const double* theta;
    int term;
} mi355gp_part;

enum {
    MI355GP_FETCH_L = 0,
    MI355GP_FETCH_KINV = 1,
    MI355GP_FETCH_DLDK = 2,
    MI355GP_FETCH_K = 3
};

enum {
    MI355GP_OUT_LML = 0,
    MI355GP_OUT_LOGDET = 1,
    MI355GP_OUT_DATAFIT = 2,
    MI355GP_OUT_DNOISE = 3,
    MI355GP_OUT_TRKINV = 4,
    MI355GP_NUM_OUT = 8
};

enum {
    MI355GP_T_KBUILD = 0, MI355GP_T_POTRF = 1, MI355GP_T_TRTRI = 2, MI355GP_T_LAUUM = 3,
    MI355GP_T_SOLVE = 4, MI355GP_T_GRAD = 5, MI355GP_T_TOTAL = 6, MI355GP_NUM_T = 8
};

const char* mi355gp_last_error(void);
const char* mi355gp_version(void);
int mi355gp_device_count(int* count);
int mi355gp_device_synchronize(int device);

int mi355gp_create(int device, mi355gp_ctx** ctx);
int mi355gp_destroy(mi355gp_ctx* ctx);

int mi355gp_set_data(mi355gp_ctx* ctx, const double* X, int64_t N, int D, const double* R, int Dy);
int mi355gp_set_targets(mi355gp_ctx* ctx, const double* R, int Dy);

int mi355gp_kern_K(int device, int kind, int ard, const double* theta, const double* X, int64_t N,
                   const double* X2, int64_t M, int D, double* K_out);
int mi355gp_kern_Kdiag(int kind, const double* theta, int64_t N, double* out);
int mi355gp_update_gradients_full(int device, int kind, int ard, const double* theta, const double* dL_dK,
                                  const double* X, int64_t N, const double* X2, int64_t M, int D,
                                  double* dtheta_out);

int mi355gp_gradients_X(int device, int kind, int ard, const double* theta, const double* dL_dK, const double* X,
                        int64_t N, const double* X2, int64_t M, int D, double* out);

int mi355gp_exact_inference(mi355gp_ctx* ctx, int kind, int ard, const double* theta,
                            const double* noise, int64_t noise_len, double jitter, double extra_jitter,
                            double* out_scalars, double* alpha_out, double* dtheta_out,
                            double* diag_dLdK_out, double* stage_ms);

int mi355gp_exact_inference_sum(mi355gp_ctx* ctx, int nparts, const mi355gp_part* parts, const double* noise,
                                int64_t noise_len, double jitter, double extra_jitter, double* out_scalars,
                                double* alpha_out, double* dtheta_out, double* diag_dLdK_out, double* stage_ms);

int mi355gp_exact_studentt_sum(mi355gp_ctx* ctx, int nparts, const mi355gp_part* parts, double nu, double jitter,
                               double extra_jitter, double* out_scalars, double* alpha_out, double* dtheta_out,
                               double* stage_ms);

int mi355gp_inference_given_K(mi355gp_ctx* ctx, const double* K_host, const double* noise, int64_t noise_len,
                              double jitter, double extra_jitter, double* out_scalars, double* alpha_out,
                              double* diag_dLdK_out, double* stage_ms);

int mi355gp_fetch(mi355gp_ctx* ctx, int which, double* out, int fortran_order);

int mi355gp_predict(mi355gp_ctx* ctx, int kind, int ard, const double* theta, const double* Xnew, int64_t M,
                    double* mu_out, double* var_out, int full_cov);

int mi355gp_predict_sum(mi355gp_ctx* ctx, int nparts, const mi355gp_part* parts, const double* Xnew, int64_t M,
                        double* mu_out, double* var_out, int full_cov);

int mi355gp_predictive_gradients_sum(mi355gp_ctx* ctx, int nparts, const mi355gp_part* parts, const double* Xnew, int64_t M,
                                     double* dmu_out, double* dvar_out);

int mi355gp_laplace_begin(mi355gp_ctx* ctx, int nparts, const mi355gp_part* parts);
int mi355gp_laplace_newton(mi355gp_ctx* ctx, const double* W, const double* b, double extra_jitter, double* a_out,
                           double* Ka_out, double* logdet_out);
int mi355gp_laplace_finish(mi355gp_ctx* ctx, const double* W, double extra_jitter, double* diagKiWi_out, double* logdet_out);
int mi355gp_laplace_gradients(mi355gp_ctx* ctx, const double* Ki_f, const double* dL_dfhat, double* dtheta_out);
int mi355gp_laplace_implicit(mi355gp_ctx* ctx, const double* dL_dfhat, double* s_out);
int mi355gp_laplace_predict(mi355gp_ctx* ctx, int nparts, const mi355gp_part* parts, const double* Xnew, int64_t M,
                            const double* wv, double* mu_out, double* var_out, int full_cov);

enum { MI355GP_EP_BERNOULLI_PROBIT = 0 };
int mi355gp_ep_recompute(mi355gp_ctx* ctx, const double* tau, const double* v, double extra_jitter, double add_diag,
                         int want_sigma, double* mu_out, double* sigdiag_out, double* logdet_out, double* ms_out);
int mi355gp_ep_sweep(mi355gp_ctx* ctx, int lik, const int64_t* order, const double* ysign, double eta, double delta, double* tau,
                     double* v, double* cav_tau_out, double* cav_v_out, double* logZhat_out, double* mu_out, double* sigdiag_out,
                     double* ms_out);

int mi355gp_covariance_between_points(mi355gp_ctx* ctx, int nparts, const mi355gp_part* parts, const double* X1,
                                      int64_t M1, const double* X2, int64_t M2, double* out);

int mi355gp_potrf(int device, double* A, int64_t N, double* ms);
int mi355gp_pdinv(int device, const double* A, int64_t N, double* Ainv, double* L_out, double* logdet, double* ms);
int mi355gp_pdinv_full(int device, const double* A, int64_t N, double* Ainv, double* L_out, double* Li_out, double* logdet,
                       double* ms);

enum { MI355GP_OPT_PROFILE = 0, MI355GP_OPT_LOOKAHEAD = 1, MI355GP_OPT_TRI_OVERLAP = 2, MI355GP_OPT_TRI_MIN_NT = 3,
       MI355GP_OPT_TRI_H = 4, MI355GP_OPT_TRI_WGS = 5, MI355GP_OPT_TRI_HALF = 6, MI355GP_OPT_PART1_ON_PANEL = 7,
       MI355GP_OPT_NBO = 8, MI355GP_OPT_SOLVE_OVERLAP = 9, MI355GP_OPT_DIAG_EXCL_FIRST = 10, MI355GP_OPT_GRAPH = 11,
       MI355GP_OPT_PERSIST = 12, MI355GP_OPT_AGG2 = 13, MI355GP_OPT_PERSIST_TEST = 14, MI355GP_OPT_PERSIST_ABORTS = 15,
       MI355GP_OPT_PERSIST_SKIP = 16, MI355GP_OPT_PERSIST_SCHED = 17, MI355GP_OPT_NUM = 18 };
int mi355gp_set_option(mi355gp_ctx* ctx, int option, int value);
int mi355gp_get_option(mi355gp_ctx* ctx, int option, int* value);
enum { MI355GP_PF_UPDATE = 0 , MI355GP_PF_TRTRI = 1, MI355GP_PF_LAUUM = 2,
       MI355GP_PF_DIAG = 3 , MI355GP_PF_TRSM = 4 ,
       MI355GP_PF_UPDATE64 = 5 ,
       MI355GP_PF_PERSIST = 6 ,
       MI355GP_PF_TRTRI_EARLY = 7 ,
       MI355GP_PF_NUM = 8 };
int mi355gp_get_profile(mi355gp_ctx* ctx, double* ms, double* flops, int* launches);

typedef struct mi355gp_grid mi355gp_grid;
int mi355gp_grid_unique_id(void* id128);
int mi355gp_grid_create(int device, int rank, int world, int Pr, int Pc, int nb, const void* id128, mi355gp_grid** out);
int mi355gp_grid_destroy(mi355gp_grid* g);
int mi355gp_grid_set_data(mi355gp_grid* g, const double* X, int64_t N, int D, const double* R, int Dy);
int mi355gp_grid_exact_inference(mi355gp_grid* g, int kind, int ard, const double* theta, const double* noise,
                                 int64_t noise_len, double jitter, double extra_jitter, double* out_scalars,
                                 double* alpha_out, double* dtheta_out, double* diag_dLdK_out, double* stage_ms);
#define MI355GP_FETCH_LINV 100
int mi355gp_grid_fetch(mi355gp_grid* g, int which, double* out);
enum { MI355GP_GRID_OPT_LOOKAHEAD = 0, MI355GP_GRID_OPT_G = 1, MI355GP_GRID_OPT_GW = 2, MI355GP_GRID_OPT_CHECK_SEQ = 3,
       MI355GP_GRID_OPT_NUM = 4 };
int mi355gp_grid_set_option(mi355gp_grid* g, int option, int value);
int mi355gp_grid_get_option(mi355gp_grid* g, int option, int* value);
int mi355gp_grid_coll_log(mi355gp_grid* g, int rank, double* out9);
typedef struct mi355gp_sparse mi355gp_sparse;
int mi355gp_sparse_create(int device, mi355gp_sparse** out);
int mi355gp_sparse_destroy(mi355gp_sparse* s);
int mi355gp_sparse_set_data(mi355gp_sparse* s, const double* X, int64_t N, int D, const double* Y, int Dy);
int mi355gp_vardtc_inference(mi355gp_sparse* s, int kind, int ard, const double* theta, const double* Z, int64_t M,
                             double noise_var, double extra_jitter, double* out_scalars, double* dtheta_out,
                             double* dZ_out, double* wv_out, double* stage_ms);
int mi355gp_vardtc_inference_sum(mi355gp_sparse* s, int nparts, const mi355gp_part* parts, const double* Z, int64_t M,
                                 const double* noise, int64_t noise_len, double extra_jitter, double* out_scalars,
                                 double* dtheta_out, double* dZ_out, double* wv_out, double* dnoise_rows_out,
                                 double* dLdm_out, double* stage_ms);
int mi355gp_sparse_set_input_variance(mi355gp_sparse* s, const double* S, int64_t N, int D);
int mi355gp_sparse_set_inputs(mi355gp_sparse* s, const double* X, const double* S, int64_t N, int D);
int mi355gp_vardtc_inference_uncertain(mi355gp_sparse* s, int nparts, const mi355gp_part* parts, const double* Z, int64_t M,
                                       const double* noise, int64_t noise_len, double extra_jitter, double* out_scalars,
                                       double* dtheta_out, double* dZ_out, double* wv_out, double* dmu_out, double* dS_out,
                                       double* stage_ms);
int mi355gp_sparse_predict(mi355gp_sparse* s, int nparts, const mi355gp_part* parts, const double* Xnew, int64_t Mn,
                           double* mu_out, double* var_out, int full_cov);
int mi355gp_sparse_predict_uncertain(mi355gp_sparse* s, int nparts, const mi355gp_part* parts, const double* mu_new,
                                     const double* S_new, int64_t Mn, double* mean_out, double* var_out);
int mi355gp_sparse_get_predict_ms(mi355gp_sparse* s, double* ms_out);
int mi355gp_sparse_fetch_dLdKnm(mi355gp_sparse* s, int64_t row0, int64_t nrows, double* out);
int mi355gp_sparse_attach_comm(mi355gp_sparse* s, int rank, int world, const void* id128);
int mi355gp_sparse_attach_loopback(mi355gp_sparse* s, int rank, int world, int group_key);
int mi355gp_sparse_fetch(mi355gp_sparse* s, int which, double* out);
int mi355gp_sparse_get_profile(mi355gp_sparse* s, double* out6);

int mi355gp_svgp_forward(mi355gp_sparse* s, int nparts, const mi355gp_part* parts, const double* Z, int64_t M, const double* q_mean,
                         const double* q_chol, int L, double extra_jitter, double* mu_out, double* v_out, double* scalars_out,
                         double* stage_ms);
int mi355gp_svgp_backward(mi355gp_sparse* s, const double* dF_dmu, const double* dF_dv, double* dtheta_out, double* dZ_out,
                          double* dm_out, double* dchol_out, double* stage_ms);
int mi355gp_svgp_predict(mi355gp_sparse* s, int nparts, const mi355gp_part* parts, const double* Xnew, int64_t Mn, int full_cov,
                         double* mu_out, double* var_out, double* wv_out, double* winv_out);

int mi355gp_pep_inference(mi355gp_sparse* s, int nparts, const mi355gp_part* parts, const double* Z, int64_t M,
                          double noise_variance, double alpha, double jitter, double* out_scalars, double* dtheta_out,
                          double* dZ_out, double* wv_out, double* dLdR_out, double* stage_ms);
int mi355gp_pep_check_sigma(const double* sigma, int64_t n, int64_t row0, double noise_variance, double alpha);

int mi355gp_rbf_psi(int device, double variance, const double* lengthscale, int ard, const double* Z, int64_t M,
                    const double* mu, const double* S, int64_t N, int D, const double* weights, double* psi1_out,
                    double* psi2_out);
int mi355gp_rbf_psi_grad(int device, double variance, const double* lengthscale, int ard, const double* Z, int64_t M,
                         const double* mu, const double* S, int64_t N, int D, const double* weights, const double* dL_dpsi0,
                         const double* dL_dpsi1, const double* dL_dpsi2, double* dvar_out, double* dl_out, double* dZ_out,
                         double* dmu_out, double* dS_out);

#ifdef __cplusplus
}
#endif
#endif
```

Baseline: 13.87 iters/s.

## Add host-planned super-block tile ordering queues for update, trtri and lauum kernels

Adds a tile-ordering scheme in which the host builds a plan that groups output tiles into super-blocks and spreads them over eight balanced queues. Persistent workgroups (two per CU) then pull tiles from device counters instead of using the linear block-id order. The aim is better cache locality, and per XCD in the lauum kernel, plus load balancing across the triangular update, trtri and lauum kernels. By default only the LAUUM family is enabled, and only above a tile-count threshold. This adds plan allocation, counter memsets and atomic queue overhead.

```diff
diff --git a/gpy_amd/_lib.py b/gpy_amd/_lib.py
--- a/gpy_amd/_lib.py
+++ b/gpy_amd/_lib.py
@@ -194,7 +194,7 @@
 
 OPTIONS = {"profile": 0, "lookahead": 1, "tri_overlap": 2, "tri_min_nt": 3, "tri_h": 4, "tri_wgs": 5, "tri_half": 6,
            "part1_on_panel": 7, "nbo": 8, "solve_overlap": 9, "diag_excl_first": 10, "graph": 11, "persist": 12, "agg2": 13,
-           "persist_test": 14, "persist_aborts": 15, "persist_skip": 16, "persist_sched": 17}
+           "persist_test": 14, "persist_aborts": 15, "persist_skip": 16, "persist_sched": 17, "tile_order": 18}
 
 
 def last_error():
diff --git a/gpy_amd/csrc/api.hip b/gpy_amd/csrc/api.hip
--- a/gpy_amd/csrc/api.hip
+++ b/gpy_amd/csrc/api.hip
@@ -32,6 +32,7 @@
     set(MI355GP_OPT_DIAG_EXCL_FIRST, &w.diag_excl_first);
     set(MI355GP_OPT_PERSIST, &w.persist);
     set(MI355GP_OPT_AGG2, &w.agg2);
+    set(MI355GP_OPT_TILE_ORDER, &w.tile_order);
     if (c->opt[MI355GP_OPT_GRAPH] != INT_MIN) c->graph_enabled = c->opt[MI355GP_OPT_GRAPH] ? 1 : 0;
 }
 
@@ -316,6 +317,7 @@
         return -1;
     }
     if (option == MI355GP_OPT_LOOKAHEAD) value = (value == 0) ? 0 : 1;
+    if (option == MI355GP_OPT_TILE_ORDER && value > 0) value = 1;
     if (option == MI355GP_OPT_NBO && value > 0 && value % NB != 0) {
         mi355gp_set_error("mi355gp_set_option: NBO must be a multiple of %d", NB);
         return -1;
@@ -338,6 +340,7 @@
             case MI355GP_OPT_DIAG_EXCL_FIRST: c->ws.diag_excl_first = env("DIAG_EXCL_FIRST", d.diag_excl_first) ? 1 : 0; break;
             case MI355GP_OPT_PERSIST: c->ws.persist = penv("PERSIST", d.persist); break;
             case MI355GP_OPT_AGG2: c->ws.agg2 = env("AGG2", d.agg2) ? 1 : 0; break;
+            case MI355GP_OPT_TILE_ORDER: c->ws.tile_order = d.tile_order; break;
             case MI355GP_OPT_GRAPH: c->graph_enabled = penv("GRAPH", 1) ? 1 : 0; break;
             default: break;
         }
@@ -361,7 +364,7 @@
     const int v[MI355GP_OPT_NUM] = {0, w.lookahead, w.tri_overlap, w.tri_min_nt, w.tri_h_override, w.tri_wgs, w.tri_half_ok,
                                     w.part1_on_panel, w.nbo_override, w.solve_overlap, w.diag_excl_first, c->graph_enabled,
                                     w.persist, w.agg2, w.persist_test, w.persist_aborts, w.persist_skip,
-                                    w.sched_state == 2 ? ((w.persist_auto_off || !w.persist) ? 2 : 1) : 0};
+                                    w.sched_state == 2 ? ((w.persist_auto_off || !w.persist) ? 2 : 1) : 0, w.tile_order};
     *value = v[option];
     return 0;
 }
diff --git a/gpy_amd/csrc/common.h b/gpy_amd/csrc/common.h
--- a/gpy_amd/csrc/common.h
+++ b/gpy_amd/csrc/common.h
@@ -19,6 +19,12 @@
 #define GEMM_DEFAULT_TRI64_MAX 512
 #define GEMM_DEFAULT_LAUUM64_MAX 528
 #define LAUUM_SPLIT_MAX_NT 44
+#define TILE_ORDER_DEFAULT_FAMILIES 0x8
+#define TILE_ORDER_MIN_TILES_UPDATE 512
+#define TILE_ORDER_MIN_TILES_TRTRI 512
+#define TILE_ORDER_MIN_TILES_LAUUM 8192
+#define TILE_ORDER_SB_ROWS 8
+#define TILE_ORDER_SB_COLS 8
 #define GEMM_DEFAULT_UPD64_MAX 128
 
 __device__ __forceinline__ d4 mfma_f64(double a, double b, d4 c) {
diff --git a/gpy_amd/csrc/factor.hip b/gpy_amd/csrc/factor.hip
--- a/gpy_amd/csrc/factor.hip
+++ b/gpy_amd/csrc/factor.hip
@@ -3,6 +3,7 @@
 #include <vector>
 
 #include "internal.h"
+#include "tile_plan.h"
 
 void KernelProf::begin(hipStream_t st, int fam, double flops) {
     open = on && ((mask >> fam) & 1u);
@@ -114,6 +115,85 @@
     return 0;
 }
 
+enum { TQ_FAM_UPDATE = 0, TQ_FAM_TRTRI1 = 1, TQ_FAM_TRTRI2 = 2, TQ_FAM_LAUUM = 3 };
+enum { TQ_DRV_POTRF = 0, TQ_DRV_PANEL = 1, TQ_DRV_EARLY = 2, TQ_DRV_TRTRI = 3, TQ_DRV_LAUUM = 4, TQ_DRV_NUM = 5 };
+static const int tq_drv_first[TQ_DRV_NUM + 1] = {0, 128, 448, 464, 528, 532};
+static const int tq_min_tiles[4] = {TILE_ORDER_MIN_TILES_UPDATE, TILE_ORDER_MIN_TILES_TRTRI, TILE_ORDER_MIN_TILES_TRTRI,
+                                    TILE_ORDER_MIN_TILES_LAUUM};
+
+static int* tq_plan_build(int fam, int a, int b, int c) {
+    static const int sb = diag_env_int(DIAG_ENV("TILE_ORDER_SB"), TILE_ORDER_SB_ROWS * 100 + TILE_ORDER_SB_COLS);
+    const int sbr = sb / 100 > 0 ? sb / 100 : 1, sbc = sb % 100 > 0 ? sb % 100 : 1;
+    std::vector<TilePlanItem> items;
+    if (fam == TQ_FAM_UPDATE) tile_items_update(a, b, c >> 1, c & 1, sbr, sbc, items);
+    else if (fam == TQ_FAM_TRTRI1) tile_items_trtri<1>(a, b, sbr, sbc, items);
+    else if (fam == TQ_FAM_TRTRI2) tile_items_trtri<2>(a, b, sbr, sbc, items);
+    else tile_items_lauum(a, sbr, sbc, items);
+    TilePlan plan;
+    tile_plan_build(items, plan);
+    std::vector<int> host(TQ_HDR + plan.order.size(), 0);
+    for (int q = 0; q <= TP_NQ; ++q) host[q] = plan.qoff[q];
+    std::copy(plan.order.begin(), plan.order.end(), host.begin() + TQ_HDR);
+    int* dev = nullptr;
+    if (hipMalloc(&dev, sizeof(int) * host.size()) != hipSuccess ||
+        hipMemcpy(dev, host.data(), sizeof(int) * host.size(), hipMemcpyHostToDevice) != hipSuccess) {
+        (void)hipGetLastError();
+        if (dev) (void)hipFree(dev);
+        return nullptr;
+    }
+    return dev;
+}
+
+static TileQueue tile_queue(FactorWs* ws, hipStream_t st, int drv, int fam, int a, int b, int c, long tiles, int wgs_cap = 0) {
+    TileQueue tq;
+    const int fams = ws->tile_order < 0 ? ws->tq_default_fams : (ws->tile_order ? 0xf : 0);
+    if (!((fams >> fam) & 1) || !ws->tq_cnt || tiles <= ws->tq_wgs) return tq;
+    if (ws->tile_order < 0 && tiles <= tq_min_tiles[fam]) return tq;
+    const int sets = tq_drv_first[drv + 1] - tq_drv_first[drv];
+    if (ws->tq_next[drv] >= sets) return tq;
+    int* dev = nullptr;
+    for (const FactorWs::TqPlan& p : ws->tq_plans)
+        if (p.fam == fam && p.a == a && p.b == b && p.c == c) dev = p.dev;
+    if (!dev) {
+        hipStreamCaptureStatus cap = hipStreamCaptureStatusNone;
+        if (hipStreamIsCapturing(st, &cap) != hipSuccess) (void)hipGetLastError();
+        if (cap != hipStreamCaptureStatusNone || !(dev = tq_plan_build(fam, a, b, c))) return tq;
+        ws->tq_plans.push_back(FactorWs::TqPlan{fam, a, b, c, dev});
+    }
+    if (ws->tq_next[drv] < 0) {
+        (void)hipMemsetAsync(ws->tq_cnt + (size_t)tq_drv_first[drv] * TP_NQ, 0, sizeof(int) * TP_NQ * sets, st);
+        ws->tq_next[drv] = 0;
+    }
+    tq.plan = dev;
+    tq.cnt = ws->tq_cnt + (size_t)(tq_drv_first[drv] + ws->tq_next[drv]++) * TP_NQ;
+    tq.wgs = (wgs_cap > 0 && wgs_cap < ws->tq_wgs) ? wgs_cap : ws->tq_wgs;
+    tq.tiles = (int)tiles;
+    return tq;
+}
+
+static TileQueue update_queue(FactorWs* ws, hipStream_t st, int ntr, int ntc, int row0t, int col0t) {
+    if (ntr <= 0 || ntc <= 0 || update_nt_uses_64(ntr, ntc, row0t, col0t)) return TileQueue();
+    const int tri = (row0t == col0t && ntr == ntc) ? 1 : 0, delta = row0t - col0t;
+    long live = 0;
+    for (int ti = 0; ti < ntr; ++ti) live += (delta + ti + 1 < ntc ? (delta + ti + 1 > 0 ? delta + ti + 1 : 0) : ntc);
+    return tile_queue(ws, st, st == ws->st_panel ? TQ_DRV_PANEL : TQ_DRV_POTRF, TQ_FAM_UPDATE, ntr, ntc, delta * 2 + tri, live);
+}
+
+static void trtri_queues(FactorWs* ws, hipStream_t st, int drv, int nt, int level, int stages, TileQueue* tq1, TileQueue* tq2,
+                         int wgs_cap = 0) {
+    const int nbt = 1 << level;
+    if (nbt >= nt || trtri_level_uses_64(nt, level)) return;
+    const long tiles = trtri_level_tiles(nt, nbt);
+    if (stages & 1) *tq1 = tile_queue(ws, st, drv, TQ_FAM_TRTRI1, nt, nbt, 0, tiles, wgs_cap);
+    if (stages & 2) *tq2 = tile_queue(ws, st, drv, TQ_FAM_TRTRI2, nt, nbt, 0, tiles, wgs_cap);
+}
+static void trtri_level_ordered(FactorWs* ws, hipStream_t st, int drv, const double* L, double* X, double* T, long ld, int nt,
+                                int level, int stages = 3, int wgs_cap = 0) {
+    TileQueue tq1, tq2;
+    trtri_queues(ws, st, drv, nt, level, stages, &tq1, &tq2, wgs_cap);
+    launch_trtri_level(st, L, X, T, ld, nt, level, stages, tq1, tq2);
+}
+
 static bool lauum_plan_wanted(const FactorWs* ws, int nt);
 static bool lauum_plan_build(FactorWs* ws, int nt);
 int factor_ws_alloc(FactorWs* ws, long npad) {
@@ -182,6 +262,9 @@
         ws->persist_cus = prop.multiProcessorCount;
         const char* envpc = DIAG_ENV("PERSIST_WGS");
         if (envpc && *envpc && atoi(envpc) >= 2 && atoi(envpc) <= ws->persist_cus) ws->persist_cus = atoi(envpc);
+        ws->tq_wgs = 2 * prop.multiProcessorCount;
+        ws->tq_default_fams = diag_env_int(DIAG_ENV("TILE_ORDER"), TILE_ORDER_DEFAULT_FAMILIES) & 0xf;
+        HIP_CHECK(hipMalloc(&ws->tq_cnt, sizeof(int) * TP_NQ * tq_drv_first[TQ_DRV_NUM]));
         HIP_CHECK(hipMalloc(&ws->persist_sync, sizeof(int) * potrf_persist_sync_ints()));
         HIP_CHECK(hipMalloc(&ws->persist_hs, sizeof(double) * (size_t)(ws->nblk < 64 ? ws->nblk : 64) * NB * NB));
     }
@@ -230,6 +313,11 @@
     if (ws->lauum_part) (void)hipFree(ws->lauum_part);
     ws->lauum_part = nullptr;
     ws->lauum_plan_nt = 0;
+    for (const FactorWs::TqPlan& p : ws->tq_plans) (void)hipFree(p.dev);
+    ws->tq_plans.clear();
+    if (ws->tq_cnt) (void)hipFree(ws->tq_cnt);
+    ws->tq_cnt = nullptr;
+    ws->tq_steal = TileQueue();
     if (ws->persist_sync) (void)hipFree(ws->persist_sync);
     ws->persist_sync = nullptr;
     if (ws->persist_hs) (void)hipFree(ws->persist_hs);
@@ -259,7 +347,8 @@
         const double* P = A + cd * ld + c;
         ws->prof.begin(s, update_nt_uses_64((int)(below / NB), (int)(ncols / NB), (int)(cd / NB), (int)(cd / NB)) ? PF_UPDATE64 : PF_UPDATE,
                        syrk_flops((double)ncols, (double)NB) + gemm_flops((double)(below - ncols), (double)ncols, (double)NB));
-        launch_update_nt(s, A + cd * ld + cd, ld, P, ld, P, ld, NB, (int)(below / NB), (int)(ncols / NB), (int)(cd / NB), (int)(cd / NB));
+        launch_update_nt(s, A + cd * ld + cd, ld, P, ld, P, ld, NB, (int)(below / NB), (int)(ncols / NB), (int)(cd / NB), (int)(cd / NB),
+                         update_queue(ws, s, (int)(below / NB), (int)(ncols / NB), (int)(cd / NB), (int)(cd / NB)));
         ws->prof.end(s);
     }
 }
@@ -271,7 +360,7 @@
     ws->prof.begin(s, update_nt_uses_64((int)(rows / NB), (int)(cols / NB), (int)(c0 / NB), (int)(c0 / NB)) ? PF_UPDATE64 : PF_UPDATE,
                    syrk_flops((double)cols, (double)W) + gemm_flops((double)(rows - cols), (double)cols, (double)W));
     launch_update_nt(s, A + c0 * ld + c0, ld, P, ld, P, ld, (int)W, (int)(rows / NB), (int)(cols / NB), (int)(c0 / NB),
-                     (int)(c0 / NB));
+                     (int)(c0 / NB), update_queue(ws, s, (int)(rows / NB), (int)(cols / NB), (int)(c0 / NB), (int)(c0 / NB)));
     ws->prof.end(s);
 }
 
@@ -293,12 +382,17 @@
     ws->prof.begin(sq, PF_TRTRI_EARLY, 0.0);
     launch_inv128(sq, A, ws->scratchX, npad, h, ws->dinv);
     int level = 0;
-    for (; (1 << level) < h; ++level) launch_trtri_level(sq, A, ws->scratchX, ws->scratchT, npad, h, level);
+    const int side_wgs = ws->tri_wgs > 0 ? ws->tri_wgs : 512 * ws->tri_cur_pct / 100;
+    for (; (1 << level) < h; ++level)
+        trtri_level_ordered(ws, sq, TQ_DRV_EARLY, A, ws->scratchX, ws->scratchT, npad, h, level, 3, side_wgs);
     (void)hipEventRecord(ws->ev_tri_lead, sq);
     const int nt_pair = ntl < 2 * h ? ntl : 2 * h;
     if (gated) launch_wait_persist_rows(sq, ws, h, nt_pair, h);
-    launch_trtri_stage1_steal(sq, A, ws->scratchX, ws->scratchT, npad, nt_pair, level, ws->tri_counter,
-                              ws->tri_wgs > 0 ? ws->tri_wgs : 512 * ws->tri_cur_pct / 100);
+    {
+        TileQueue none;
+        trtri_queues(ws, sq, TQ_DRV_EARLY, nt_pair, level, 1, &ws->tq_steal, &none);
+    }
+    launch_trtri_stage1_steal(sq, A, ws->scratchX, ws->scratchT, npad, nt_pair, level, ws->tri_counter, side_wgs, ws->tq_steal);
     ws->prof.end(sq);
     (void)hipEventRecord(ws->ev_tri, sq);
     ws->early_pending = 1;
@@ -342,6 +436,8 @@
     }
     ws->ovl_h = 0;
     ws->persist_used = 0;
+    ws->tq_next[TQ_DRV_POTRF] = ws->tq_next[TQ_DRV_PANEL] = ws->tq_next[TQ_DRV_EARLY] = -1;
+    ws->tq_steal = TileQueue();
     if (potrf_persist_eligible(npad, ws)) {
         const int h = persist_early_h(npad, ws);
         const int gate_gives_up = (ws->persist_test == 3) ? 1 : 0;
@@ -476,27 +572,30 @@
     ws->ovl_h = 0;
     ws->evals_done += 1;
     ws->early_pending = 0;
+    ws->tq_next[TQ_DRV_TRTRI] = -1;
     if (h > 0 && X == ws->scratchX && T == ws->scratchT && h < nt) {
         int lev = 0;
         while ((1 << lev) < h) ++lev;
         const long off = (long)h * NB * npad + (long)h * NB;
         launch_inv128(st, L + off, X + off, npad, nt - h, ws->dinv + (long)h * 8 * 256);
-        for (int level = 0; level < lev; ++level) launch_trtri_level(st, L + off, X + off, T + off, npad, nt - h, level);
+        for (int level = 0; level < lev; ++level)
+            trtri_level_ordered(ws, st, TQ_DRV_TRTRI, L + off, X + off, T + off, npad, nt - h, level);
         if (nt > 2 * h) {
             const long off2 = (long)2 * h * NB * npad + (long)2 * h * NB;
-            launch_trtri_level(st, L + off2, X + off2, T + off2, npad, nt - 2 * h, lev);
+            trtri_level_ordered(ws, st, TQ_DRV_TRTRI, L + off2, X + off2, T + off2, npad, nt - 2 * h, lev);
         }
         const int nt_pair = nt < 2 * h ? nt : 2 * h;
         (void)hipStreamWaitEvent(st, ws->ev_tri_lead, 0);
-        launch_trtri_stage1_steal(st, L, X, T, npad, nt_pair, lev, ws->tri_counter, 512);
+        launch_trtri_stage1_steal(st, L, X, T, npad, nt_pair, lev, ws->tri_counter, 512, ws->tq_steal);
         (void)hipStreamWaitEvent(st, ws->ev_tri, 0);
-        launch_trtri_level(st, L, X, T, npad, nt_pair, lev, 2);
-        for (int level = lev + 1; (1 << level) < nt; ++level) launch_trtri_level(st, L, X, T, npad, nt, level);
+        trtri_level_ordered(ws, st, TQ_DRV_TRTRI, L, X, T, npad, nt_pair, lev, 2);
+        for (int level = lev + 1; (1 << level) < nt; ++level) trtri_level_ordered(ws, st, TQ_DRV_TRTRI, L, X, T, npad, nt, level);
     } else {
         if (h > 0) (void)hipStreamWaitEvent(st, ws->ev_tri, 0);
         launch_inv128(st, L, X, npad, nt, ws->dinv);
-        for (int level = 0; (1 << level) < nt; ++level) launch_trtri_level(st, L, X, T, npad, nt, level);
-    }
+        for (int level = 0; (1 << level) < nt; ++level) trtri_level_ordered(ws, st, TQ_DRV_TRTRI, L, X, T, npad, nt, level);
+    }
+    ws->tq_steal = TileQueue();
     ws->prof.end(st);
 }
 
@@ -541,7 +640,10 @@
         launch_lauum_split(st, X, W, npad, nt, (const LauumItem*)ws->lauum_plan_dev, ws->lauum_nitems,
                            (const LauumSum*)((const char*)ws->lauum_plan_dev + sizeof(LauumItem) * ws->lauum_nitems), ws->lauum_nsums,
                            ws->lauum_part);
-    else
-        launch_lauum(st, X, W, npad, nt);
+    else {
+        ws->tq_next[TQ_DRV_LAUUM] = -1;
+        launch_lauum(st, X, W, npad, nt,
+                     lauum_uses_64(nt) ? TileQueue() : tile_queue(ws, st, TQ_DRV_LAUUM, TQ_FAM_LAUUM, nt, 0, 0, (long)nt * (nt + 1) / 2));
+    }
     ws->prof.end(st);
 }
diff --git a/gpy_amd/csrc/gemm.hip b/gpy_amd/csrc/gemm.hip
--- a/gpy_amd/csrc/gemm.hip
+++ b/gpy_amd/csrc/gemm.hip
@@ -1,5 +1,6 @@
 #include "gemm_tile.h"
 #include "internal.h"
+#include "tile_plan.h"
 
 #define LDS_OPT_IN(kernel)                                                                              \
     do {                                                                                                \
@@ -18,35 +19,85 @@
 #define LB(NW) __launch_bounds__((NW) * 64, (NW) / 2)
 
 template <int NW, bool PRE>
+__device__ __forceinline__ void update_nt_tile(long bid, double* __restrict__ C, long ldc, const double* __restrict__ A, long lda,
+                                               const double* __restrict__ B, long ldb, int K, int ntc, int row0t, int col0t,
+                                               int tri, double* smem) {
+    int ti, tj;
+    if (tri) {
+        ti = (int)((sqrtf(8.0f * (float)bid + 1.0f) - 1.0f) * 0.5f);
+        while ((long)ti * (ti + 1) / 2 > bid) --ti;
+        while ((long)(ti + 1) * (ti + 2) / 2 <= bid) ++ti;
+        tj = (int)(bid - (long)ti * (ti + 1) / 2);
+    } else {
+        ti = (int)(bid / ntc);
+        tj = (int)(bid - (long)ti * ntc);
+        if (col0t + tj > row0t + ti) return;
+    }
+    d4 acc[4][GTCfg<NW>::NI];
+    double* Ct = C + (long)ti * NB * ldc + (long)tj * NB;
+    if (PRE) {
+        gt_load_buf<NW>(Ct, ldc, acc);
+        gemm_tile_128<true, true, NW, true>(A + (long)ti * NB * lda, lda, B + (long)tj * NB * ldb, ldb, K, acc, smem);
+        gt_store<0, NW>(Ct, ldc, acc);
+    } else {
+        gt_zero<NW>(acc);
+        gemm_tile_128<true, true, NW>(A + (long)ti * NB * lda, lda, B + (long)tj * NB * ldb, ldb, K, acc, smem);
+        gt_store<2, NW>(Ct, ldc, acc);
+    }
+}
+
+template <int NW, bool PRE>
 __global__ LB(NW) void k_update_nt(double* __restrict__ C, long ldc,
                                                       const double* __restrict__ A, long lda,
                                                       const double* __restrict__ B, long ldb, int K, int ntc,
                                                       int row0t, int col0t, int tri, long ntiles) {
     extern __shared__ __attribute__((aligned(16))) double smem[];
-    for (long bid = blockIdx.x; bid < ntiles; bid += gridDim.x) {
-        int ti, tj;
-        if (tri) {
-            ti = (int)((sqrtf(8.0f * (float)bid + 1.0f) - 1.0f) * 0.5f);
-            while ((long)ti * (ti + 1) / 2 > bid) --ti;
-            while ((long)(ti + 1) * (ti + 2) / 2 <= bid) ++ti;
-            tj = (int)(bid - (long)ti * (ti + 1) / 2);
-        } else {
-            ti = (int)(bid / ntc);
-            tj = (int)(bid - (long)ti * ntc);
-            if (col0t + tj > row0t + ti) continue;
+    for (long bid = blockIdx.x; bid < ntiles; bid += gridDim.x)
+        update_nt_tile<NW, PRE>(bid, C, ldc, A, lda, B, ldb, K, ntc, row0t, col0t, tri, smem);
+}
+
+__device__ __forceinline__ int xcc_id() { return __builtin_amdgcn_s_getreg((3 << 11) | (0 << 6) | 20) & (TP_NQ - 1); }
+
+__device__ __forceinline__ int tq_pop(const int* __restrict__ plan, int* __restrict__ cnt, int& q) {
+    for (;;) {
+        const int first = plan[q], n = plan[q + 1] - first;
+        if (n > 0) {
+            const int i = atomicAdd(cnt + q, 1);
+            if (i < n) return plan[TQ_HDR + first + i];
         }
-        d4 acc[4][GTCfg<NW>::NI];
-        double* Ct = C + (long)ti * NB * ldc + (long)tj * NB;
-        if (PRE) {
-            gt_load_buf<NW>(Ct, ldc, acc);
-            gemm_tile_128<true, true, NW, true>(A + (long)ti * NB * lda, lda, B + (long)tj * NB * ldb, ldb, K, acc, smem);
-            gt_store<0, NW>(Ct, ldc, acc);
-        } else {
-            gt_zero<NW>(acc);
-            gemm_tile_128<true, true, NW>(A + (long)ti * NB * lda, lda, B + (long)tj * NB * ldb, ldb, K, acc, smem);
-            gt_store<2, NW>(Ct, ldc, acc);
+        int most = 0, at = -1;
+        for (int k = 0; k < TP_NQ; ++k) {
+            const int left = plan[k + 1] - plan[k] - __hip_atomic_load(cnt + k, __ATOMIC_RELAXED, __HIP_MEMORY_SCOPE_AGENT);
+            if (left > most) {
+                most = left;
+                at = k;
+            }
         }
-    }
+        if (at < 0) return -1;
+        q = at;
+    }
+}
+
+template <bool ONCE, class Tile>
+__device__ __forceinline__ void tq_drain(const int* __restrict__ plan, int* __restrict__ cnt, Tile tile) {
+    __shared__ int s_bid;
+    int q = xcc_id();
+    for (;;) {
+        if (threadIdx.x == 0) s_bid = tq_pop(plan, cnt, q);
+        __syncthreads();
+        const int bid = s_bid;
+        __syncthreads();
+        if (bid < 0) return;
+        tile(bid);
+        if (ONCE) return;
+    }
+}
+
+__global__ LB(4) void k_update_nt_xcd(double* __restrict__ C, long ldc, const double* __restrict__ A, long lda,
+                                      const double* __restrict__ B, long ldb, int K, int ntc, int row0t, int col0t, int tri,
+                                      const int* __restrict__ plan, int* __restrict__ cnt) {
+    extern __shared__ __attribute__((aligned(16))) double smem[];
+    tq_drain<true>(plan, cnt, [&](int bid) { update_nt_tile<4, true>(bid, C, ldc, A, lda, B, ldb, K, ntc, row0t, col0t, tri, smem); });
 }
 
 __global__ __launch_bounds__(256) void k_update_nt64(double* __restrict__ C, long ldc, const double* __restrict__ A, long lda,
@@ -82,13 +133,19 @@
 }
 
 void launch_update_nt(hipStream_t st, double* C, long ldc, const double* A, long lda, const double* B, long ldb,
-                      int K, int ntr, int ntc, int row0t, int col0t) {
+                      int K, int ntr, int ntc, int row0t, int col0t, TileQueue tq) {
     if (ntr <= 0 || ntc <= 0) return;
     const int tri = (row0t == col0t && ntr == ntc) ? 1 : 0;
     const long nblocks = tri ? (long)ntr * (ntr + 1) / 2 : (long)ntr * ntc;
     if (update_nt_uses_64(ntr, ntc, row0t, col0t)) {
         hipLaunchKernelGGL(k_update_nt64, dim3((unsigned)(4 * nblocks)), dim3(256), GT64_LDS_BYTES, st, C, ldc, A, lda, B, ldb,
                            K, ntc, row0t, col0t, tri);
+        return;
+    }
+    if (tq.plan) {
+        LDS_OPT_IN(k_update_nt_xcd);
+        hipLaunchKernelGGL(k_update_nt_xcd, dim3((unsigned)tq.tiles), dim3(256), GT_LDS_BYTES, st, C, ldc, A, lda, B, ldb, K, ntc, row0t,
+                           col0t, tri, tq.plan, tq.cnt);
         return;
     }
     LDS_OPT_IN((k_update_nt<4, true>));
@@ -129,40 +186,6 @@
 }
 #endif
 
-__host__ __device__ __forceinline__ int trtri_rows_last(int nt, int nbt) {
-    const int pairs = (nt + 2 * nbt - 1) / (2 * nbt), right0 = (2 * (pairs - 1) + 1) * nbt;
-    const int rows = nt - right0;
-    return rows < 0 ? 0 : (rows > nbt ? nbt : rows);
-}
-__host__ __device__ __forceinline__ long trtri_level_tiles(int nt, int nbt) {
-    const int pairs = (nt + 2 * nbt - 1) / (2 * nbt);
-    return (long)(pairs - 1) * nbt * nbt + (long)nbt * trtri_rows_last(nt, nbt);
-}
-template <int STAGE>
-__device__ __forceinline__ void trtri_map(int bid, int nt, int nbt, int& p, int& ri, int& cj) {
-    const int per = nbt * nbt, pairs = (nt + 2 * nbt - 1) / (2 * nbt), full = (pairs - 1) * per;
-    if (bid < full) {
-        p = bid / per;
-        const int rem = bid - p * per;
-        if (STAGE == 1) {
-            cj = rem / nbt;
-            ri = rem - cj * nbt;
-        } else {
-            ri = nbt - 1 - rem / nbt;
-            cj = rem % nbt;
-        }
-    } else {
-        p = pairs - 1;
-        const int rem = bid - full, rows = trtri_rows_last(nt, nbt);
-        if (STAGE == 1) {
-            cj = rem / rows;
-            ri = rem - cj * rows;
-        } else {
-            ri = rows - 1 - rem / nbt;
-            cj = rem % nbt;
-        }
-    }
-}
 
 template <int STAGE, int NW>
 __device__ __forceinline__ void trtri_stage_tile(int bid, const double* __restrict__ L, double* __restrict__ X,
@@ -232,12 +255,31 @@
     }
 }
 
+template <int STAGE>
+__global__ LB(4) void k_trtri_stage_xcd(const double* __restrict__ L, double* __restrict__ X, double* __restrict__ T, long ld, int nt,
+                                        int nbt, const int* __restrict__ plan, int* __restrict__ cnt) {
+    extern __shared__ __attribute__((aligned(16))) double smem[];
+    tq_drain<false>(plan, cnt, [&](int bid) { trtri_stage_tile<STAGE, 4>(bid, L, X, T, ld, nt, nbt, smem); });
+}
+
+template <int STAGE>
+static void launch_trtri_stage_xcd(hipStream_t st, const double* L, double* X, double* T, long ld, int nt, int nbt, TileQueue tq,
+                                   int grid) {
+    LDS_OPT_IN((k_trtri_stage_xcd<STAGE>));
+    hipLaunchKernelGGL((k_trtri_stage_xcd<STAGE>), dim3((unsigned)grid), dim3(256), GT_LDS_BYTES, st, L, X, T, ld, nt, nbt, tq.plan,
+                       tq.cnt);
+}
+
 void launch_trtri_stage1_steal(hipStream_t st, const double* L, double* X, double* T, long ld, int nt, int level,
-                               int* counter, int grid) {
+                               int* counter, int grid, TileQueue tq) {
     const int nbt = 1 << level;
     if (nbt >= nt) return;
     const int nblocks = (int)trtri_level_tiles(nt, nbt);
     if (nblocks <= 0) return;
+    if (tq.plan) {
+        launch_trtri_stage_xcd<1>(st, L, X, T, ld, nt, nbt, tq, grid < tq.wgs ? grid : tq.wgs);
+        return;
+    }
     LDS_OPT_IN(k_trtri_stage1_steal);
     if (grid > nblocks) grid = nblocks;
     hipLaunchKernelGGL(k_trtri_stage1_steal, dim3((unsigned)grid), dim3(256), GT_LDS_BYTES, st, L, X, T, ld, nt, nbt,
@@ -255,7 +297,8 @@
         hipLaunchKernelGGL((k_trtri_stage<2, NW>), dim3((unsigned)nblocks), dim3(NW * 64), GT_LDS_BYTES, st, L, X, T, ld, nt, nbt);
 }
 
-void launch_trtri_level(hipStream_t st, const double* L, double* X, double* T, long ld, int nt, int level, int stages) {
+void launch_trtri_level(hipStream_t st, const double* L, double* X, double* T, long ld, int nt, int level, int stages,
+                        TileQueue tq1, TileQueue tq2) {
     const int nbt = 1 << level;
     if (nbt >= nt) return;
     const long nblocks = trtri_level_tiles(nt, nbt);
@@ -268,13 +311,25 @@
             hipLaunchKernelGGL((k_trtri_stage64<2>), dim3((unsigned)(4 * nblocks)), dim3(256), GT64_LDS_BYTES, st, L, X, T, ld, nt, nbt);
         return;
     }
-    launch_trtri_level_t<4>(st, nblocks, L, X, T, ld, nt, nbt, stages);
+    if ((stages & 1) && tq1.plan) {
+        launch_trtri_stage_xcd<1>(st, L, X, T, ld, nt, nbt, tq1, tq1.wgs);
+        stages &= ~1;
+    }
+    if ((stages & 2) && tq2.plan) {
+        if (stages & 1) launch_trtri_level_t<4>(st, nblocks, L, X, T, ld, nt, nbt, 1);
+        launch_trtri_stage_xcd<2>(st, L, X, T, ld, nt, nbt, tq2, tq2.wgs);
+        return;
+    }
+    if (stages) launch_trtri_level_t<4>(st, nblocks, L, X, T, ld, nt, nbt, stages);
+}
+
+bool trtri_level_uses_64(int nt, int level) {
+    static const int tri64_max = env_int("TRI64_MAX", GEMM_DEFAULT_TRI64_MAX);
+    return trtri_level_tiles(nt, 1 << level) <= tri64_max;
 }
 
 template <int NW>
-__global__ LB(NW) void k_lauum(const double* __restrict__ X, double* __restrict__ W, long ld, int nt) {
-    extern __shared__ __attribute__((aligned(16))) double smem[];
-    const int bid = blockIdx.x;
+__device__ __forceinline__ void lauum_tile(int bid, const double* __restrict__ X, double* __restrict__ W, long ld, int nt, double* smem) {
     int ti = (int)((sqrtf(8.0f * (float)bid + 1.0f) - 1.0f) * 0.5f);
     while ((long)ti * (ti + 1) / 2 > bid) --ti;
     while ((long)(ti + 1) * (ti + 2) / 2 <= bid) ++ti;
@@ -285,6 +340,18 @@
     gemm_tile_128<false, false, NW>(X + (long)ti * NB * ld + (long)ti * NB, ld, X + (long)ti * NB * ld + (long)tj * NB, ld,
                                 K, acc, smem);
     gt_store<0, NW>(W + (long)ti * NB * ld + (long)tj * NB, ld, acc);
+}
+
+template <int NW>
+__global__ LB(NW) void k_lauum(const double* __restrict__ X, double* __restrict__ W, long ld, int nt) {
+    extern __shared__ __attribute__((aligned(16))) double smem[];
+    lauum_tile<NW>((int)blockIdx.x, X, W, ld, nt, smem);
+}
+
+__global__ LB(4) void k_lauum_xcd(const double* __restrict__ X, double* __restrict__ W, long ld, int nt,
+                                  const int* __restrict__ plan, int* __restrict__ cnt) {
+    extern __shared__ __attribute__((aligned(16))) double smem[];
+    tq_drain<false>(plan, cnt, [&](int bid) { lauum_tile<4>(bid, X, W, ld, nt, smem); });
 }
 
 __global__ __launch_bounds__(256) void k_lauum64(const double* __restrict__ X, double* __restrict__ W, long ld, int nt) {
@@ -431,11 +498,16 @@
     return (long)nt * (nt + 1) / 2 <= lauum64_max;
 }
 
-void launch_lauum(hipStream_t st, const double* X, double* W, long ld, int nt) {
+void launch_lauum(hipStream_t st, const double* X, double* W, long ld, int nt, TileQueue tq) {
     const long nblocks = (long)nt * (nt + 1) / 2;
     static const int lauum64_max = env_int("LAUUM64_MAX", GEMM_DEFAULT_LAUUM64_MAX);
     if (nblocks <= lauum64_max) {
         hipLaunchKernelGGL(k_lauum64, dim3((unsigned)(4 * nblocks)), dim3(256), GT64_LDS_BYTES, st, X, W, ld, nt);
+        return;
+    }
+    if (tq.plan) {
+        LDS_OPT_IN(k_lauum_xcd);
+        hipLaunchKernelGGL(k_lauum_xcd, dim3((unsigned)tq.wgs), dim3(256), GT_LDS_BYTES, st, X, W, ld, nt, tq.plan, tq.cnt);
         return;
     }
     launch_lauum_t<4>(st, nblocks, X, W, ld, nt);
diff --git a/gpy_amd/csrc/internal.h b/gpy_amd/csrc/internal.h
--- a/gpy_amd/csrc/internal.h
+++ b/gpy_amd/csrc/internal.h
@@ -9,11 +9,14 @@
 #ifdef MI355GP_DIAG
 void launch_update_nt_queue(hipStream_t st, double* A, long ld, const UpdTask* tasks_dev, int ntasks, int* counter, int wgs);
 #endif
+#define TQ_HDR 16
+struct TileQueue { const int* plan = nullptr; int* cnt = nullptr; int wgs = 0, tiles = 0; };
 void launch_update_nt(hipStream_t st, double* C, long ldc, const double* A, long lda, const double* B, long ldb,
-                      int K, int ntr, int ntc, int row0t, int col0t);
+                      int K, int ntr, int ntc, int row0t, int col0t, TileQueue tq = TileQueue());
 void launch_trtri_level(hipStream_t st, const double* L, double* X, double* T, long ld, int nt, int level,
-                        int stages = 3);
-void launch_lauum(hipStream_t st, const double* X, double* W, long ld, int nt);
+                        int stages = 3, TileQueue tq1 = TileQueue(), TileQueue tq2 = TileQueue());
+bool trtri_level_uses_64(int nt, int level);
+void launch_lauum(hipStream_t st, const double* X, double* W, long ld, int nt, TileQueue tq = TileQueue());
 struct LauumItem { int ti, tj, q, k0, klen, part; };
 struct LauumSum { int ti, tj, q, first, n; };
 void lauum_split_plan(int nt, std::vector<LauumItem>& items, std::vector<LauumSum>& sums, int* nparts);
@@ -36,7 +39,7 @@
                     int exclusive = 0);
 void launch_trsm128(hipStream_t st, double* A, long ld, long c0, long r0, long mrows, const double* dinv);
 void launch_trtri_stage1_steal(hipStream_t st, const double* L, double* X, double* T, long ld, int nt, int level,
-                               int* counter, int grid);
+                               int* counter, int grid, TileQueue tq = TileQueue());
 void launch_inv128(hipStream_t st, const double* L, double* X, long ld, int nblk, const double* dinv_all);
 void launch_dbg_mfma(hipStream_t st, const double* a, const double* b, double* d);
 
@@ -103,6 +106,12 @@
     int persist_grid_last = 0;
     int persist_tune = 0;
     int persist_test = 0;
+    int tile_order = -1, tq_wgs = 0, tq_default_fams = TILE_ORDER_DEFAULT_FAMILIES;
+    struct TqPlan { int fam, a, b, c; int* dev; };
+    std::vector<TqPlan> tq_plans;
+    int* tq_cnt = nullptr;
+    int tq_next[5] = {-1, -1, -1, -1, -1};
+    TileQueue tq_steal;
     int* persist_sync = nullptr;
     double* persist_hs = nullptr;
     KernelProf prof;
diff --git a/gpy_amd/csrc/tile_plan.h b/gpy_amd/csrc/tile_plan.h
--- /dev/null
+++ b/gpy_amd/csrc/tile_plan.h
@@ -0,0 +1,117 @@
+#pragma once
+#include <algorithm>
+#include <vector>
+
+#if defined(__HIPCC__)
+#define TP_HD __host__ __device__ __forceinline__
+#else
+#define TP_HD inline
+#endif
+
+#define TP_NQ 8
+
+TP_HD int trtri_rows_last(int nt, int nbt) {
+    const int pairs = (nt + 2 * nbt - 1) / (2 * nbt), right0 = (2 * (pairs - 1) + 1) * nbt;
+    const int rows = nt - right0;
+    return rows < 0 ? 0 : (rows > nbt ? nbt : rows);
+}
+TP_HD long trtri_level_tiles(int nt, int nbt) {
+    const int pairs = (nt + 2 * nbt - 1) / (2 * nbt);
+    return (long)(pairs - 1) * nbt * nbt + (long)nbt * trtri_rows_last(nt, nbt);
+}
+template <int STAGE>
+TP_HD void trtri_map(int bid, int nt, int nbt, int& p, int& ri, int& cj) {
+    const int per = nbt * nbt, pairs = (nt + 2 * nbt - 1) / (2 * nbt), full = (pairs - 1) * per;
+    if (bid < full) {
+        p = bid / per;
+        const int rem = bid - p * per;
+        if (STAGE == 1) {
+            cj = rem / nbt;
+            ri = rem - cj * nbt;
+        } else {
+            ri = nbt - 1 - rem / nbt;
+            cj = rem % nbt;
+        }
+    } else {
+        p = pairs - 1;
+        const int rem = bid - full, rows = trtri_rows_last(nt, nbt);
+        if (STAGE == 1) {
+            cj = rem / rows;
+            ri = rem - cj * rows;
+        } else {
+            ri = rows - 1 - rem / nbt;
+            cj = rem % nbt;
+        }
+    }
+}
+
+struct TilePlanItem { int bid, sb, work; };
+struct TilePlan {
+    std::vector<int> order;
+    std::vector<int> sb, work;
+    int qoff[TP_NQ + 1] = {0};
+};
+
+inline void tile_plan_build(std::vector<TilePlanItem> items, TilePlan& plan) {
+    std::stable_sort(items.begin(), items.end(), [](const TilePlanItem& a, const TilePlanItem& b) { return a.sb < b.sb; });
+    struct Block { size_t first, n; long work; };
+    std::vector<Block> blocks;
+    for (size_t i = 0; i < items.size(); ++i) {
+        if (i == 0 || items[i].sb != items[i - 1].sb) blocks.push_back(Block{i, 0, 0});
+        blocks.back().n += 1;
+        blocks.back().work += items[i].work;
+    }
+    std::stable_sort(blocks.begin(), blocks.end(), [](const Block& a, const Block& b) { return a.work > b.work; });
+    std::vector<size_t> of_queue[TP_NQ];
+    long load[TP_NQ] = {0};
+    for (size_t b = 0; b < blocks.size(); ++b) {
+        int q = 0;
+        for (int k = 1; k < TP_NQ; ++k)
+            if (load[k] < load[q]) q = k;
+        of_queue[q].push_back(b);
+        load[q] += blocks[b].work;
+    }
+    plan.order.clear();
+    plan.sb.clear();
+    plan.work.clear();
+    for (int q = 0; q < TP_NQ; ++q) {
+        plan.qoff[q] = (int)plan.order.size();
+        for (size_t b : of_queue[q])
+            for (size_t i = blocks[b].first; i < blocks[b].first + blocks[b].n; ++i) {
+                plan.order.push_back(items[i].bid);
+                plan.sb.push_back(items[i].sb);
+                plan.work.push_back(items[i].work);
+            }
+    }
+    plan.qoff[TP_NQ] = (int)plan.order.size();
+}
+
+inline void tile_items_update(int ntr, int ntc, int delta, int tri, int sbr, int sbc, std::vector<TilePlanItem>& items) {
+    items.clear();
+    const int nbc = (ntc + sbc - 1) / sbc;
+    for (int ti = 0; ti < ntr; ++ti)
+        for (int tj = 0; tj < ntc; ++tj) {
+            if (tj > delta + ti) continue;
+            const int bid = tri ? ti * (ti + 1) / 2 + tj : ti * ntc + tj;
+            items.push_back(TilePlanItem{bid, (ti / sbr) * nbc + tj / sbc, 1});
+        }
+}
+
+template <int STAGE>
+inline void tile_items_trtri(int nt, int nbt, int sbr, int sbc, std::vector<TilePlanItem>& items) {
+    items.clear();
+    const int n = (int)trtri_level_tiles(nt, nbt), nbr = (nbt + sbr - 1) / sbr, nbc = (nbt + sbc - 1) / sbc;
+    for (int bid = 0; bid < n; ++bid) {
+        int p, ri, cj;
+        trtri_map<STAGE>(bid, nt, nbt, p, ri, cj);
+        if ((2 * p + 1) * nbt + ri >= nt) continue;
+        items.push_back(TilePlanItem{bid, (p * nbr + ri / sbr) * nbc + cj / sbc, STAGE == 1 ? nbt - cj : ri + 1});
+    }
+}
+
+inline void tile_items_lauum(int nt, int sbr, int sbc, std::vector<TilePlanItem>& items) {
+    items.clear();
+    const int nbc = (nt + sbc - 1) / sbc;
+    for (int ti = 0; ti < nt; ++ti)
+        for (int tj = 0; tj <= ti; ++tj) items.push_back(TilePlanItem{ti * (ti + 1) / 2 + tj, (ti / sbr) * nbc + tj / sbc, nt - ti});
+}
diff --git a/include/mi355gp.h b/include/mi355gp.h
--- a/include/mi355gp.h
+++ b/include/mi355gp.h
@@ -126,7 +126,7 @@
        MI355GP_OPT_TRI_H = 4, MI355GP_OPT_TRI_WGS = 5, MI355GP_OPT_TRI_HALF = 6, MI355GP_OPT_PART1_ON_PANEL = 7,
        MI355GP_OPT_NBO = 8, MI355GP_OPT_SOLVE_OVERLAP = 9, MI355GP_OPT_DIAG_EXCL_FIRST = 10, MI355GP_OPT_GRAPH = 11,
        MI355GP_OPT_PERSIST = 12, MI355GP_OPT_AGG2 = 13, MI355GP_OPT_PERSIST_TEST = 14, MI355GP_OPT_PERSIST_ABORTS = 15,
-       MI355GP_OPT_PERSIST_SKIP = 16, MI355GP_OPT_PERSIST_SCHED = 17, MI355GP_OPT_NUM = 18 };
+       MI355GP_OPT_PERSIST_SKIP = 16, MI355GP_OPT_PERSIST_SCHED = 17, MI355GP_OPT_TILE_ORDER = 18, MI355GP_OPT_NUM = 19 };
 int mi355gp_set_option(mi355gp_ctx* ctx, int option, int value);
 int mi355gp_get_option(mi355gp_ctx* ctx, int option, int* value);
 enum { MI355GP_PF_UPDATE = 0 , MI355GP_PF_TRTRI = 1, MI355GP_PF_LAUUM = 2,
```

New measurement: 13.81 iters/s. No clear change (-0.5%).
